# MycroftAI/mimic3

Hardware: AMD Instinct MI355X
Metric: 22.05 kHz audio samples/sec/node (en_UK/apope_low VITS hot path: run + int16, host ids in -> host int16 out) (higher is better)
Workload: dtype f32 (dense convs: operands split exactly into 3 x bf16, 6 bf16-MFMA products per multiply-add, f32 accumulate; f32 in / f32 out, parity at the f32 tolerances)

## Files before the change

include/mi355vits_lab.h:

```cpp
#ifndef MI355VITS_LAB_H
#define MI355VITS_LAB_H

#include "mi355vits.h"

#ifdef __cplusplus
extern "C" {
#endif

typedef struct mi355vits_conv_test {
    int32_t impl, B, Cin, Cout, T, K, dilation;
    const float* x;
    const float* w;
    const float* bias;
    const float* res;
    const int32_t* in_len;
    const int32_t* out_len;
    float in_slope;
    int32_t relu;
    float out_scale;
    int32_t res_sub;
    float* y;
    int32_t accumulate;
    int32_t math;
    const float* cond;
    int32_t mask_before_res;
    int32_t fixed_rule;
} mi355vits_conv_test;
int mi355vits_test_conv1d(int device, const mi355vits_conv_test* t);
int mi355vits_test_conv_transpose1d(int device, int impl, int B, int Cin, int Cout, int Tin, int K, int stride,
                                    const float* x, const float* w, const float* bias, float in_slope, const int32_t* in_len, float* y);
enum {
    MI355VITS_CONVK_GENERIC = 0, MI355VITS_CONVK_F32_STAGED = 1, MI355VITS_CONVK_F32_DIRECT = 2, MI355VITS_CONVK_F32_SPLITK = 3,
    MI355VITS_CONVK_B3_STAGED32 = 4, MI355VITS_CONVK_B3_STAGED64 = 5, MI355VITS_CONVK_B3_PC = 6, MI355VITS_CONVK_ENC_B3 = 7,
    MI355VITS_CONVK_ENC_B3W8 = 8, MI355VITS_CONVK_ENC_B3W6 = 9, MI355VITS_CONVK_RB_CONV = 10, MI355VITS_CONVK_RB_CONV_PW = 11,
    MI355VITS_CONVK_UPS_PL = 12, MI355VITS_CONVK_UPS64 = 13, MI355VITS_CONVK_CONVT_GENERIC = 14
};
typedef struct mi355vits_conv_plan {
    int32_t kernel;
    int32_t cols, rows;
    int32_t MT, NT, WM, WN;
    int32_t chunk;
    int32_t ring;
    int32_t rb_loop;
    int32_t vec, yvec, ovec;
    int32_t grid[3];
    int32_t lds_bytes;
} mi355vits_conv_plan;
int mi355vits_lab_conv_plan(int impl, int B, int Cin, int Cout, int T, int K, int dilation, int stride, int math, int fixed_rule,
                            int has_res, int has_cond, const int32_t* len, mi355vits_conv_plan* out);
int mi355vits_test_enc_o_ln(int device, int math, int B, int T, const float* x, const float* w, const float* bias, const float* res,
                            const float* gamma, const float* beta, float eps, const int32_t* in_len, const int32_t* ln_out_len,
                            int in_place, float* y);
int mi355vits_test_conv_post(int device, int B, int Cin, int K, int L, const float* x, const float* w, const int32_t* valid_len,
                             const double* volumes, float* audio, float* peaks, int16_t* pcm, int32_t* kernel);
int mi355vits_test_fill_workspace(mi355vits_handle h, uint32_t pattern);
int mi355vits_test_rel_attention(int device, int impl, int B, int T, int H, int n_heads, int W, const float* qkv,
                                 const float* emb_rel_k, const float* emb_rel_v, const int32_t* len, float* out);
typedef struct mi355vits_wn_test {
    int32_t impl, B, H, T, K, dilation, Crs, skip_init, math;
    const float* h_in;
    const float* w_in;
    const float* b_in;
    const float* w_rs;
    const float* b_rs;
    const float* cond;
    const int32_t* len;
    float* h_out;
    float* skip;
} mi355vits_wn_test;
int mi355vits_test_wn_layer(int device, const mi355vits_wn_test* t);
int mi355vits_lab_wn_plan(int B, int T, int K, int dilation, int32_t* b3_tile, int32_t* f32_geometry);
typedef struct mi355vits_mrf_test {
    int32_t impl, B, C, T, nrb, math, seg;
    int32_t k[4], d1[4], d2[4];
    const float* x;
    const float* w[4][2];
    const float* bias[4][2];
    const int32_t* len;
    float out_scale;
    float* y;
} mi355vits_mrf_test;
int mi355vits_test_mrf_stage(int device, const mi355vits_mrf_test* t);
int mi355vits_lab_mrf_plan(int impl, int C, int nrb, const int32_t* k, const int32_t* d1, const int32_t* d2, int32_t* width,
                           int32_t* halo, int32_t* x_ring, int32_t* x1_ring);
typedef struct mi355vits_dds_stack_test {
    int32_t impl, math, B, C, T, K, n_layers, pre_mode, zch, proj_cout, spline, nb;
    float tail, inv_sqrt_fc;
    const float* src;
    const float* pre_w;
    const float* pre_b;
    const float* cond;
    const float* dw_w[4];
    const float* dw_b[4];
    const float* g1[4];
    const float* b1[4];
    const float* w1x1[4];
    const float* bias1x1[4];
    const float* g2[4];
    const float* b2[4];
    const float* proj_w;
    const float* proj_b;
    const int32_t* len;
    float* z;
    float* out;
    float* x_out;
} mi355vits_dds_stack_test;
int mi355vits_test_dds_stack(int device, const mi355vits_dds_stack_test* t);
int mi355vits_test_spline_inverse(int device, int B, int T, int nb, int ch_x0, float tail, float inv_sqrt_fc, const float* theta,
                                  const int32_t* len, float* z);
int mi355vits_test_durations(int device, int B, int T, int ch, float ea_m, float ea_logs, const float* z, const int32_t* len,
                             const int32_t* forced, const float* scales, float* logw, int32_t* w_ceil, int32_t* cum, int32_t* ylen);
int mi355vits_test_fit_durations(int device, int B, int T, const float* u, const int32_t* len, const int32_t* min_frames,
                                 const int32_t* target, int32_t* frames, int32_t* cum, int32_t* ylen, float* factor, int32_t* status);
int mi355vits_test_expand_prior(int device, int B, int I, int Tx, int Ty, const float* stats, const int32_t* cum, const int32_t* ylen,
                                const float* injected, int injected_frames, const float* scales, float* z);
int mi355vits_test_speaker_cond(int device, int B, int gin, int n_speakers, int Cout, const float* emb_g, const int64_t* sid,
                                const float* w, const float* bias, float* out, size_t out_floats);
typedef struct mi355vits_speaker_mix_test {
    int32_t B, gin, n_speakers, n_terms, n_jobs;
    const float* emb_g;
    const int64_t* mix_sid;
    const float* mix_weight;
    const float* vectors;
    const float* w[10];
    const float* bias[10];
    int32_t Cout[10];
    float* out[10];
    size_t out_floats[10];
    float* g;
    size_t g_floats;
} mi355vits_speaker_mix_test;
int mi355vits_test_speaker_cond_mix(int device, const mi355vits_speaker_mix_test* t);
int mi355vits_test_levels(int device, int B, int T, int hop, const int32_t* cum, const int32_t* len, const float* gain,
                          const int32_t* ramp, const int32_t* alen, int64_t audio_bs, float* audio, size_t audio_floats, float* peaks);
int mi355vits_test_pitch_table(float* out, size_t capacity);
int mi355vits_test_pitch_plan(int device, int B, int T, int hop, const int32_t* cum, const int32_t* len, const float* ratio,
                              int64_t* tq, int32_t* wc, int32_t* wlen);
int mi355vits_test_pitch(int device, int B, int T, int hop, const int32_t* cum, const int32_t* len, const float* ratio,
                         const float* x, int64_t x_bs, size_t x_floats, float* y, int64_t y_bs, int32_t y_ld, size_t y_floats,
                         float* peaks, int32_t* wlen);
int mi355vits_test_resample(int device, int B, int64_t row_stride, const float* x, const int32_t* lengths, int32_t in_hz,
                            int32_t out_hz, int64_t y_stride, float* y, int32_t* y_lengths, float* peaks);
int mi355vits_test_alignment(int device, int B, int T, const int32_t* frames, const int32_t* len, int64_t row_stride, const float* audio,
                             const int32_t* alen, int32_t hop, int32_t L, int32_t M, int32_t* out_frames, int32_t* out_start,
                             int32_t* out_samples, float* out_peak, float* out_rms);
int mi355vits_lab_edges(const float* audio, long stride, const int32_t* lens, const float* peaks, int B, float ratio, int32_t* s_first,
                        int32_t* s_last);
int mi355vits_lab_loudness(const float* audio, long stride, const int32_t* lens, int B, int32_t rate, double* lufs, int32_t* blocks,
                           int32_t* gated);
int mi355vits_lab_limit(const float* audio, long stride, const int32_t* lens, int B, const double* g, double c, double U, int32_t L,
                        float* scale_out, int64_t* sq_min, int32_t* reduced);
int mi355vits_lab_limit_env(const float* audio, long stride, const int32_t* lens, int B, const double* g, double c, double U, int32_t L,
                            const double* env, float* scale_out, int64_t* sq_min, int32_t* reduced);
int mi355vits_lab_true_peak(const float* audio, long stride, const int32_t* lens, int B, int32_t offset_floats, double* tp, double* env_out);
// ... 18 lines not shown
```

mimic3_amd/_native.py:

```python
from __future__ import annotations

import contextlib
import ctypes
import os
import threading
from typing import Dict, List, Optional, Tuple

import numpy as np

from .config import CVitsConfig, VitsConfig

WANT_FLOAT = 1
WANT_PCM16 = 2
DEVICE_ONLY = 4
DEBUG_TAPS = 8

_HERE = os.path.dirname(os.path.abspath(__file__))
DEFAULT_LIBRARY = os.path.join(_HERE, "csrc", "libmi355vits.so")
HOOKS_LIBRARY = os.path.join(_HERE, "csrc", "libmi355vits_hooks.so")

EXPORTED_SYMBOLS = (
    "mi355vits_version", "mi355vits_device_count", "mi355vits_create", "mi355vits_create_from_buffer", "mi355vits_clone", "mi355vits_destroy",
    "mi355vits_device_result", "mi355vits_set_math", "mi355vits_get_math",
    "mi355vits_get_config", "mi355vits_run", "mi355vits_run_rows", "mi355vits_run_timed", "mi355vits_run_speakers", "mi355vits_run_levels", "mi355vits_run_pitch",
    "mi355vits_get_speaker_embedding", "mi355vits_fetch", "mi355vits_free_result",
    "mi355vits_last_error", "mi355vits_profile_enable", "mi355vits_profile_reset",
    "mi355vits_profile_report", "mi355vits_last_run_ms", "mi355vits_get_tap", "mi355vits_get_tap_rows", "mi355vits_list_taps",
    "mi355vits_run_packed", "mi355vits_fetch_packed", "mi355vits_free_packed",
    "mi355vits_set_output_rate", "mi355vits_get_output_rate",
    "mi355vits_set_output_encoding", "mi355vits_get_output_encoding",
    "mi355vits_set_output_compression", "mi355vits_get_output_compression",
    "mi355vits_fetch_alignment", "mi355vits_free_alignment",
    "mi355vits_set_edge_trim", "mi355vits_get_edge_trim", "mi355vits_fetch_edges", "mi355vits_free_edges",
    "mi355vits_set_loudness_target", "mi355vits_get_loudness_target", "mi355vits_fetch_loudness", "mi355vits_free_loudness",
    "mi355vits_run_streams", "mi355vits_fetch_streams", "mi355vits_free_streams",
    "mi355vits_run_streams2", "mi355vits_fetch_streams2", "mi355vits_free_streams2",
    "mi355vits_set_loudness_limiter", "mi355vits_get_loudness_limiter", "mi355vits_fetch_limiter", "mi355vits_free_limiter",
    "mi355vits_set_loudness_ceiling_mode", "mi355vits_get_loudness_ceiling_mode", "mi355vits_fetch_true_peak", "mi355vits_free_true_peak",
)
LAB_SYMBOLS = (
    "mi355vits_test_conv1d", "mi355vits_test_conv_transpose1d", "mi355vits_test_mfma_layout", "mi355vits_bench_conv1d", "mi355vits_probe_device", "mi355vits_probe_weights",
    "mi355vits_test_rel_attention", "mi355vits_test_fill_workspace", "mi355vits_test_resample",
    "mi355vits_lab_g711_encode", "mi355vits_test_alignment", "mi355vits_lab_edges",
    "mi355vits_lab_loudness", "mi355vits_lab_loudness_plan", "mi355vits_lab_limit",
    "mi355vits_lab_limit_env", "mi355vits_lab_true_peak", "mi355vits_lab_true_peak_plan", "mi355vits_lab_flac", "mi355vits_lab_flac_jobs",
    "mi355vits_test_wn_layer", "mi355vits_lab_wn_plan", "mi355vits_test_mrf_stage", "mi355vits_lab_mrf_plan",
    "mi355vits_test_dds_stack", "mi355vits_test_spline_inverse", "mi355vits_test_durations", "mi355vits_test_expand_prior",
    "mi355vits_test_fit_durations", "mi355vits_test_speaker_cond", "mi355vits_test_speaker_cond_mix", "mi355vits_test_levels",
    "mi355vits_test_pitch_table", "mi355vits_test_pitch_plan", "mi355vits_test_pitch",
    "mi355vits_lab_conv_plan", "mi355vits_test_enc_o_ln", "mi355vits_test_conv_post",
)


class NativeError(RuntimeError):
    def __init__(self, code: int, message: str):
        super().__init__(f"mi355vits error {code}: {message}")
        self.code = code


class WnTest(ctypes.Structure):
    _fields_ = [(n, ctypes.c_int32) for n in ("impl", "B", "H", "T", "K", "dilation", "Crs", "skip_init", "math")] + [
        (n, ctypes.POINTER(ctypes.c_float)) for n in ("h_in", "w_in", "b_in", "w_rs", "b_rs", "cond")] + [
        ("len", ctypes.POINTER(ctypes.c_int32)), ("h_out", ctypes.POINTER(ctypes.c_float)), ("skip", ctypes.POINTER(ctypes.c_float))]


class MrfTest(ctypes.Structure):
    _fields_ = [(n, ctypes.c_int32) for n in ("impl", "B", "C", "T", "nrb", "math", "seg")] + [
        (n, ctypes.c_int32 * 4) for n in ("k", "d1", "d2")] + [
        ("x", ctypes.POINTER(ctypes.c_float)), ("w", (ctypes.POINTER(ctypes.c_float) * 2) * 4),
        ("bias", (ctypes.POINTER(ctypes.c_float) * 2) * 4), ("len", ctypes.POINTER(ctypes.c_int32)),
        ("out_scale", ctypes.c_float), ("y", ctypes.POINTER(ctypes.c_float))]


class DdsStackTest(ctypes.Structure):
    _fields_ = [(n, ctypes.c_int32) for n in ("impl", "math", "B", "C", "T", "K", "n_layers", "pre_mode", "zch", "proj_cout", "spline", "nb")] + [
        ("tail", ctypes.c_float), ("inv_sqrt_fc", ctypes.c_float)] + [
        (n, ctypes.POINTER(ctypes.c_float)) for n in ("src", "pre_w", "pre_b", "cond")] + [
        (n, ctypes.POINTER(ctypes.c_float) * 4) for n in ("dw_w", "dw_b", "g1", "b1", "w1x1", "bias1x1", "g2", "b2")] + [
        ("proj_w", ctypes.POINTER(ctypes.c_float)), ("proj_b", ctypes.POINTER(ctypes.c_float)), ("len", ctypes.POINTER(ctypes.c_int32)),
        ("z", ctypes.POINTER(ctypes.c_float)), ("out", ctypes.POINTER(ctypes.c_float)), ("x_out", ctypes.POINTER(ctypes.c_float))]


MATH_F32, MATH_BF16X3, MATH_BF16W = 0, 1, 2


class RunArgs(ctypes.Structure):
    _fields_ = [
        ("batch", ctypes.c_int32),
        ("tx_max", ctypes.c_int32),
        ("ids", ctypes.POINTER(ctypes.c_int64)),
        ("lengths", ctypes.POINTER(ctypes.c_int64)),
        ("scales", ctypes.POINTER(ctypes.c_float)),
        ("sid", ctypes.POINTER(ctypes.c_int64)),
        ("seed", ctypes.c_uint64),
        ("utterance_base", ctypes.c_uint64),
        ("noise_w", ctypes.POINTER(ctypes.c_float)),
        ("noise_z", ctypes.POINTER(ctypes.c_float)),
        ("noise_z_frames", ctypes.c_int32),
        ("forced_durations", ctypes.POINTER(ctypes.c_int32)),
        ("flags", ctypes.c_uint32),
        ("pcm_volume", ctypes.c_double),
    ]


class RowArgs(ctypes.Structure):
    _fields_ = [
        ("scales", ctypes.POINTER(ctypes.c_float)),
        ("pcm_volume", ctypes.POINTER(ctypes.c_double)),
        ("utterance", ctypes.POINTER(ctypes.c_uint64)),
    ]


class TimingArgs(ctypes.Structure):
    _fields_ = [
        ("stretch", ctypes.POINTER(ctypes.c_float)),
        ("min_frames", ctypes.POINTER(ctypes.c_int32)),
        ("target_frames", ctypes.POINTER(ctypes.c_int32)),
        ("factor_out", ctypes.POINTER(ctypes.c_float)),
        ("reserved", ctypes.c_int32 * 6),
    ]


class SpeakerArgs(ctypes.Structure):
    _fields_ = [
        ("n_terms", ctypes.c_int32),
        ("mix_sid", ctypes.POINTER(ctypes.c_int64)),
        ("mix_weight", ctypes.POINTER(ctypes.c_float)),
        ("vectors", ctypes.POINTER(ctypes.c_float)),
        ("reserved", ctypes.c_int32 * 6),
# ... 400 lines not shown
        L.mi355vits_free_streams2.restype = None
        L.mi355vits_fetch_alignment.argtypes = [H, ctypes.c_uint32, ctypes.POINTER(AlignmentResult)]
        L.mi355vits_free_alignment.argtypes = [ctypes.POINTER(AlignmentResult)]
        L.mi355vits_free_alignment.restype = None
        L.mi355vits_set_edge_trim.argtypes = [H, ctypes.c_float, ctypes.c_int32]
        L.mi355vits_get_edge_trim.argtypes = [H, ctypes.POINTER(ctypes.c_float), ctypes.POINTER(ctypes.c_int32)]
        L.mi355vits_fetch_edges.argtypes = [H, ctypes.POINTER(EdgesResult)]
        L.mi355vits_free_edges.argtypes = [ctypes.POINTER(EdgesResult)]
        L.mi355vits_free_edges.restype = None
        L.mi355vits_set_loudness_target.argtypes = [H, ctypes.c_float, ctypes.c_float]
        L.mi355vits_get_loudness_target.argtypes = [H, ctypes.POINTER(ctypes.c_float), ctypes.POINTER(ctypes.c_float)]
        L.mi355vits_fetch_loudness.argtypes = [H, ctypes.POINTER(LoudnessResult)]
        L.mi355vits_free_loudness.argtypes = [ctypes.POINTER(LoudnessResult)]
        L.mi355vits_free_loudness.restype = None
        L.mi355vits_set_loudness_limiter.argtypes = [H, ctypes.c_int32]
        L.mi355vits_get_loudness_limiter.argtypes = [H]
        L.mi355vits_get_loudness_limiter.restype = ctypes.c_int32
        L.mi355vits_fetch_limiter.argtypes = [H, ctypes.POINTER(LimiterResult)]
        L.mi355vits_free_limiter.argtypes = [ctypes.POINTER(LimiterResult)]
        L.mi355vits_free_limiter.restype = None
        L.mi355vits_set_loudness_ceiling_mode.argtypes = [H, ctypes.c_int]
        L.mi355vits_get_loudness_ceiling_mode.argtypes = [H]
        L.mi355vits_fetch_true_peak.argtypes = [H, ctypes.POINTER(TruePeakResult)]
        L.mi355vits_free_true_peak.argtypes = [ctypes.POINTER(TruePeakResult)]
        L.mi355vits_free_true_peak.restype = None
        L.mi355vits_last_error.argtypes = [H]
        L.mi355vits_last_error.restype = ctypes.c_char_p
        L.mi355vits_profile_enable.argtypes = [H, ctypes.c_int]
        L.mi355vits_profile_reset.argtypes = [H]
        L.mi355vits_profile_report.argtypes = [H, ctypes.c_char_p, ctypes.c_size_t]
        L.mi355vits_profile_report.restype = ctypes.c_long
        L.mi355vits_last_run_ms.argtypes = [H]
        L.mi355vits_last_run_ms.restype = ctypes.c_float
        L.mi355vits_get_tap.argtypes = [H, ctypes.c_char_p, ctypes.POINTER(ctypes.c_float), ctypes.c_size_t,
                                        ctypes.POINTER(ctypes.c_int64)]
        L.mi355vits_get_tap.restype = ctypes.c_long
        L.mi355vits_get_tap_rows.argtypes = [H, ctypes.c_char_p, ctypes.c_long, ctypes.c_long, ctypes.POINTER(ctypes.c_float), ctypes.c_size_t,
                                            ctypes.POINTER(ctypes.c_int64)]
        L.mi355vits_get_tap_rows.restype = ctypes.c_long
        L.mi355vits_list_taps.argtypes = [H, ctypes.c_char_p, ctypes.c_size_t]
        L.mi355vits_list_taps.restype = ctypes.c_long
        present = [hasattr(L, sym) for sym in LAB_SYMBOLS]
        if any(present) and not all(present):
            raise RuntimeError(f"{self.path} exports only part of include/mi355vits_lab.h")
        self.has_hooks = all(present)
        if self.has_hooks:
            L.mi355vits_test_conv1d.argtypes = [ctypes.c_int, ctypes.POINTER(ConvTest)]
            L.mi355vits_test_conv_transpose1d.argtypes = [
                ctypes.c_int, ctypes.c_int, ctypes.c_int, ctypes.c_int, ctypes.c_int, ctypes.c_int, ctypes.c_int,
                ctypes.c_int, ctypes.POINTER(ctypes.c_float), ctypes.POINTER(ctypes.c_float),
                ctypes.POINTER(ctypes.c_float), ctypes.c_float, ctypes.POINTER(ctypes.c_int32), ctypes.POINTER(ctypes.c_float)]
            L.mi355vits_test_fill_workspace.argtypes = [ctypes.c_void_p, ctypes.c_uint32]
            L.mi355vits_test_mfma_layout.argtypes = [ctypes.c_int, ctypes.POINTER(ctypes.c_float)]
            L.mi355vits_bench_conv1d.argtypes = [ctypes.c_int] * 9 + [ctypes.POINTER(ctypes.c_float)]
            L.mi355vits_probe_device.argtypes = [ctypes.c_int, ctypes.POINTER(ctypes.c_double)]
            L.mi355vits_probe_weights.argtypes = [ctypes.c_void_p, ctypes.POINTER(ctypes.c_double)]
            L.mi355vits_test_resample.argtypes = [ctypes.c_int, ctypes.c_int, ctypes.c_int64, ctypes.POINTER(ctypes.c_float),
                                                  ctypes.POINTER(ctypes.c_int32), ctypes.c_int32, ctypes.c_int32, ctypes.c_int64,
                                                  ctypes.POINTER(ctypes.c_float), ctypes.POINTER(ctypes.c_int32),
                                                  ctypes.POINTER(ctypes.c_float)]
            L.mi355vits_lab_g711_encode.argtypes = [ctypes.c_int, ctypes.POINTER(ctypes.c_int16), ctypes.c_long, ctypes.POINTER(ctypes.c_uint8)]
            i32p, f32p = ctypes.POINTER(ctypes.c_int32), ctypes.POINTER(ctypes.c_float)
            L.mi355vits_lab_flac.argtypes = [ctypes.c_void_p, ctypes.c_long, ctypes.c_int32, ctypes.c_int32, ctypes.POINTER(ctypes.c_uint8),
                                             ctypes.c_size_t, ctypes.POINTER(ctypes.c_size_t), i32p]
            L.mi355vits_lab_flac_jobs.argtypes = [ctypes.POINTER(ctypes.c_void_p), ctypes.POINTER(ctypes.c_long), ctypes.c_int32, ctypes.c_int32,
                                                  ctypes.POINTER(ctypes.c_uint8), ctypes.c_size_t, ctypes.POINTER(ctypes.c_size_t),
                                                  ctypes.POINTER(ctypes.c_int64), ctypes.POINTER(ctypes.c_int64)]
            L.mi355vits_lab_edges.argtypes = [f32p, ctypes.c_long, i32p, f32p, ctypes.c_int, ctypes.c_float, i32p, i32p]
            L.mi355vits_lab_loudness.argtypes = [f32p, ctypes.c_long, i32p, ctypes.c_int, ctypes.c_int32, ctypes.POINTER(ctypes.c_double), i32p, i32p]
            L.mi355vits_lab_loudness_plan.argtypes = [ctypes.c_int32, i32p, i32p, i32p]
            L.mi355vits_lab_limit.argtypes = [f32p, ctypes.c_long, i32p, ctypes.c_int, ctypes.POINTER(ctypes.c_double), ctypes.c_double,
                                              ctypes.c_double, ctypes.c_int32, f32p, ctypes.POINTER(ctypes.c_int64), i32p]
            f64p = ctypes.POINTER(ctypes.c_double)
            L.mi355vits_lab_limit_env.argtypes = [f32p, ctypes.c_long, i32p, ctypes.c_int, f64p, ctypes.c_double, ctypes.c_double,
                                                  ctypes.c_int32, f64p, f32p, ctypes.POINTER(ctypes.c_int64), i32p]
            L.mi355vits_lab_true_peak.argtypes = [f32p, ctypes.c_long, i32p, ctypes.c_int, ctypes.c_int32, f64p, f64p]
            L.mi355vits_lab_true_peak_plan.argtypes = [f64p, i32p]
            L.mi355vits_test_alignment.argtypes = [ctypes.c_int, ctypes.c_int, ctypes.c_int, i32p, i32p, ctypes.c_int64, f32p, i32p,
                                                   ctypes.c_int32, ctypes.c_int32, ctypes.c_int32, i32p, i32p, i32p, f32p, f32p]
            L.mi355vits_test_rel_attention.argtypes = [ctypes.c_int] * 7 + [ctypes.POINTER(ctypes.c_float)] * 3 + [
                ctypes.POINTER(ctypes.c_int32), ctypes.POINTER(ctypes.c_float)]
            L.mi355vits_test_wn_layer.argtypes = [ctypes.c_int, ctypes.POINTER(WnTest)]
            L.mi355vits_lab_wn_plan.argtypes = [ctypes.c_int] * 4 + [i32p, i32p]
            L.mi355vits_test_mrf_stage.argtypes = [ctypes.c_int, ctypes.POINTER(MrfTest)]
            L.mi355vits_lab_mrf_plan.argtypes = [ctypes.c_int] * 3 + [i32p] * 7
            L.mi355vits_lab_conv_plan.argtypes = [ctypes.c_int] * 12 + [i32p, ctypes.POINTER(ConvPlan)]
            L.mi355vits_test_enc_o_ln.argtypes = [ctypes.c_int] * 4 + [f32p] * 6 + [ctypes.c_float, i32p, i32p, ctypes.c_int, f32p]
            L.mi355vits_test_conv_post.argtypes = [ctypes.c_int] * 5 + [f32p, f32p, i32p, ctypes.POINTER(ctypes.c_double), f32p, f32p,
                                                   ctypes.POINTER(ctypes.c_int16), i32p]
            L.mi355vits_test_dds_stack.argtypes = [ctypes.c_int, ctypes.POINTER(DdsStackTest)]
            L.mi355vits_test_spline_inverse.argtypes = [ctypes.c_int] * 5 + [ctypes.c_float, ctypes.c_float, f32p, i32p, f32p]
            L.mi355vits_test_fit_durations.argtypes = [ctypes.c_int] * 3 + [f32p, i32p, i32p, i32p, i32p, i32p, i32p, f32p, i32p]
            L.mi355vits_test_speaker_cond.argtypes = [ctypes.c_int] * 5 + [f32p, ctypes.POINTER(ctypes.c_int64), f32p, f32p, f32p, ctypes.c_size_t]
            L.mi355vits_test_speaker_cond_mix.argtypes = [ctypes.c_int, ctypes.POINTER(SpeakerMixTest)]
            L.mi355vits_test_levels.argtypes = [ctypes.c_int] * 4 + [i32p, i32p, f32p, i32p, i32p, ctypes.c_int64, f32p, ctypes.c_size_t, f32p]
            L.mi355vits_test_pitch_table.argtypes = [f32p, ctypes.c_size_t]
            L.mi355vits_test_pitch_plan.argtypes = [ctypes.c_int] * 4 + [i32p, i32p, f32p, ctypes.POINTER(ctypes.c_int64), i32p, i32p]
            L.mi355vits_test_pitch.argtypes = [ctypes.c_int] * 4 + [i32p, i32p, f32p, f32p, ctypes.c_int64, ctypes.c_size_t, f32p, ctypes.c_int64,
                                               ctypes.c_int32, ctypes.c_size_t, f32p, i32p]
            L.mi355vits_test_durations.argtypes = [ctypes.c_int] * 4 + [ctypes.c_float, ctypes.c_float, f32p, i32p, i32p, f32p, f32p, i32p, i32p, i32p]
            L.mi355vits_test_expand_prior.argtypes = [ctypes.c_int] * 5 + [f32p, i32p, i32p, f32p, ctypes.c_int, f32p, f32p]

    def _need_hooks(self):
        if not self.has_hooks:
            raise RuntimeError(f"{self.path} is the product library: the hooks of include/mi355vits_lab.h live in "
                               "libmi355vits_hooks.so (mimic3_amd._native.hooks_library()), the lab build and the CPU model")

    def version(self) -> str:
        return self.lib.mi355vits_version().decode()

    def device_count(self) -> int:
        return int(self.lib.mi355vits_device_count())

    def create_error(self) -> str:
        return (self.lib.mi355vits_last_error(None) or b"").decode("utf-8", "replace")

    def lab_g711_encode(self, law, samples) -> np.ndarray:
        self._need_hooks()
        x = np.ascontiguousarray(samples, np.int16).reshape(-1)
        out = np.empty(x.shape[0], np.uint8)
        rc = self.lib.mi355vits_lab_g711_encode(encoding_id(law), x.ctypes.data_as(ctypes.POINTER(ctypes.c_int16)), x.shape[0],
                                                out.ctypes.data_as(ctypes.POINTER(ctypes.c_uint8)))
        if rc != 0:
            raise NativeError(rc, self.create_error())
        return out

    def lab_flac(self, samples, rate: int, first_frame: int = 0):
        self._need_hooks()
        x = np.asarray(samples)
        if x.dtype != np.int16 or x.ndim != 1 or not x.flags.c_contiguous:
            x = np.ascontiguousarray(samples, np.int16).reshape(-1)
        n = int(x.shape[0])
        frames = (n + 4095) // 4096
        out = np.empty(42 + 16 * frames + 2 * n, np.uint8)
        sizes = np.zeros(max(frames, 1), np.int32)
        got = ctypes.c_size_t(0)
        rc = self.lib.mi355vits_lab_flac(ctypes.c_void_p(x.ctypes.data), n, int(rate), int(first_frame),
                                         out.ctypes.data_as(ctypes.POINTER(ctypes.c_uint8)), out.shape[0], ctypes.byref(got),
                                         sizes.ctypes.data_as(ctypes.POINTER(ctypes.c_int32)))
        if rc != 0:
            raise NativeError(rc, self.create_error())
        return out[: int(got.value)].tobytes(), sizes[:frames].copy()

    def lab_flac_jobs(self, arrays, rate: int):
        self._need_hooks()
        xs = []
        for a in arrays:
            x = np.asarray(a)
            if x.dtype != np.int16 or x.ndim != 1 or not x.flags.c_contiguous:
                x = np.ascontiguousarray(a, np.int16).reshape(-1)
            xs.append(x)
        J = len(xs)
        ptrs = (ctypes.c_void_p * max(J, 1))(*[x.ctypes.data for x in xs])
        ns = (ctypes.c_long * max(J, 1))(*[int(x.shape[0]) for x in xs])
        cap = sum(((42 + 16 * ((int(x.shape[0]) + 4095) // 4096) + 2 * int(x.shape[0]) + 15) & ~15) for x in xs) + 16
        out = np.empty(cap, np.uint8)
        offsets, sizes = np.zeros(max(J, 1), np.int64), np.zeros(max(J, 1), np.int64)
        got = ctypes.c_size_t(0)
        rc = self.lib.mi355vits_lab_flac_jobs(ptrs, ns, J, int(rate), out.ctypes.data_as(ctypes.POINTER(ctypes.c_uint8)), cap, ctypes.byref(got),
                                              offsets.ctypes.data_as(ctypes.POINTER(ctypes.c_int64)),
                                              sizes.ctypes.data_as(ctypes.POINTER(ctypes.c_int64)))
        if rc != 0:
            raise NativeError(rc, self.create_error())
        return out[: int(got.value)].copy(), offsets[:J].copy(), sizes[:J].copy()

    def lab_edges(self, audio, lengths, peaks, ratio):
# ... 163 lines not shown
        assert C == 192 and res.shape == x.shape and w.shape == (C, C, 1) and gamma.shape == beta.shape == (C,)
        y = np.zeros_like(x) if y_prior is None else f(y_prior).copy()
        i32 = lambda a: None if a is None else np.ascontiguousarray(a, np.int32)
        il, ol = i32(in_len), i32(ln_out_len)
        ip = lambda a: None if a is None else a.ctypes.data_as(ctypes.POINTER(ctypes.c_int32))
        rc = self.lib.mi355vits_test_enc_o_ln(device, int(math), B, T, _fptr(x), _fptr(w), _fptr(bias), _fptr(res), _fptr(gamma), _fptr(beta),
                                              float(eps), ip(il), ip(ol), int(bool(in_place)), _fptr(y))
        if rc != 0:
            raise NativeError(rc, self.create_error())
        return y

    def test_conv_post(self, x, w, valid_len, volumes=None, audio_prior=None, pcm_prior=None, device=0):
        self._need_hooks()
        x = np.ascontiguousarray(x, np.float32)
        w = np.ascontiguousarray(w, np.float32)
        B, Cin, L = x.shape
        assert w.shape[:2] == (1, Cin)
        K = w.shape[2]
        vl = np.ascontiguousarray(valid_len, np.int32)
        assert vl.shape == (B,)
        vol = None if volumes is None else np.ascontiguousarray(volumes, np.float64)
        audio = np.zeros((B, L), np.float32) if audio_prior is None else np.ascontiguousarray(audio_prior, np.float32).copy()
        pcm = np.zeros((B, L), np.int16) if pcm_prior is None else np.ascontiguousarray(pcm_prior, np.int16).copy()
        peaks = np.full(B, -1.0, np.float32)
        kernel = ctypes.c_int32(-1)
        rc = self.lib.mi355vits_test_conv_post(device, B, Cin, K, L, _fptr(x), _fptr(w), vl.ctypes.data_as(ctypes.POINTER(ctypes.c_int32)),
                                               None if vol is None else vol.ctypes.data_as(ctypes.POINTER(ctypes.c_double)), _fptr(audio),
                                               _fptr(peaks), pcm.ctypes.data_as(ctypes.POINTER(ctypes.c_int16)), ctypes.byref(kernel))
        if rc != 0:
            raise NativeError(rc, self.create_error())
        return audio, peaks, pcm, int(kernel.value)

    def emu_set_cu_count(self, n: int) -> None:
        if not hasattr(self.lib, "mi355vits_emu_set_cu_count"):
            raise RuntimeError(f"{self.path} is not the CPU model of the kernels")
        self.lib.mi355vits_emu_set_cu_count(ctypes.c_int(int(n)))

    def test_rel_attention(self, qkv, emb_rel_k, emb_rel_v, lengths, n_heads, impl=2, device=0) -> np.ndarray:
        self._need_hooks()
        qkv = np.ascontiguousarray(qkv, np.float32)
        ek = np.ascontiguousarray(emb_rel_k, np.float32)
        ev = np.ascontiguousarray(emb_rel_v, np.float32)
        ln = np.ascontiguousarray(lengths, np.int32)
        B, H3, T = qkv.shape
        H = H3 // 3
        W = (ek.shape[0] - 1) // 2
        out = np.zeros((B, H, T), np.float32)
        rc = self.lib.mi355vits_test_rel_attention(device, impl, B, T, H, n_heads, W, _fptr(qkv), _fptr(ek), _fptr(ev),
                                                   ln.ctypes.data_as(ctypes.POINTER(ctypes.c_int32)), _fptr(out))
        if rc != 0:
            raise NativeError(rc, self.create_error())
        return out

    def test_wn_layer(self, h, skip, w_in, b_in, w_rs, b_rs, lengths, dilation=1, cond=None, skip_init=False, impl=1, math=None,
                      h_out_prior=None, device=0):
        self._need_hooks()
        f = lambda a: np.ascontiguousarray(a, np.float32)
        h, w_in, b_in, w_rs, b_rs = f(h), f(w_in), f(b_in), f(w_rs), f(b_rs)
        skip = f(skip).copy()
        B, H, T = h.shape
        ln = np.ascontiguousarray(lengths, np.int32)
        h_out = np.zeros_like(h) if h_out_prior is None else f(h_out_prior).copy()
        assert skip.shape == h.shape == h_out.shape and w_in.shape[:2] == (2 * H, H) and w_rs.shape[1:] == (H, 1) and ln.shape == (B,)
        assert b_in.shape == (2 * H,) and b_rs.shape == (w_rs.shape[0],)
        c = None if cond is None else f(cond)
        assert c is None or c.shape == (B, 2 * H)
        t = WnTest()
        t.impl, t.B, t.H, t.T, t.K, t.dilation, t.Crs, t.skip_init = impl, B, H, T, w_in.shape[2], int(dilation), w_rs.shape[0], int(bool(skip_init))
        t.math = (MATH_BF16X3 if impl == 2 else MATH_F32) if math is None else int(math)
        t.h_in, t.w_in, t.b_in, t.w_rs, t.b_rs, t.cond = _fptr(h), _fptr(w_in), _fptr(b_in), _fptr(w_rs), _fptr(b_rs), _fptr(c)
        t.len, t.h_out, t.skip = ln.ctypes.data_as(ctypes.POINTER(ctypes.c_int32)), _fptr(h_out), _fptr(skip)
        rc = self.lib.mi355vits_test_wn_layer(device, ctypes.byref(t))
        if rc != 0:
            raise NativeError(rc, self.create_error())
        return h_out, skip

    def lab_wn_plan(self, B, T, K=5, dilation=1):
        self._need_hooks()
        tile, geom = ctypes.c_int32(), ctypes.c_int32()
        rc = self.lib.mi355vits_lab_wn_plan(int(B), int(T), int(K), int(dilation), ctypes.byref(tile), ctypes.byref(geom))
        if rc != 0:
            raise NativeError(rc, self.create_error())
        return int(tile.value), int(geom.value)

    def test_mrf_stage(self, x, ks, d1, d2, weights, biases, lengths, impl=0, math=None, out_scale=0.0, seg=0, y_prior=None, device=0):
        self._need_hooks()
        x = np.ascontiguousarray(x, np.float32)
        B, C, T = x.shape
        ln = np.ascontiguousarray(lengths, np.int32)
        y = np.zeros_like(x) if y_prior is None else np.ascontiguousarray(y_prior, np.float32).copy()
        nrb = len(ks)
        assert y.shape == x.shape and ln.shape == (B,) and 1 <= nrb <= 4 and len(d1) == len(d2) == len(weights) == len(biases) == nrb
        t = MrfTest()
        t.impl, t.B, t.C, t.T, t.nrb, t.seg = impl, B, C, T, nrb, int(seg)
        t.math = (MATH_F32 if impl == 0 else MATH_BF16X3) if math is None else int(math)
        keep = []
        for j in range(nrb):
            t.k[j], t.d1[j], t.d2[j] = int(ks[j]), int(d1[j]), int(d2[j])
            for q in range(2):
                w = np.ascontiguousarray(weights[j][q], np.float32)
                bq = np.ascontiguousarray(biases[j][q], np.float32)
                assert w.shape == (C, C, ks[j]) and bq.shape == (C,)
                keep += [w, bq]
                t.w[j][q], t.bias[j][q] = _fptr(w), _fptr(bq)
        t.x, t.len, t.out_scale, t.y = _fptr(x), ln.ctypes.data_as(ctypes.POINTER(ctypes.c_int32)), float(out_scale), _fptr(y)
        rc = self.lib.mi355vits_test_mrf_stage(device, ctypes.byref(t))
        if rc != 0:
            raise NativeError(rc, self.create_error())
        return y

    def lab_mrf_plan(self, impl, C, ks, d1, d2):
        self._need_hooks()
        arr = lambda v: (ctypes.c_int32 * len(v))(*[int(e) for e in v])
        out = [ctypes.c_int32() for _ in range(4)]
        rc = self.lib.mi355vits_lab_mrf_plan(int(impl), int(C), len(ks), arr(ks), arr(d1), arr(d2), *[ctypes.byref(o) for o in out])
        if rc != 0:
            raise NativeError(rc, self.create_error())
        return tuple(int(o.value) for o in out)

    def test_dds_stack(self, src, pre_w, pre_b, layers, lengths, impl=2, math=None, cond=None, z=None, zch=0, proj_w=None, proj_b=None,
                       spline=False, nb=0, tail=0.0, inv_sqrt_fc=0.0, out_prior=None, x_out_prior=None, device=0):
        self._need_hooks()
        f = lambda a: np.ascontiguousarray(a, np.float32)
        src, pre_w, pre_b = f(src), f(pre_w), f(pre_b)
        B, C, T = src.shape
        ln = np.ascontiguousarray(lengths, np.int32)
        affine = pre_w.ndim == 1
        assert pre_w.shape == ((C,) if affine else (C, C, 1)) and pre_b.shape == (C,) and ln.shape == (B,) and 1 <= len(layers) <= 4
        t = DdsStackTest()
        keep = []
        K = np.asarray(layers[0]["dw_w"]).shape[2]
        for i, lay in enumerate(layers):
            for name, shape in (("dw_w", (C, 1, K)), ("dw_b", (C,)), ("g1", (C,)), ("b1", (C,)), ("w1x1", (C, C, 1)), ("bias1x1", (C,)),
                                ("g2", (C,)), ("b2", (C,))):
                a = f(lay[name])
                assert a.shape == shape, (name, a.shape, shape)
                keep.append(a)
                getattr(t, name)[i] = _fptr(a)
        c = None if cond is None else f(cond)
        assert c is None or c.shape == (B, C)
        zz = None if z is None else f(z).copy()
        assert zz is None or zz.shape == (B, 2, T)
        pw = None if proj_w is None else f(proj_w)
        pb = None if proj_b is None else f(proj_b)
        Cp = 0 if pw is None else pw.shape[0]
        assert pw is None or (pw.shape == (Cp, C, 1) and pb is not None and pb.shape == (Cp,))
        out = None if pw is None else (np.zeros((B, Cp, T), np.float32) if out_prior is None else f(out_prior).copy())
        x_out = np.zeros_like(src) if x_out_prior is None else f(x_out_prior).copy()
        assert x_out.shape == src.shape and (out is None or out.shape == (B, Cp, T))
        t.impl, t.B, t.C, t.T, t.K, t.n_layers, t.pre_mode, t.zch = int(impl), B, C, T, K, len(layers), int(affine), int(zch)
        t.math = (MATH_BF16X3 if impl == 3 else MATH_F32) if math is None else int(math)
        t.proj_cout, t.spline, t.nb, t.tail, t.inv_sqrt_fc = Cp, int(bool(spline)), int(nb), float(tail), float(inv_sqrt_fc)
        t.src, t.pre_w, t.pre_b, t.cond, t.proj_w, t.proj_b = _fptr(src), _fptr(pre_w), _fptr(pre_b), _fptr(c), _fptr(pw), _fptr(pb)
        t.len, t.z, t.out, t.x_out = ln.ctypes.data_as(ctypes.POINTER(ctypes.c_int32)), _fptr(zz), _fptr(out), _fptr(x_out)
        rc = self.lib.mi355vits_test_dds_stack(device, ctypes.byref(t))
        if rc != 0:
            raise NativeError(rc, self.create_error())
        return x_out, out, zz

    def test_spline_inverse(self, theta, z, lengths, nb, ch_x0=0, tail=5.0, inv_sqrt_fc=1.0, device=0) -> np.ndarray:
        self._need_hooks()
        theta = np.ascontiguousarray(theta, np.float32)
        z = np.ascontiguousarray(z, np.float32).copy()
        ln = np.ascontiguousarray(lengths, np.int32)
        B, _, T = z.shape
        assert z.shape == (B, 2, T) and theta.shape[0] == B and theta.shape[2] == T and ln.shape == (B,)
# ... 1008 lines not shown
```

mimic3_amd/csrc/b3.h:

```cpp
#pragma once
#include "kernels.h"

namespace m355 {

#ifdef MI355_EMU
static inline int b3_drop() {
    const char* e = getenv("MI355VITS_EMU_DROP");
    return e ? atoi(e) : 0;
}
#else
__device__ __forceinline__ constexpr int b3_drop() { return 0; }
#endif

template <int MT, int NT, int NG, int NA = NT, bool W1 = false>
__device__ __forceinline__ void b3_chunk(f32x16 (&acc)[MT][NA], const uint4* const (&wp)[MT], const uint4* __restrict__ xq, int PS ,
                                         int LD, int K, int groups_per_tap, int dil) {
    uint4 ra[2][MT][3];
    uint4 rb[2][NT][3];
    const int drop = b3_drop();
    constexpr int NPA = W1 ? 1 : 3;
    MI355_UNROLL
    for (int i = 0; i < MT; ++i)
        MI355_UNROLL
        for (int p = 0; p < NPA; ++p) ra[0][i][p] = wp[i][p * 64];
// ... 207 lines not shown
        MI355_UNROLL
        for (int i = 0; i < MT; ++i)
            MI355_UNROLL
            for (int p = 0; p < NPA; ++p) dst[i][p] = wp[i][woff + p * 64];
    };
    MI355_UNROLL
    for (int d = 0; d < D; ++d) load_a(d, ra[d]);
    MI355_UNROLL
    for (int j = 0; j < NT; ++j)
        MI355_UNROLL
        for (int p = 0; p < 3; ++p) rb[j][p] = xq[p * PS + j * 32];
    for (int k = 0; k < K; ++k) {
        const bool last_tap = k == K - 1;
        MI355_UNROLL
        for (int g = 0; g < NG; ++g) {
            const bool wrap = g + 1 == NG;
            const int xoff = wrap ? (last_tap ? k * dil + g * 2 * LD : (k + 1) * dil) : k * dil + (g + 1) * 2 * LD;
            load_a(k * NG + g + D, ra[(g + D) % RA]);
            SCHED_FENCE();
            MI355_UNROLL
            for (int j = 0; j < NT; ++j) {
                if constexpr (!W1) {
                    MI355_UNROLL
                    for (int i = 0; i < MT; ++i) acc[i][j] = MFMA_32x32x16_BF16(ra[g % RA][i][2], rb[j][0], acc[i][j]);
                }
                MI355_UNROLL
                for (int i = 0; i < MT; ++i) acc[i][j] = MFMA_32x32x16_BF16(ra[g % RA][i][0], rb[j][2], acc[i][j]);
                if constexpr (!W1) {
                    MI355_UNROLL
                    for (int i = 0; i < MT; ++i) acc[i][j] = MFMA_32x32x16_BF16(ra[g % RA][i][1], rb[j][1], acc[i][j]);
                    MI355_UNROLL
                    for (int i = 0; i < MT; ++i) acc[i][j] = MFMA_32x32x16_BF16(ra[g % RA][i][1], rb[j][0], acc[i][j]);
                }
                MI355_UNROLL
                for (int i = 0; i < MT; ++i) acc[i][j] = MFMA_32x32x16_BF16(ra[g % RA][i][0], rb[j][1], acc[i][j]);
                MI355_UNROLL
                for (int i = 0; i < MT; ++i) acc[i][j] = MFMA_32x32x16_BF16(ra[g % RA][i][0], rb[j][0], acc[i][j]);
                SCHED_FENCE();
                MI355_UNROLL
                for (int p = 0; p < 3; ++p) rb[j][p] = xq[p * PS + xoff + j * 32];
                SCHED_FENCE();
            }
        }
    }
}

template <int MT, int NT, int NG>
__device__ __forceinline__ void h2_chunk_lean(f32x16 (&acc)[MT][NT], const uint4* const (&wp)[MT], const uint4* __restrict__ xq, int PS, int LD,
                                              int K, int groups_per_tap, int dil) {
    uint4 ra[2][MT][2];
    uint4 rb[NT][2];
    MI355_UNROLL
    for (int i = 0; i < MT; ++i)
        MI355_UNROLL
        for (int p = 0; p < 2; ++p) ra[0][i][p] = wp[i][p * 64];
    MI355_UNROLL
    for (int j = 0; j < NT; ++j)
        MI355_UNROLL
        for (int p = 0; p < 2; ++p) rb[j][p] = xq[p * PS + j * 32];
    for (int k = 0; k < K; ++k) {
        const bool last_tap = k == K - 1;
        MI355_UNROLL
        for (int g = 0; g < NG; ++g) {
            const int cur = g & 1, nxt = cur ^ 1;
            const bool wrap = g + 1 == NG;
            const long woff = (wrap ? (last_tap ? (long)k * groups_per_tap + g : (long)(k + 1) * groups_per_tap) : (long)k * groups_per_tap + g + 1) * 128;
            const int xoff = wrap ? (last_tap ? k * dil + g * 2 * LD : (k + 1) * dil) : k * dil + (g + 1) * 2 * LD;
            MI355_UNROLL
            for (int i = 0; i < MT; ++i)
                MI355_UNROLL
                for (int p = 0; p < 2; ++p) ra[nxt][i][p] = wp[i][woff + p * 64];
            SCHED_FENCE();
            MI355_UNROLL
            for (int j = 0; j < NT; ++j) {
                MI355_UNROLL
                for (int i = 0; i < MT; ++i) acc[i][j] = MFMA_32x32x16_F16(ra[cur][i][1], rb[j][0], acc[i][j]);
                MI355_UNROLL
                for (int i = 0; i < MT; ++i) acc[i][j] = MFMA_32x32x16_F16(ra[cur][i][0], rb[j][1], acc[i][j]);
                MI355_UNROLL
                for (int i = 0; i < MT; ++i) acc[i][j] = MFMA_32x32x16_F16(ra[cur][i][0], rb[j][0], acc[i][j]);
                SCHED_FENCE();
                MI355_UNROLL
                for (int p = 0; p < 2; ++p) rb[j][p] = xq[p * PS + xoff + j * 32];
                SCHED_FENCE();
            }
        }
    }
}

template <int NG, int GB = 4, bool F16 = false>
__device__ __forceinline__ void stage_planes(const float* __restrict__ xb, long x_ld, int LD, int ts, int tend, float slope,
                                             uint4* __restrict__ planes, int PS, int tid, int nthreads) {
    static_assert((NG * 2) % GB == 0, "batches of GB (group, half) rows");
    const int last = tend > 0 ? tend - 1 : 0;
    int nparts = 1, part = 0, col0 = tid;
    if (nthreads >= 2 * LD) {
        nparts = nthreads / LD;
        part = tid / LD;
        col0 = tid - part * LD;
        if (part >= nparts) return;
    }
    for (int col = col0; col < LD; col += nthreads) {
        const int tt = ts + col;
        const bool in = tt >= 0 && tt < tend;
        const int tc = tt < 0 ? 0 : (tt > last ? last : tt);
        for (int g0 = part * GB; g0 < NG * 2; g0 += nparts * GB) {
            float v[GB][8];
            MI355_UNROLL
            for (int u = 0; u < GB; ++u) {
                const int gh = g0 + u, cbase = (gh >> 1) * 16 + (gh & 1) * 4;
                MI355_UNROLL
                for (int e = 0; e < 8; ++e) v[u][e] = xb[(long)(cbase + 8 * (e >> 2) + (e & 3)) * x_ld + tc];
            }
            SCHED_FENCE();
            MI355_UNROLL
            for (int u = 0; u < GB; ++u) {
                MI355_UNROLL
                for (int e = 0; e < 8; ++e) v[u][e] = in ? lrelu_f(v[u][e], slope) : 0.0f;
                const int o = (g0 + u) * LD + col;
                if constexpr (F16) {
                    MI355_UNROLL
                    for (int e = 0; e < 8; ++e) v[u][e] *= F16X2_X_SCALE;
                    uint4 h, m;
                    split2_pk(v[u][0], v[u][1], h.x, m.x);
                    split2_pk(v[u][2], v[u][3], h.y, m.y);
                    split2_pk(v[u][4], v[u][5], h.z, m.z);
                    split2_pk(v[u][6], v[u][7], h.w, m.w);
                    planes[o] = h;
                    planes[PS + o] = m;
                } else {
                    uint4 h, m, l;
                    split3_pk(v[u][0], v[u][1], h.x, m.x, l.x);
                    split3_pk(v[u][2], v[u][3], h.y, m.y, l.y);
                    split3_pk(v[u][4], v[u][5], h.z, m.z, l.z);
                    split3_pk(v[u][6], v[u][7], h.w, m.w, l.w);
                    planes[o] = h;
                    planes[PS + o] = m;
                    planes[2 * PS + o] = l;
                }
            }
        }
    }
}

}
```

mimic3_amd/csrc/engine.cpp:

```cpp
#include "engine.h"

#include <algorithm>
#include <cmath>
#include <cstdlib>
#include <cstring>
#include <fstream>
#include <sstream>
#include <type_traits>

namespace m355 {

namespace {
struct Reader {
    const unsigned char* p;
    size_t n, pos = 0;
    void need(size_t k) const {
        if (pos + k > n) throw EngineError(MI355VITS_ERR_FORMAT, "weight container truncated");
    }
    template <typename T> T get() {
        need(sizeof(T));
        T v;
        memcpy(&v, p + pos, sizeof(T));
        pos += sizeof(T);
        return v;
// ... 144 lines not shown
void Profiler::clear() {
    (void)hipStreamSynchronize(stream);
    for (auto& r : recs) { pool.push_back(r.a); pool.push_back(r.b); }
    recs.clear();
}
std::string Profiler::report() {
    HIP_CHECK(hipStreamSynchronize(stream));
    struct Agg { long calls = 0; double ms = 0, flops = 0, bytes = 0; };
    std::vector<Agg> agg(names.size());
    for (auto& r : recs) {
        float ms = 0;
        if (hipEventElapsedTime(&ms, r.a, r.b) != hipSuccess) ms = 0;
        Agg& a = agg[r.name_id];
        a.calls++;
        a.ms += ms;
        a.flops += r.flops;
        a.bytes += r.bytes;
    }
    std::ostringstream os;
    os.precision(9);
    for (size_t i = 0; i < names.size(); ++i)
        if (agg[i].calls) os << names[i] << " " << agg[i].calls << " " << agg[i].ms << " " << agg[i].flops << " " << agg[i].bytes << "\n";
    return os.str();
}

size_t Engine::stage(const float* p, size_t n) {
    const size_t off = (host_stage_.size() + 63) & ~size_t(63);
    host_stage_.resize(off + n);
    if (n) memcpy(host_stage_.data() + off, p, n * sizeof(float));
    return off;
}

const ConvW& Engine::add_conv_data(const std::string& key, const std::vector<float>& w, const std::vector<float>* bias,
                                   int Cout, int Cin, int K, int epi, ConvRole role) {
    if (w.size() != (size_t)Cout * Cin * K) throw EngineError(MI355VITS_ERR_INTERNAL, "add_conv_data size: " + key);
    ConvW c;
    c.Cout = Cout; c.Cin = Cin; c.K = K; c.epi = epi;
    c.raw = stage(w.data(), w.size());
    if (bias) c.bias = stage(bias->data(), bias->size());
    if (conv1d_mfma_supported(Cin, Cout, K, 1)) {
        std::vector<float> pk(mfma_packed_floats(Cout, Cin, K), 0.0f);
        pack_conv_weights_mfma_mode(w.data(), Cout, Cin, K, epi == EPI_GATE ? EPI_GATE : EPI_STD, pk.data());
        c.packed = stage(pk.data(), pk.size());
        const bool rb = role == ROLE_RESBLOCK && epi == EPI_STD;
        if (rb && Cin % 8 == 0 && Cout % 32 == 0) {
            std::vector<float> p4(pk.size());
            regroup_packed_x4(pk.data(), pk.size(), p4.data());
            c.packed4 = stage(p4.data(), p4.size());
        }
        if (rb && Cin % 16 == 0 && Cout % 32 == 0) {
            std::vector<uint32_t> b3(bf16x3_packed_words(Cout, Cin, K));
            pack_conv_weights_bf16x3(w.data(), Cout, Cin, K, b3.data());
            static_assert(sizeof(uint32_t) == sizeof(float), "bit patterns travel in the float arena");
            c.packed_b3 = stage(reinterpret_cast<const float*>(b3.data()), b3.size());
            std::vector<uint32_t> h2(f16x2_packed_words(Cout, Cin, K));
            if (pack_conv_weights_f16x2(w.data(), Cout, Cin, K, h2.data()))
                c.packed_h2 = stage(reinterpret_cast<const float*>(h2.data()), h2.size());
        }
        if (rb && Cin == Cout && Cin % 32 == 0 && (K == 3 || K == 5 || K == 7)) {
            std::vector<uint32_t> pp(p16_packed_words(Cout, Cin, K));
            pack_conv_weights_p16(w.data(), Cout, Cin, K, pp.data());
            c.packed_p = stage(reinterpret_cast<const float*>(pp.data()), pp.size());
        }
        if (role == ROLE_UPSAMPLER && epi == EPI_STD && (Cin == 64 || Cin == 128 || Cin == 256) && Cout % 128 == 0 && K == 2) {
            std::vector<uint32_t> pp(p16_packed_words(Cout, Cin, K));
            pack_conv_weights_p16n(w.data(), Cout, Cin, K, pp.data());
            c.packed_p = stage(reinterpret_cast<const float*>(pp.data()), pp.size());
        }
        if (Cin % 32 == 0 && (epi == EPI_GATE ? (Cout / 2) % 32 == 0 : true)) {
            const int pe = epi == EPI_GATE ? EPI_GATE : EPI_STD;
            std::vector<uint32_t> b3(bf16x3_packed_words_mode(Cout, Cin, K, pe));
            pack_conv_weights_bf16x3_mode(w.data(), Cout, Cin, K, pe, 1, b3.data());
            c.packed_b3s = stage(reinterpret_cast<const float*>(b3.data()), b3.size());
            std::vector<float> wg;
            if (epi == EPI_GATE && Cout % 32 == 0) {
                const int Hh = Cout / 2;
                const size_t row = (size_t)Cin * K;
                wg.resize(w.size());
                for (int q = 0; q < Cout / 32; ++q)
                    for (int r = 0; r < 32; ++r) {
                        const int src = (r < 16 ? 0 : Hh) + 16 * q + (r & 15);
                        memcpy(wg.data() + ((size_t)32 * q + r) * row, w.data() + (size_t)src * row, row * sizeof(float));
                    }
                std::vector<uint32_t> bw(bf16x3_packed_words_mode(Cout, Cin, K, EPI_STD));
                pack_conv_weights_bf16x3_mode(wg.data(), Cout, Cin, K, EPI_STD, 1, bw.data());
                c.packed_b3w = stage(reinterpret_cast<const float*>(bw.data()), bw.size());
            }
            if (Cin % 16 == 0 && Cout % 32 == 0) {
                std::vector<uint32_t> h2(f16x2_packed_words(Cout, Cin, K));
                if (pack_conv_weights_f16x2(wg.empty() ? w.data() : wg.data(), Cout, Cin, K, h2.data(), 1))
                    c.packed_h2s = stage(reinterpret_cast<const float*>(h2.data()), h2.size());
            }
        }
    }
    return model_->convs[key] = c;
}

const ConvW& Engine::add_conv(const WeightsFile& wf, const std::string& key, const std::string& tensor, int Cout, int Cin,
                              int K, bool bias, int epi, ConvRole role) {
    const HostTensor& w = wf.get(tensor + ".weight", {Cout, Cin, K});
    std::vector<float> wv(w.data, w.data + w.count), bv;
    if (bias) {
        const HostTensor& b = wf.get(tensor + ".bias", {Cout});
        bv.assign(b.data, b.data + b.count);
    }
    return add_conv_data(key, wv, bias ? &bv : nullptr, Cout, Cin, K, epi, role);
}

void Engine::add_vec(const WeightsFile& wf, const std::string& name, std::initializer_list<int> dims) {
    const HostTensor& t = wf.get(name, dims);
    model_->vecs[name] = stage(t.data, t.count);
}
const float* Engine::vec(const std::string& name) const {
    auto it = model_->vecs.find(name);
    if (it == model_->vecs.end()) throw EngineError(MI355VITS_ERR_INTERNAL, "unknown tensor: " + name);
    return model_->dev_weights + it->second;
}
const ConvW& Engine::cw(const std::string& key) const {
    auto it = model_->convs.find(key);
    if (it == model_->convs.end()) throw EngineError(MI355VITS_ERR_INTERNAL, "unknown conv: " + key);
    return it->second;
}

static std::string S(const char* fmt, int a = 0, int b = 0, int c = 0) {
    char buf[160];
    snprintf(buf, sizeof(buf), fmt, a, b, c);
    return buf;
}

static void validate_config(const mi355vits_config& c) {
    auto bad = [](const std::string& m) { throw EngineError(MI355VITS_ERR_FORMAT, "invalid voice config: " + m); };
    if (c.num_symbols < 1 || c.n_speakers < 1) bad("num_symbols / n_speakers");
    if (c.hidden_channels < 2 || c.hidden_channels % 2 || c.inter_channels < 2 || c.inter_channels % 2) bad("channel counts must be even");
    if (c.n_heads < 1 || c.hidden_channels % c.n_heads) bad("hidden_channels % n_heads");
    if (c.resblock != 1 && c.resblock != 2) bad("resblock must be 1 or 2");
    if (c.n_upsamples < 1 || c.n_upsamples > MI355VITS_MAX_STAGES) bad("n_upsamples");
    if (c.n_resblock_kernels < 1 || c.n_resblock_kernels > MI355VITS_MAX_STAGES) bad("n_resblock_kernels");
    long hop = 1;
    int ch = c.upsample_initial_channel;
    for (int i = 0; i < c.n_upsamples; ++i) {
        if (c.upsample_rates[i] < 1 || c.upsample_kernel_sizes[i] < c.upsample_rates[i]) bad("upsample stage");
        if ((c.upsample_kernel_sizes[i] - c.upsample_rates[i]) % 2) bad("upsample kernel - rate must be even");
        if (ch % 2) bad("upsample channels must halve evenly");
        ch /= 2;
        hop *= c.upsample_rates[i];
    }
    if (ch % 2) bad("decoder channel counts must be even");
    if (hop != c.hop_length) bad("hop_length must equal the product of upsample_rates");
    for (int j = 0; j < c.n_resblock_kernels; ++j) {
        if (c.resblock_kernel_sizes[j] < 1 || c.resblock_kernel_sizes[j] % 2 == 0) bad("resblock kernel sizes must be odd");
        if (c.resblock_n_dilations[j] < 1 || c.resblock_n_dilations[j] > MI355VITS_MAX_STAGES) bad("resblock dilations");
    }
    if (c.n_speakers > 1 && c.gin_channels < 1) bad("multi-speaker voice needs gin_channels");
    const bool det_dp = c.dp_n_flows == 0;
    if (det_dp ? (c.dp_num_bins != 0 || c.dp_dds_layers != 0) : (c.dp_num_bins < 2 || c.dp_num_bins > 16)) bad("dp_num_bins");
    if ((!det_dp && c.dp_n_flows < 2) || c.flow_n_flows < 1 || c.flow_wn_layers < 1) bad("flow depth");
    if (c.flow_wn_kernel % 2 == 0 || c.dp_kernel_size % 2 == 0) bad("flow / dp kernels must be odd");
    if (c.window_size < 0 || c.n_layers < 1 || c.kernel_size < 1) bad("encoder");
    if (c.num_symbols > (1 << 20) || c.n_speakers > (1 << 20) || c.hidden_channels > 8192 || c.inter_channels > 8192 ||
        c.filter_channels < 1 || c.filter_channels > 32768 || c.upsample_initial_channel < 2 || c.upsample_initial_channel > 8192 ||
        c.gin_channels < 0 || c.gin_channels > 8192)
        bad("channel / symbol counts out of range");
    if (c.n_layers > 64 || c.kernel_size > 63 || c.window_size > 15 || c.flow_n_flows > 32 || c.flow_wn_layers > 32 ||
        c.flow_wn_kernel < 1 || c.flow_wn_kernel > 63 || c.flow_wn_dilation_rate < 1 || c.flow_wn_dilation_rate > 8 ||
        c.dp_n_flows > 16 || (!det_dp && c.dp_dds_layers < 1) || c.dp_dds_layers > 8 || c.dp_kernel_size < 1 || c.dp_kernel_size > 63 ||
        !(c.dp_tail_bound > 0.0f) || c.hop_length > (1 << 16))
        bad("depth / kernel sizes out of range");
    for (int i = 0; i < c.n_upsamples; ++i)
        if (c.upsample_rates[i] > 64 || c.upsample_kernel_sizes[i] > 256) bad("upsample stage out of range");
// ... 757 lines not shown
    ConvArgs pr;
    pr.x = d_d0_; pr.x_bs = bs; pr.x_ld = Tx;
    pr.y = d_h_; pr.y_bs = bs; pr.y_ld = Tx;
    pr.in_len = d_len_; pr.out_len = d_len_;
    pr.B = B; pr.T = Tx;
    if (!stack) conv("dp.proj", cw("dp.proj"), pr);
    tap("dp.h", d_h_, {B, H, Tx});

    {
        ProfScope ps(prof_, "sdp.noise");
        launch_sdp_noise(d_z2_, d_noise_w_, B, Tx, d_scales_, in.seed, d_utt_, stream_);
    }
    int ch0 = 0;
    for (int j = c.dp_n_flows - 1; j >= 1; --j) {
        ch0 ^= 1;
        const std::string p = S("dp.flows.%d", 1 + 2 * j);
        if (stack && stack_w(cw(p + ".proj")) != nullptr) {
            DdsStackArgs a;
            a.src = d_h_;
            a.pre_mode = DDS_PRE_AFFINE;
            a.pre_w = vec(p + ".pre.weight");
            a.pre_b = vec(p + ".pre.bias");
            a.z = d_z2_;
            a.zch = ch0;
            stack_layers(a, p + ".convs");
            a.proj_w = stack_w(cw(p + ".proj"));
            a.proj_b = P(cw(p + ".proj").bias);
            a.proj_cout = nth;
            a.spline = 1;
            a.nb = c.dp_num_bins;
            a.tail = c.dp_tail_bound;
            a.inv_sqrt_fc = 1.0f / sqrtf((float)H);
            ProfScope ps(prof_, "convflow.stack", stack_flops * c.dp_dds_layers + 2.0 * B * (double)Tx * H * nth, 12.0 * B * H * Tx);
            launch_dds_stack(a, H, stream_);
            continue;
        }
        {
            ProfScope ps(prof_, "convflow.pre", 0, 12.0 * B * H * Tx);
            launch_convflow_pre(d_z2_, ch0, vec(p + ".pre.weight"), vec(p + ".pre.bias"), d_h_, B, H, Tx, d_d0_, stream_);
        }
        dds(p + ".convs", d_d0_, d_d1_, d_d2_, B, Tx);
        ConvArgs a;
        a.x = d_d0_; a.x_bs = bs; a.x_ld = Tx;
        a.y = d_theta_; a.y_bs = (long)nth * Tx; a.y_ld = Tx;
        a.in_len = d_len_; a.out_len = d_len_;
        a.B = B; a.T = Tx;
        conv("convflow.proj", cw(p + ".proj"), a);
        {
            ProfScope ps(prof_, "spline");
            launch_spline_inverse(d_z2_, ch0, d_theta_, d_len_, B, Tx, c.dp_num_bins, c.dp_tail_bound,
                                  1.0f / sqrtf((float)H), stream_);
        }
    }
    ch0 ^= 1;
    durations(in, ch0, model_->ea_m[0], model_->ea_logs[0]);
}

static const char* stage_label(int i, const char* const (&t)[4]) { return t[std::min(i, 3)]; }

void Engine::coupling_layer(int j, int B, int Ty) {
    const mi355vits_config& c = cfg_;
    const int H = c.hidden_channels, I = c.inter_channels, half = I / 2;
    const long zbs = (long)I * Ty, hbs = (long)H * Ty;
    const bool rev = ((c.flow_n_flows - 1 - j) % 2) == 0;
    float* x0 = d_z_ + (rev ? (long)half * Ty : 0);
    float* x1 = d_z_ + (rev ? 0 : (long)half * Ty);
    ConvArgs pre;
    pre.x = x0; pre.x_bs = zbs; pre.x_ld = Ty;
    pre.y = d_fh_; pre.y_bs = hbs; pre.y_ld = Ty;
    pre.out_len = d_ylen_;
    pre.B = B; pre.T = Ty;
    conv("flow.pre", cw(S("flow.%d.pre", j)), pre);
    float* hcur = d_fh_;
    float* hnext = d_fh2_;
    for (int l = 0; l < c.flow_wn_layers; ++l) {
        int dil = 1;
        for (int q = 0; q < l; ++q) dil *= c.flow_wn_dilation_rate;
        const ConvW& win = cw(S("flow.%d.in.%d", j, l));
        const ConvW& wrs = cw(S("flow.%d.rs.%d", j, l));
        const float* cond_l = d_cond_flow_.empty() ? nullptr : d_cond_flow_[j] + (long)l * 2 * H;
        const bool wn_b3 = sw_.wn_b3 && math_on_bf16(kmath()) && win.packed_b3s != NO_OFF && wrs.packed_b3s != NO_OFF &&
                           conv1d_b3_supported(win.Cin, win.Cout, win.K, dil, Ty) && !sw_.force_generic;
        const bool fused = !sw_.force_generic && !sw_.no_fused_wn && !wn_b3;
        const bool b3 = fused && math_on_bf16(kmath()) && win.packed_b3w != NO_OFF && wrs.packed_b3s != NO_OFF &&
                        wn_layer_b3_supported(H, win.K, dil);
        if (b3 || (fused && wn_layer_fused_supported(H, win.K, dil))) {
            const bool h2 = b3 && math_ == MATH_F16X2 && win.packed_h2s != NO_OFF && wrs.packed_h2s != NO_OFF;
            WnArgs w;
            w.h_in = hcur; w.h_out = hnext; w.h_bs = hbs; w.h_ld = Ty;
            w.skip = d_fskip_; w.s_bs = hbs; w.s_ld = Ty;
            w.w_in = P(h2 ? win.packed_h2s : (b3 ? win.packed_b3w : win.packed)); w.b_in = P(win.bias);
            w.w_rs = P(h2 ? wrs.packed_h2s : (b3 ? wrs.packed_b3s : wrs.packed)); w.b_rs = P(wrs.bias);
            w.cond = cond_l; w.cond_bs = 2L * H * c.flow_wn_layers;
            w.len = d_ylen_;
            w.B = B; w.H = H; w.T = Ty; w.K = win.K; w.dil = dil; w.Crs = wrs.Cout; w.skip_init = (l == 0);
            if (b3) w.math = h2 ? (int)MATH_F16X2 : kmath();
            const double fl = 2.0 * B * (double)Ty * H * ((double)win.Cout * win.K + wrs.Cout);
            ProfScope ps(prof_, b3 ? "flow.wn_layer_b3" : "flow.wn_layer", fl, 4.0 * B * (double)Ty * H * 4);
            if (b3) launch_wn_layer_b3(w, stream_);
            else launch_wn_layer(w, stream_);
            if (wrs.Cout == 2 * H) std::swap(hcur, hnext);
            continue;
        }
        ConvArgs in;
        in.x = hcur; in.x_bs = hbs; in.x_ld = Ty;
        in.y = d_fu_; in.y_bs = hbs; in.y_ld = Ty;
        in.epi = EPI_GATE; in.H = H; in.dil = dil;
        if (cond_l) {
            in.cond = cond_l;
            in.cond_bs = 2L * H * c.flow_wn_layers;
        }
        in.B = B; in.T = Ty;
        if (wn_b3) in.math = kmath();
        conv("flow.in_gate", win, in);
        ConvArgs rs;
        rs.x = d_fu_; rs.x_bs = hbs; rs.x_ld = Ty;
        rs.y = hcur; rs.y_bs = hbs; rs.y_ld = Ty;
        rs.y2 = d_fskip_; rs.y2_bs = hbs; rs.y2_ld = Ty;
        rs.epi = EPI_RESSKIP; rs.H = H; rs.skip_init = (l == 0);
        rs.out_len = d_ylen_;
        rs.B = B; rs.T = Ty;
        if (wn_b3) rs.math = kmath();
        conv("flow.res_skip", wrs, rs);
    }
    ConvArgs post;
    post.x = d_fskip_; post.x_bs = hbs; post.x_ld = Ty;
    post.y = x1; post.y_bs = zbs; post.y_ld = Ty;
    post.res = x1; post.res_bs = zbs; post.res_ld = Ty; post.res_sub = 1;
    post.in_len = d_ylen_; post.out_len = d_ylen_;
    post.B = B; post.T = Ty;
    conv("flow.post_couple", cw(S("flow.%d.post", j)), post);
}

ConvArgs Engine::rb2_conv_args(int i, int j, int m, int B, int ch, long T) const {
    const mi355vits_config& c = cfg_;
    float* const pp[2] = {d_bufB_, d_bufT_};
    const bool last = (m == c.resblock_n_dilations[j] - 1);
    const float* src = m == 0 ? d_bufA_ : pp[(m - 1) & 1];
    ConvArgs a;
    a.x = src; a.x_bs = (long)ch * T; a.x_ld = (int)T;
    a.y = last ? d_bufC_ : pp[m & 1]; a.y_bs = (long)ch * T; a.y_ld = (int)T;
    a.res = src; a.res_bs = (long)ch * T; a.res_ld = (int)T;
    a.in_slope = 0.1f; a.dil = c.resblock_dilations[j * MI355VITS_MAX_STAGES + m];
    a.in_len = d_slen_ + (long)(i + 1) * B;
    if (last) { a.out_scale = 1.0f / c.n_resblock_kernels; a.accumulate = (j > 0); }
    a.B = B; a.T = (int)T;
    return a;
}

int Engine::mrf_stage(int i, int B, int ch, long T) {
    const mi355vits_config& c = cfg_;
    const int nk = c.n_resblock_kernels;
    if (sw_.force_generic || sw_.no_fused_mrf || c.resblock != 2 || nk > MRF_MAX_RB) return 0;
    MrfArgs m;
    for (int j = 0; j < nk; ++j) {
        if (c.resblock_n_dilations[j] != 2) return 0;
        m.k[j] = c.resblock_kernel_sizes[j];
        m.d1[j] = c.resblock_dilations[j * MI355VITS_MAX_STAGES + 0];
        m.d2[j] = c.resblock_dilations[j * MI355VITS_MAX_STAGES + 1];
    }
    m.x = d_bufA_; m.x_bs = (long)ch * T; m.x_ld = (int)T;
    m.y = d_bufC_; m.y_bs = (long)ch * T; m.y_ld = (int)T;
    m.len = d_slen_ + (long)(i + 1) * B; m.B = B; m.C = ch; m.T = (int)T;
    m.len_host = h_slen_.data() + (size_t)(i + 1) * B;
    auto rb = [&](int j, int q) -> const ConvW& { return cw(S("dec.rb.%d.c.%d", i * nk + j, q)); };
    double flops = 0;
    auto take = [&](int n, size_t ConvW::*fmt) {
        flops = 0;
        for (int j = 0; j < n; ++j) {
            for (int q = 0; q < 2; ++q) {
                const ConvW& w = rb(j, q);
                if (w.*fmt == NO_OFF) return false;
                m.w[j][q] = P(w.*fmt);
                m.bias[j][q] = P(w.bias);
            }
// ... 652 lines not shown
```

mimic3_amd/csrc/engine.h:

```cpp
#pragma once
#include <map>
#include <memory>
#include <mutex>
#include <string>
#include <unordered_map>
#include <vector>

#include "../../include/mi355vits.h"
#include "kernels.h"

namespace m355 {

struct EngineError : std::runtime_error {
    int code;
    EngineError(int c, const std::string& m) : std::runtime_error(m), code(c) {}
};

struct HostTensor {
    std::vector<int> dims;
    const float* data = nullptr;
    size_t count = 0;
};
struct WeightsFile {
    mi355vits_config cfg{};
    std::map<std::string, HostTensor> tensors;
    std::vector<unsigned char> storage;
    void parse(const void* blob, size_t n);
    void load(const std::string& path);
    const HostTensor& get(const std::string& name, std::initializer_list<int> dims) const;
};

class DeviceArena {
  public:
    ~DeviceArena();
    void reserve(size_t bytes, hipStream_t s);
    void reset() { off_ = 0; }
    void rewind(size_t off) { off_ = off; }
    void fill(uint32_t pattern, hipStream_t s);
    template <typename T> T* alloc(size_t n) { return reinterpret_cast<T*>(alloc_bytes(n * sizeof(T))); }
    size_t capacity() const { return cap_; }
    size_t used() const { return off_; }
    static size_t padded(size_t bytes) { return (bytes + 255) & ~size_t(255); }

  private:
    void* alloc_bytes(size_t bytes);
    unsigned char* base_ = nullptr;
    size_t cap_ = 0, off_ = 0;
};
struct ArenaCount {
    size_t bytes = 0;
    template <typename T> T* alloc(size_t n) { bytes += DeviceArena::padded(n * sizeof(T)); return nullptr; }
};

struct Profiler {
    struct Rec { int name_id; hipEvent_t a, b; double flops, bytes; };
    bool enabled = false;
    std::vector<std::string> names;
    std::unordered_map<std::string, int> ids;
    std::vector<Rec> recs;
    std::vector<hipEvent_t> pool;
    hipStream_t stream = nullptr;
    ~Profiler();
    int begin(const char* name, double flops, double bytes);
    void end(int rec);
    void clear();
    std::string report();
  private:
    hipEvent_t get_event();
};
struct ProfScope {
    Profiler& p;
    int rec;
    ProfScope(Profiler& prof, const char* name, double flops = 0, double bytes = 0) : p(prof), rec(-1) {
        if (p.enabled) rec = p.begin(name, flops, bytes);
    }
    ~ProfScope() {
        if (rec >= 0) p.end(rec);
    }
};

struct Tap {
    std::string name;
    float* dev;
    std::vector<int64_t> dims;
    size_t count;
};

constexpr size_t NO_OFF = ~size_t(0);

struct ConvW {
    size_t raw = NO_OFF;
    size_t packed = NO_OFF;
    size_t packed4 = NO_OFF;
    size_t packed_b3 = NO_OFF;
    size_t packed_b3s = NO_OFF;
    size_t packed_b3w = NO_OFF;
    size_t packed_h2 = NO_OFF;
    size_t packed_p = NO_OFF;
    size_t packed_h2s = NO_OFF;
    size_t bias = NO_OFF;
    int Cout = 0, Cin = 0, K = 1;
    int epi = EPI_STD;
};
enum ConvRole { ROLE_PLAIN, ROLE_RESBLOCK, ROLE_UPSAMPLER };
enum ConvKernel { UPS_PL, RB_CONV, ENC_B3, STAGED_B3, STAGED_F16X2, MFMA_F32, GENERIC };

struct LabSwitches {
    bool force_generic = false;
    bool no_fused_wn = false;
    bool no_fused_mrf = false;
    int b3_min_work = 256;
    bool wn_b3 = false;
    bool no_mrf_p = false;
    bool no_rbc = false;
    bool no_fused_dds = false;
    bool no_dds_stack = false;
    bool no_dds_stack_b3 = false;
    bool no_enc_gemm = false;
    bool no_enc_o_ln = false;
    bool no_flow_gemm = false;
    bool no_f16x2_convs = false;
    static LabSwitches from_env();
};

struct Model {
    int device = 0;
    float* dev_weights = nullptr;
    std::unordered_map<std::string, ConvW> convs;
    std::unordered_map<std::string, size_t> vecs;
    float ea_m[2] = {0, 0}, ea_logs[2] = {0, 0};
    std::vector<float> emb_g;
    int dp_filter = 0;
    bool flow_reversed_out = false;
    size_t bytes = 0;
    ~Model();
};

struct PackSettings {
    int enc = PACK_ENC_S16;
    float trim_ratio = 0.0f;
    int trim_keep = 0;
    float loud_target = 0.0f, loud_ceiling = -1.0f;
    int limit_window = 0;
    int ceil_mode = 0;
    int compress = 0;
    bool trimmed() const { return trim_ratio != 0.0f; }
    bool normalised() const { return loud_target != 0.0f; }
    bool limiting() const { return normalised() && limit_window > 0; }
    bool true_peak() const { return normalised() && ceil_mode == MI355VITS_CEILING_TRUE_PEAK; }
    bool flac() const { return compress == MI355VITS_COMPRESS_FLAC; }
};

struct RunCall {
    const mi355vits_run_args& args;
    const mi355vits_row_args* rows = nullptr;
    const mi355vits_timing_args* timing = nullptr;
    const mi355vits_speaker_args* speakers = nullptr;
    const mi355vits_level_args* levels = nullptr;
    const mi355vits_pitch_args* pitch = nullptr;
};
struct RunInputs {
    int B = 0, Tx = 0;
    uint64_t seed = 0;
    uint32_t flags = 0;
    const int64_t* ids = nullptr;
    const int64_t* sid = nullptr;
    std::vector<int> len32;
    std::vector<float> sc3;
    std::vector<double> vol;
    std::vector<unsigned long long> utt;
    const int32_t* forced_durations = nullptr;
    const float* noise_w = nullptr;
    const float* noise_z = nullptr;
    int noise_z_frames = 0;
    bool any_noise_z = false;
    mi355vits_timing_args timing{};
    bool timed() const { return timing.stretch || timing.min_frames || timing.target_frames; }
    enum Speakers { SPK_NONE, SPK_MIX, SPK_VECTORS };
// ... 330 lines not shown
```

mimic3_amd/csrc/kernels.h:

```cpp
#pragma once
#include "hipx.h"

#include <vector>

namespace m355 {

struct Profiler;

enum ConvEpilogue { EPI_STD = 0, EPI_GATE = 1, EPI_RESSKIP = 2 };

struct ConvArgs {
    const float* x = nullptr; long x_bs = 0; int x_ld = 0;
    float* y = nullptr;       long y_bs = 0; int y_ld = 0;
    const float* w = nullptr;
    const float* wb3 = nullptr;
    int math = 0;
    const float* bias = nullptr;
    const float* cond = nullptr; long cond_bs = 0;
    const float* res = nullptr; long res_bs = 0; int res_ld = 0;
    float* y2 = nullptr; long y2_bs = 0; int y2_ld = 0;
    const int* in_len = nullptr;
    const int* in_len_host = nullptr;
    int nvalid = 0;
    int rb_loop = 0;
// ... 77 lines not shown
size_t bf16x3_packed_words_mode(int Cout, int Cin, int K, int epi);
void pack_conv_weights_bf16x3_mode(const float* w, int Cout, int Cin, int K, int epi, int layout, uint32_t* out);
bool conv1d_b3_supported(int Cin, int Cout, int K, int dil, int T_hint);
void pack_conv_weights_mfma_mode(const float* w, int Cout, int Cin, int K, int epi, float* out);

struct ConvTArgs {
    const float* x = nullptr; long x_bs = 0; int x_ld = 0;
    float* y = nullptr; long y_bs = 0; int y_ld = 0;
    const float* w = nullptr;
    const float* bias = nullptr;
    const int* in_len = nullptr;
    int B = 1, Cin = 0, Cout = 0, Tin = 0, K = 0, stride = 0, pad = 0;
    float in_slope = 1.0f;
};
void launch_conv_transpose1d(const ConvTArgs& a, hipStream_t s);
ConvPlan conv_transpose1d_plan(const ConvTArgs& a);
int convt_taps(int K, int stride);
void convt_to_polyphase(const float* w, const float* bias, int Cin, int Cout, int K, int stride, float* w_out,
                        float* bias_out);

constexpr int MRF_MAX_RB = 4;
struct MrfArgs {
    const float* x = nullptr; long x_bs = 0; int x_ld = 0;
    float* y = nullptr; long y_bs = 0; int y_ld = 0;
    const float* w[MRF_MAX_RB][2] = {};
    int math = 0;
    const float* bias[MRF_MAX_RB][2] = {};
    int k[MRF_MAX_RB] = {}, d1[MRF_MAX_RB] = {}, d2[MRF_MAX_RB] = {};
    int nrb = 0;
    const int* len = nullptr;
    int B = 1, C = 0, T = 0;
    int R = 0, ldx = 0, ld1 = 0, vec = 0;
    float out_scale = 0.0f;
    int ablate = 0;
    int seg = 0;
    unsigned* clk = nullptr;
    const int* len_host = nullptr;
    int nvalid = 0;
    int prio = 0;
};
bool mrf_fused_supported(int C, int nrb, const int* k, const int* d1, const int* d2);
void launch_mrf_fused(MrfArgs a, hipStream_t s);
inline int mrf_stage_halo(int nrb, const int* k, const int* d1, const int* d2) {
    int R = 0;
    for (int j = 0; j < nrb; ++j) {
        const int r = (k[j] - 1) / 2 * d1[j] + (k[j] - 1) / 2 * d2[j];
        R = R > r ? R : r;
    }
    return R;
}
struct MrfPlan { int width = 0, halo = 0, x_ring = 0, x1_ring = 0; };
bool mrf_fused_plan(int C, int nrb, const int* k, const int* d1, const int* d2, MrfPlan* out);
bool mrf_p_plan(int C, int nrb, const int* k, const int* d1, const int* d2, MrfPlan* out);
bool mrf_s_plan(int C, int nrb, const int* k, const int* d1, const int* d2, MrfPlan* out);
size_t p16_packed_words(int Cout, int Cin, int K);
void pack_conv_weights_p16(const float* w, int Cout, int Cin, int K, uint32_t* out);
bool mrf_p_supported(int C, int nrb, const int* k, const int* d1, const int* d2);
void launch_mrf_p(MrfArgs a, hipStream_t s);
bool mrf_s_supported(int C, int nrb, const int* k, const int* d1, const int* d2);
int mrf_s_segment(int C, int B, int T, int cus, const int* len_host = nullptr);
void launch_mrf_s(MrfArgs a, hipStream_t s);
bool rb_conv_supported(const ConvArgs& a);
void launch_rb_conv(ConvArgs a, hipStream_t s);
void pack_conv_weights_p16n(const float* w, int Cout, int Cin, int K, uint32_t* out);
bool ups_pl_supported(const ConvArgs& a);
void launch_ups_pl(ConvArgs a, hipStream_t s);
int valid_items(const int* len_host, const int* len_dev, int B, int T, int block, int extra = 0);
int current_device_cu_count();
void set_max_dynamic_lds(const void* fn, int bytes);

struct WnArgs {
    const float* h_in = nullptr; float* h_out = nullptr; long h_bs = 0; int h_ld = 0;
    float* skip = nullptr; long s_bs = 0; int s_ld = 0;
    const float* w_in = nullptr;
    const float* b_in = nullptr;
    const float* w_rs = nullptr;
    const float* b_rs = nullptr;
    const float* cond = nullptr; long cond_bs = 0;
    const int* len = nullptr;
    int B = 1, H = 0, T = 0, K = 1, dil = 1, Crs = 0, skip_init = 0;
    int ldx = 0, vec = 0;
    int ablate = 0;
    int math = 0;
};
bool wn_layer_fused_supported(int H, int K, int dil);
void launch_wn_layer(WnArgs a, hipStream_t s);
bool wn_layer_b3_supported(int H, int K, int dil);
void launch_wn_layer_b3(WnArgs a, hipStream_t s);
int wn_layer_b3_column_tiles(const WnArgs& a);
int wn_layer_geometry(const WnArgs& a);

void launch_conv_post_tanh(const float* x, long x_bs, int x_ld, const float* w, int Cin, int K, int B, int L,
                           const int* valid_len, float* audio, long audio_bs, unsigned* peak_bits, hipStream_t s);
int conv_post_kernel(const float* x, long x_bs, int x_ld, int Cin, int K, const float* audio, long audio_bs);
void launch_pcm16(const float* audio, long audio_bs, const unsigned* peak_bits, const int* valid_len, int B, int L,
                  int16_t* pcm, long pcm_bs, hipStream_t s, const double* volumes = nullptr);
enum PackEncoding { PACK_ENC_S16 = 0, PACK_ENC_ULAW = 1, PACK_ENC_ALAW = 2, PACK_ENC_F32 = 3 };
constexpr int pack_bytes_per_sample(int enc) { return enc == PACK_ENC_S16 ? 2 : enc == PACK_ENC_F32 ? 4 : 1; }
inline size_t pack_capacity_bytes(int enc, long total) { return ((size_t)total * pack_bytes_per_sample(enc) + 15) & ~size_t(15); }
enum { PACK_SEG_OFFSET = 0, PACK_SEG_ROW = 1, PACK_SEG_LENGTH = 2, PACK_SEG_SKIP = 3 };
constexpr int pack_seg_scale_row(bool trimmed) { return trimmed ? 4 : 3; }
constexpr int pack_seg_rows(bool trimmed, bool normalised) { return pack_seg_scale_row(trimmed) + (normalised ? 1 : 0); }
constexpr int pack_seg_curve_row(bool trimmed) { return pack_seg_scale_row(trimmed) + 1; }
constexpr int pack_seg_rows(bool trimmed, bool normalised, bool curved) { return pack_seg_rows(trimmed, normalised) + (curved ? 1 : 0); }
void launch_pack(int enc, const float* audio, long audio_bs, const unsigned* peak_bits, const double* volumes, const int* seg, int n,
                 uint8_t* out, long total, hipStream_t s, bool trimmed, bool normalised, const float* curve = nullptr);
enum { PACK_ENT_OFFSET = 0, PACK_ENT_ROW = 1, PACK_ENT_LENGTH = 2, PACK_ENT_SKIP = 3, PACK_ENT_ENC = 4, PACK_ENT_SCALE = 5, PACK_ENT_ROWS = 6 };
enum { PACK_ENT_SCALED = 4, PACK_ENT_CURVED = 8 };
enum { PACK_ENT_CURVE = 6 };
constexpr int pack_ent_rows(bool curved) { return curved ? PACK_ENT_ROWS + 1 : PACK_ENT_ROWS; }
enum { PACK_STREAM_BEGIN = 0, PACK_STREAM_DATA = 1, PACK_STREAM_END = 2, PACK_STREAM_ENC = 3, PACK_STREAM_HEADER = 4, PACK_STREAM_WORDS = 20 };
constexpr long PACK_STREAMS_ITEM_BYTES = 256L * 16;
inline size_t pack_streams_capacity(long n_bytes) { return ((size_t)n_bytes + 15) & ~size_t(15); }
inline size_t pack_streams_table_words(int n_entries, int n_streams, bool curved = false) {
    return (size_t)pack_ent_rows(curved) * n_entries + (size_t)PACK_STREAM_WORDS * n_streams;
}
void launch_pack_streams(const float* audio, long audio_bs, const unsigned* peak_bits, const double* volumes, const int* tab, int n_entries,
                         int n_streams, uint8_t* out, long n_bytes, hipStream_t s, const float* curve = nullptr);
void launch_g711_encode(int law, const int16_t* in, long n, uint8_t* out, hipStream_t s);

constexpr int FLAC_BLOCK = 4096;
constexpr int FLAC_SLOT_BYTES = 8208;
constexpr int FLAC_HEADER_BYTES = 42;
constexpr int FLAC_MAX_RATE = 0xfffff;
constexpr long FLAC_MAX_FRAME_NUMBER = 0x1fffff;
struct FlacJob {
    const int16_t* src;
    long n;
    int first_frame;
    int slot0;
};
inline long flac_frames(long n) { return (n + FLAC_BLOCK - 1) / FLAC_BLOCK; }
inline size_t flac_out_capacity(long n_frames, long total) { return (16 * (size_t)n_frames + 2 * (size_t)total + 15) & ~size_t(15); }
void launch_flac_frames(const FlacJob* jobs, int n_jobs, long n_frames, int rate, uint8_t* slots, int* sizes, hipStream_t s);
void launch_flac_gather(const uint8_t* slots, int* sizes, long long* offsets, long n_frames, uint8_t* out, hipStream_t s);
void flac_stream_header(uint8_t* h, int rate, int64_t total, const int* sizes, long n_frames);
enum { FLAC_INFO_BASE = 0, FLAC_INFO_BYTES = 1, FLAC_INFO_MIN = 2, FLAC_INFO_MAX = 3, FLAC_INFO_WORDS = 4 };
constexpr int FLAC_HDR_WORDS = 12;
constexpr int FLAC_JTAB_ROWS = 5;
constexpr long FLAC_GATHER_ITEM_BYTES = 256L * 16;
inline size_t flac_info_words(long n_frames, int n_jobs) { return (size_t)n_frames + (size_t)FLAC_INFO_WORDS * n_jobs + 1; }
inline size_t flac_gather_items(long bound_bytes) { return (size_t)((bound_bytes + FLAC_GATHER_ITEM_BYTES - 1) / FLAC_GATHER_ITEM_BYTES) + 2; }
inline long flac_file_bound(long total) { return (FLAC_HEADER_BYTES + 16 * flac_frames(total) + 2 * total + 15) & ~15L; }
void launch_flac_place(const FlacJob* jobs, int n_jobs, long n_frames, int rate, long base0, int* sizes, unsigned* pre, int2* ftab,
                       unsigned* hdr, int* item_first, int* jtab, hipStream_t s);
void launch_flac_gather_streams(int n_jobs, long n_frames, const uint8_t* slots, const int* sizes, const int2* ftab, const unsigned* hdr,
                                const int* item_first, long base0, long bound_bytes, uint8_t* out, hipStream_t s);

constexpr int RESAMPLE_MAX_RATIO = 640;
struct ResampleFilter {
    int in_hz = 0, out_hz = 0;
    int L = 1, M = 1, half = 0;
    int tpp = 0;
    int tp = 0;
    int tile = 0;
    std::vector<float> table;
};
bool resample_design(int in_hz, int out_hz, ResampleFilter& f);
inline long long resample_out_len(long long n, int L, int M) { return (n * L + M - 1) / M; }
inline size_t resample_tab_ints(int B) { return 2 * (size_t)B + 1; }
long resample_fill_tab(const ResampleFilter& f, const int* n_in, int B, int* tab);
void launch_resample(const ResampleFilter& f, const float* coef, const float* x, long x_bs, const int* x_len, int B, const int* tab,
                     long items, float* y, long y_bs, int y_ld, unsigned* peak_bits, hipStream_t s);

void launch_align(const int* w_ceil, const int* cum, const int* len, int B, int T, const float* audio, long audio_bs, const int* alen,
                  int hop, int L, int M, int* frames, int* start, int* samples, float* peak, float* rms, hipStream_t s,
                  const int* wc = nullptr );

void launch_edges(const float* audio, long audio_bs, const int* alen, const unsigned* peak_bits, int B, long l_max, float ratio,
                  int* first, int* last, hipStream_t s);

// ... 212 lines not shown
```

mimic3_amd/csrc/kernels_conv.cpp:

```cpp
#include <cmath>
#include <cstdio>
#include <cstdlib>

#include <cstring>

#include "kernels.h"
#include <atomic>
#include <type_traits>
#include "b3.h"

namespace m355 {

__device__ __forceinline__ void epi_std(const ConvArgs& a, int b, int co, int t, float v, int out_len) {
    if (a.bias) v += a.bias[co];
    if (a.shuf_s) {
        const int c = co / a.shuf_s, r = co - c * a.shuf_s;
        const int n = t * a.shuf_s + r - a.shuf_p;
        if (n >= 0 && n < a.shuf_T) a.y[(long)b * a.y_bs + (long)c * a.y_ld + n] = v;
        return;
    }
    if (a.cond) v += a.cond[(long)b * a.cond_bs + co];
    if (a.relu) v = fmaxf(v, 0.0f);
    if (a.mask_before_res && t >= out_len) v = 0.0f;
    if (a.res) {
// ... 377 lines not shown
    p.gz = a.B;
    return p;
}

void launch_conv1d_generic(const ConvArgs& a, hipStream_t s) {
    if (a.T <= 0 || a.B <= 0) return;
    const ConvPlan p = conv1d_generic_plan(a);
    LAUNCH_KERNEL(k_conv1d_generic, dim3(p.gx, p.gy, p.gz), dim3(256), p.shmem, s, a);
}

static inline int tile_row_to_co(int epi, int tile, int r, int Cout, int H) {
    if (epi == EPI_GATE) {
        const int c = 32 * (tile >> 1) + r;
        return c < H ? (tile & 1) * H + c : -1;
    }
    const int co = 32 * tile + r;
    return co < Cout ? co : -1;
}
static inline int n_tiles_for(int epi, int Cout, int H) {
    return epi == EPI_GATE ? 2 * ((H + 31) / 32) : (Cout + 31) / 32;
}

size_t mfma_packed_floats(int Cout, int Cin, int K) {
    const int nt_std = (Cout + 31) / 32;
    const int nt_gate = 2 * ((Cout / 2 + 31) / 32);
    const int nt = nt_std > nt_gate ? nt_std : nt_gate;
    return (size_t)nt * K * (Cin / 2) * 64;
}

void pack_conv_weights_mfma_mode(const float* w, int Cout, int Cin, int K, int epi, float* out) {
    const int H = Cout / 2;
    const int nt = n_tiles_for(epi, Cout, H);
    const int cp_n = Cin / 2;
    for (int tile = 0; tile < nt; ++tile)
        for (int k = 0; k < K; ++k)
            for (int cp = 0; cp < cp_n; ++cp)
                for (int l = 0; l < 64; ++l) {
                    const int co = tile_row_to_co(epi, tile, l & 31, Cout, H);
                    const int ci = 2 * cp + (l >> 5);
                    out[(((size_t)tile * K + k) * cp_n + cp) * 64 + l] = co >= 0 ? w[((size_t)co * Cin + ci) * K + k] : 0.0f;
                }
}
void regroup_packed_x4(const float* packed, size_t n_floats, float* out) {
    const size_t recs = n_floats / 64;
    for (size_t r = 0; r < recs; ++r)
        for (int l = 0; l < 64; ++l) out[((r >> 2) * 64 + l) * 4 + (r & 3)] = packed[r * 64 + l];
}
size_t bf16x3_packed_words(int Cout, int Cin, int K) { return (size_t)(Cout / 32) * K * (Cin / 16) * 3 * 64 * 4; }

static inline uint32_t bf16_rne_bits(float f) {
    uint32_t u;
    memcpy(&u, &f, 4);
    if ((u & 0x7fffffffu) > 0x7f800000u) return (u >> 16) | 0x40u;
    u += 0x7fffu + ((u >> 16) & 1u);
    return u >> 16;
}
static inline float bf16_bits_to_float(uint32_t b) {
    const uint32_t u = b << 16;
    float f;
    memcpy(&f, &u, 4);
    return f;
}

static inline int b3_slot_channel(int layout, int half, int e) {
    return layout == 0 ? (e < 4 ? 0 : 8) + half + 2 * (e & 3) : 8 * (e >> 2) + 4 * half + (e & 3);
}

size_t bf16x3_packed_words_mode(int Cout, int Cin, int K, int epi) {
    return (size_t)n_tiles_for(epi, Cout, Cout / 2) * K * (Cin / 16) * 3 * 64 * 4;
}

void pack_conv_weights_bf16x3_mode(const float* w, int Cout, int Cin, int K, int epi, int layout, uint32_t* out) {
    const int ng = Cin / 16, H = Cout / 2;
    const int nt = n_tiles_for(epi, Cout, H);
    for (int tile = 0; tile < nt; ++tile)
        for (int k = 0; k < K; ++k)
            for (int g = 0; g < ng; ++g)
                for (int l = 0; l < 64; ++l) {
                    const int co = tile_row_to_co(epi, tile, l & 31, Cout, H), half = l >> 5;
                    uint32_t plane[3][8];
                    for (int e = 0; e < 8; ++e) {
                        const int ci = 16 * g + b3_slot_channel(layout, half, e);
                        const float v = co >= 0 ? w[((size_t)co * Cin + ci) * K + k] : 0.0f;
                        const uint32_t h = bf16_rne_bits(v);
                        const float r1 = v - bf16_bits_to_float(h);
                        const uint32_t m = bf16_rne_bits(r1);
                        const float r2 = r1 - bf16_bits_to_float(m);
                        plane[0][e] = h; plane[1][e] = m; plane[2][e] = bf16_rne_bits(r2);
                    }
                    for (int p = 0; p < 3; ++p) {
                        uint32_t* o = out + (((((size_t)tile * K + k) * ng + g) * 3 + p) * 64 + l) * 4;
                        for (int j = 0; j < 4; ++j) o[j] = plane[p][2 * j] | (plane[p][2 * j + 1] << 16);
                    }
                }
}

static inline uint32_t f16_rne_bits(float f) {
    uint32_t u;
    memcpy(&u, &f, 4);
    const uint32_t sign = (u >> 16) & 0x8000u, ax = u & 0x7fffffffu;
    if (ax > 0x7f800000u) return sign | 0x7e00u;
    if (ax >= 0x477ff000u) return sign | 0x7c00u;
    const int e = (int)(ax >> 23) - 127;
    if (e < -25) return sign;
    if (e >= -14) {
        uint32_t r = ax + 0xfffu + ((ax >> 13) & 1u);
        return sign | (((r >> 23) - 112) << 10) | ((r >> 13) & 0x3ffu);
    }
    const double v = (double)f < 0 ? -(double)f : (double)f;
    const double q = v * 16777216.0;
    uint32_t n = (uint32_t)q;
    const double frac = q - n;
    if (frac > 0.5 || (frac == 0.5 && (n & 1))) ++n;
    return sign | n;
}
static inline float f16_bits_to_float(uint32_t h) {
    const uint32_t sign = (h & 0x8000u) << 16, e = (h >> 10) & 0x1fu, m = h & 0x3ffu;
    uint32_t u;
    float f;
    if (e == 0) {
        f = (float)m * 5.9604644775390625e-08f;
        memcpy(&u, &f, 4);
        u |= sign;
    } else if (e == 31) {
        u = sign | 0x7f800000u | (m << 13);
    } else {
        u = sign | ((e + 112) << 23) | (m << 13);
    }
    memcpy(&f, &u, 4);
    return f;
}

size_t f16x2_packed_words(int Cout, int Cin, int K) { return (size_t)(Cout / 32) * K * (Cin / 16) * 2 * 64 * 4; }

bool pack_conv_weights_f16x2(const float* w, int Cout, int Cin, int K, uint32_t* out, int layout) {
    const size_t n = (size_t)Cout * Cin * K;
    for (size_t i = 0; i < n; ++i)
        if (!(std::fabs(w[i]) < 7.99f)) return false;
    const int ng = Cin / 16, nt = Cout / 32;
    for (int tile = 0; tile < nt; ++tile)
        for (int k = 0; k < K; ++k)
            for (int g = 0; g < ng; ++g)
                for (int l = 0; l < 64; ++l) {
                    const int co = 32 * tile + (l & 31), half = l >> 5;
                    uint32_t plane[2][8];
                    for (int e = 0; e < 8; ++e) {
                        const int ci = 16 * g + b3_slot_channel(layout, half, e);
                        const float v = w[((size_t)co * Cin + ci) * K + k] * F16X2_W_SCALE;
                        const uint32_t h = f16_rne_bits(v);
                        plane[0][e] = h;
                        plane[1][e] = f16_rne_bits(v - f16_bits_to_float(h));
                    }
                    for (int p = 0; p < 2; ++p) {
                        uint32_t* o = out + (((((size_t)tile * K + k) * ng + g) * 2 + p) * 64 + l) * 4;
                        for (int j = 0; j < 4; ++j) o[j] = plane[p][2 * j] | (plane[p][2 * j + 1] << 16);
                    }
                }
    return true;
}

void pack_conv_weights_bf16x3(const float* w, int Cout, int Cin, int K, uint32_t* out) {
    pack_conv_weights_bf16x3_mode(w, Cout, Cin, K, EPI_STD, 0, out);
}

void pack_conv_weights_mfma(const float* w, int Cout, int Cin, int K, float* out) {
    pack_conv_weights_mfma_mode(w, Cout, Cin, K, EPI_STD, out);
// ... 1681 lines not shown
```

mimic3_amd/csrc/kernels_wn.cpp:

```cpp
#include "kernels.h"
#include "b3.h"

namespace m355 {

template <int CP>
__device__ __forceinline__ void wn_mfma2(f32x16& acc0, f32x16& acc1, const float* __restrict__ wp0,
                                         const float* __restrict__ wp1, const float* __restrict__ xw, int LD, int K, int dil) {
    static_assert(CP % 8 == 0, "channel pairs per tap must be a multiple of 8");
    const int ld2 = 2 * LD;
    float r0[8], r1[8];
    MI355_UNROLL
    for (int u = 0; u < 4; ++u) { r0[u] = wp0[u * 64]; r1[u] = wp1[u * 64]; }
    float bb[2];
    bb[0] = xw[0];
    const float* g0 = wp0;
    const float* g1 = wp1;
    for (int k = 0; k < K; ++k) {
        MI355_UNROLL
        for (int cp0 = 0; cp0 < CP; cp0 += 8) {
            const float* base = xw + k * dil + cp0 * ld2;
            const bool last = (k == K - 1) && (cp0 + 8 == CP);
            const float* nbase = last ? base : ((cp0 + 8 < CP) ? base + 8 * ld2 : xw + (k + 1) * dil);
            const float* h0 = last ? g0 - 8 * 64 : g0;
            const float* h1 = last ? g1 - 8 * 64 : g1;
// ... 305 lines not shown
                a.h_out[(long)b * a.h_bs + (long)(32 * q + (r & 3) + 8 * (r >> 2) + 4 * brow) * a.h_ld + t] = live ? hr[r] + acc[r] : 0.0f;
            return;
        }
        float* sp = a.skip + (long)b * a.s_bs + (long)(32 * q - (two ? H : 0) + 4 * brow) * a.s_ld + t;
        float old[16];
        if (!a.skip_init) {
            MI355_UNROLL
            for (int r = 0; r < 16; ++r) old[r] = sp[(long)((r & 3) + 8 * (r >> 2)) * a.s_ld];
        }
        MI355_UNROLL
        for (int r = 0; r < 16; ++r) sp[(long)((r & 3) + 8 * (r >> 2)) * a.s_ld] = a.skip_init ? acc[r] : old[r] + acc[r];
    };
    if (two) {
        f32x16 acc[MT];
        const float* wp[MT];
        MI355_UNROLL
        for (int m = 0; m < MT; ++m) {
            const int q = MT * w + m;
            MI355_UNROLL
            for (int r = 0; r < 16; ++r) acc[m][r] = a.b_rs[32 * q + (r & 3) + 8 * (r >> 2) + 4 * brow];
            wp[m] = a.w_rs + (long)q * CP * 64 + lane;
        }
        if (!(LAB_ABLATE(a) & 1)) wn_mfma_b4<MT, CP>(acc, wp, U, 32, 1, 0);
        MI355_UNROLL
        for (int m = 0; m < MT; ++m) finish(acc[m], MT * w + m, hres[m]);
    } else if (NW == 12) {
        if (w < 6) {
            f32x16 a1[1];
            const float* w1[1] = {a.w_rs + (long)w * CP * 64 + lane};
            MI355_UNROLL
            for (int r = 0; r < 16; ++r) a1[0][r] = a.b_rs[32 * w + (r & 3) + 8 * (r >> 2) + 4 * brow];
            if (!(LAB_ABLATE(a) & 1)) wn_mfma_b4<1, CP>(a1, w1, U, 32, 1, 0);
            finish(a1[0], w, hres[0]);
        }
    } else {
        const int nq = w < 2 ? 2 : 1;
        f32x16 acc[2];
        const float* wp[2];
        MI355_UNROLL
        for (int m = 0; m < 2; ++m) {
            const int q = m == 0 ? w : w + 4;
            const int qq = q < 6 ? q : w;
            MI355_UNROLL
            for (int r = 0; r < 16; ++r) acc[m][r] = a.b_rs[32 * qq + (r & 3) + 8 * (r >> 2) + 4 * brow];
            wp[m] = a.w_rs + (long)qq * CP * 64 + lane;
        }
        if (!(LAB_ABLATE(a) & 1)) {
            if (nq == 2) {
                wn_mfma_b4<2, CP>(acc, wp, U, 32, 1, 0);
            } else {
                f32x16 a1[1] = {acc[0]};
                const float* w1[1] = {wp[0]};
                wn_mfma_b4<1, CP>(a1, w1, U, 32, 1, 0);
                acc[0] = a1[0];
            }
        }
        finish(acc[0], w, hres[0]);
        if (nq == 2) finish(acc[1], w + 4, hres[0]);
    }
}

constexpr int WNB_H = 192, WNB_NG = WNB_H / 16;
constexpr int WNB_RING = 4;
constexpr int WNB_EPI = 1;
#if defined(MI355_LAB) && !defined(MI355_EMU)
#define WN_TS_DECL() long long wn_ts[7] = {0, 0, 0, 0, 0, 0, 0}
#define WN_TS(i) do { if (a.ablate & 64) wn_ts[i] = __builtin_readcyclecounter(); } while (0)
#define WN_TS_END()                                                                                                                  \
    do {                                                                                                                             \
        if ((a.ablate & 64) && blockIdx.x == 3 && blockIdx.y == 5 && threadIdx.x == 0) {                                            \
            __builtin_amdgcn_s_waitcnt(0);                                                                                           \
            wn_ts[6] = __builtin_readcyclecounter();                                                                                 \
            printf("wn phases (cycles): stage %lld inconv %lld rawstore %lld gate+planes %lld rs %lld epilogue %lld total %lld\n", wn_ts[1] - wn_ts[0], \
                   wn_ts[2] - wn_ts[1], wn_ts[3] - wn_ts[2], wn_ts[4] - wn_ts[3], wn_ts[5] - wn_ts[4], wn_ts[6] - wn_ts[5], wn_ts[6] - wn_ts[0]);   \
        }                                                                                                                            \
    } while (0)
#else
#define WN_TS_DECL() ((void)0)
#define WN_TS(i) ((void)0)
#define WN_TS_END() ((void)0)
#endif


template <bool W1, int NT, bool H2, int RA, int EP>
__device__ __forceinline__ void wn_layer_b3_body(const WnArgs& a) {
    constexpr int MW = 3, NWV = 4, NTH = 256;
    static_assert(!(W1 && H2), "one reduced-operand variant at a time");
    constexpr int H = WNB_H, T_B = 32 * NT, NG = WNB_NG;
    constexpr int NP = H2 ? 2 : 3, GW = H2 ? 128 : 192;
    constexpr float ACC = H2 ? F16X2_ACC_SCALE : 1.0f, UNACC = H2 ? 1.0f / F16X2_ACC_SCALE : 1.0f;
    DYN_SMEM(float, smem);
    uint4* planes = reinterpret_cast<uint4*>(smem);
    const int tid = threadIdx.x, lane = tid & 63, w = WAVE_UNIFORM(tid >> 6);
    const int brow = lane >> 5, bcol = lane & 31;
    const int b = blockIdx.y;
    const int t0 = blockIdx.x * T_B;
    int len = a.len ? a.len[b] : a.T;
    if (len > a.T) len = a.T;
    if (t0 >= len) return;
    const int pad = (a.K - 1) / 2 * a.dil;
    const int tlo = t0 - pad;
    const int ts = tlo >= 0 ? (tlo & ~3) : -(((-tlo) + 3) & ~3);
    const int toff = tlo - ts;
    const int LD = a.ldx;
    WN_TS_DECL();
    WN_TS(0);
    const int PS = NG * 2 * LD;
    const bool two = a.Crs == 2 * H;

    if (!(LAB_ABLATE(a) & 2)) stage_planes<NG, NG, H2>(a.h_in + (long)b * a.h_bs, a.h_ld, LD, ts, len, 1.0f, planes, PS, tid, NTH);
    __syncthreads();
    WN_TS(1);

    const float* condp = a.cond ? a.cond + (long)b * a.cond_bs : a.b_in;
    const float cond_on = a.cond ? 1.0f : 0.0f;
    {
        f32x16 acc[MW][NT];
        const uint4* wp[MW];
        MI355_UNROLL
        for (int i = 0; i < MW; ++i) {
            const int q = w + NWV * i;
            MI355_UNROLL
            for (int r = 0; r < 16; ++r) {
                const int c = (r < 8 ? 0 : H) + 16 * q + (r & 3) + 8 * ((r >> 2) & 1) + 4 * brow;
                const float v = (a.b_in[c] + cond_on * condp[c]) * ACC;
                MI355_UNROLL
                for (int j = 0; j < NT; ++j) acc[i][j][r] = v;
            }
            wp[i] = reinterpret_cast<const uint4*>(a.w_in) + (long)q * a.K * NG * GW + lane;
        }
        if (!(LAB_ABLATE(a) & 1)) {
            if constexpr (H2) h2_chunk<MW, NT, NG, NT>(acc, wp, planes + brow * LD + bcol + toff, PS, LD, a.K, NG, a.dil);
            else if constexpr (RA > 2 && NT >= 4) b3_chunk_lean_ra<MW, NT, NG, W1, RA>(acc, wp, planes + brow * LD + bcol + toff, PS, LD, a.K, NG, a.dil);
            else if constexpr (RA > 2) b3_chunk_ra<MW, NT, NG, NT, W1, RA>(acc, wp, planes + brow * LD + bcol + toff, PS, LD, a.K, NG, a.dil);
            else b3_chunk<MW, NT, NG, NT, W1>(acc, wp, planes + brow * LD + bcol + toff, PS, LD, a.K, NG, a.dil);
        }
        __syncthreads();
        WN_TS(2);
        WN_TS(3);
        constexpr int PSU0 = NG * 2 * T_B;
        MI355_UNROLL
        for (int i = 0; i < MW; ++i)
            MI355_UNROLL
            for (int j = 0; j < NT; ++j) {
                float u[8];
                MI355_UNROLL
                for (int e = 0; e < 8; ++e) u[e] = wn_gate_f(acc[i][j][e] * UNACC, acc[i][j][e + 8] * UNACC);
                const int idx = (2 * (w + NWV * i) + brow) * T_B + 32 * j + bcol;
                if constexpr (H2) {
                    uint4 h4, m4;
                    split2_pk(u[0] * F16X2_X_SCALE, u[1] * F16X2_X_SCALE, h4.x, m4.x);
                    split2_pk(u[2] * F16X2_X_SCALE, u[3] * F16X2_X_SCALE, h4.y, m4.y);
                    split2_pk(u[4] * F16X2_X_SCALE, u[5] * F16X2_X_SCALE, h4.z, m4.z);
                    split2_pk(u[6] * F16X2_X_SCALE, u[7] * F16X2_X_SCALE, h4.w, m4.w);
                    planes[idx] = h4;
                    planes[PSU0 + idx] = m4;
                } else {
                    uint4 h4, m4, l4;
                    split3_pk(u[0], u[1], h4.x, m4.x, l4.x);
                    split3_pk(u[2], u[3], h4.y, m4.y, l4.y);
                    split3_pk(u[4], u[5], h4.z, m4.z, l4.z);
                    split3_pk(u[6], u[7], h4.w, m4.w, l4.w);
                    planes[idx] = h4;
                    planes[PSU0 + idx] = m4;
                    planes[2 * PSU0 + idx] = l4;
                }
            }
    }
    const int ntr = a.Crs / 32;
    const float* src[MW];
    float* dst[MW];
    long ldr[MW];
    bool valid[MW], use_old[MW], to_h[MW];
    MI355_UNROLL
    for (int i = 0; i < MW; ++i) {
        const int q = w + NWV * i;
        valid[i] = q < ntr;
        const int qc = valid[i] ? q : ntr - 1;
        to_h[i] = two && 32 * qc < H;
        if (to_h[i]) {
            src[i] = a.h_in + (long)b * a.h_bs + (long)(32 * qc) * a.h_ld;
            dst[i] = a.h_out + (long)b * a.h_bs + (long)(32 * qc) * a.h_ld;
            ldr[i] = a.h_ld;
            use_old[i] = true;
        } else {
            const int sub = two ? H : 0;
            src[i] = a.skip + (long)b * a.s_bs + (long)(32 * qc - sub) * a.s_ld;
            dst[i] = a.skip + (long)b * a.s_bs + (long)(32 * qc - sub) * a.s_ld;
            ldr[i] = a.s_ld;
            use_old[i] = !a.skip_init;
        }
    }
    auto load_tile = [&](int i, int j, float (&old)[16]) {
        const int t = t0 + j * 32 + bcol;
        const int tc = t < a.T ? t : a.T - 1;
        if (valid[i] && use_old[i]) {
            MI355_UNROLL
            for (int r = 0; r < 16; ++r) old[r] = src[i][(long)((r & 3) + 8 * (r >> 2) + 4 * brow) * ldr[i] + tc];
        } else {
            MI355_UNROLL
            for (int r = 0; r < 16; ++r) old[r] = 0.0f;
        }
    };
    constexpr int EPA = EP == 0 ? 1 : 3, EPR = EPA + 1;
    float old[EPR][16];
    auto load_tile_b = [&](int i, int j, float (&o)[16]) MI355_INLINE_LAMBDA {
        const int t = t0 + j * 32 + bcol;
        const int tc = t < a.T ? t : a.T - 1;
        const BufRsrc rs = buf_rsrc(src[i]);
        const unsigned row4 = 4u * (unsigned)ldr[i];
        const unsigned vo = (valid[i] && use_old[i]) ? (unsigned)(4 * brow) * row4 + 4u * (unsigned)tc : BUF_OOB;
        MI355_UNROLL
        for (int r = 0; r < 16; ++r) o[r] = buf_load_f32(rs, vo, (unsigned)((r & 3) + 8 * (r >> 2)) * row4);
    };
    constexpr int PSU = NG * 2 * T_B;
    __syncthreads();
    WN_TS(4);
    f32x16 acc[MW][NT];
    {
        const uint4* wp[MW];
        MI355_UNROLL
        for (int i = 0; i < MW; ++i) {
            int q = w + NWV * i;
            if (q >= ntr) q = ntr - 1;
            MI355_UNROLL
            for (int r = 0; r < 16; ++r) {
                const float v = a.b_rs[32 * q + (r & 3) + 8 * (r >> 2) + 4 * brow] * ACC;
                MI355_UNROLL
                for (int j = 0; j < NT; ++j) acc[i][j][r] = v;
            }
            wp[i] = reinterpret_cast<const uint4*>(a.w_rs) + (long)q * NG * GW + lane;
        }
        if (!(LAB_ABLATE(a) & 1)) {
            if (two) {
                if constexpr (H2) h2_chunk<MW, NT, NG, NT>(acc, wp, planes + brow * T_B + bcol, PSU, T_B, 1, NG, 0);
                else if constexpr (RA > 2 && NT >= 4) b3_chunk_lean_ra<MW, NT, NG, W1, RA>(acc, wp, planes + brow * T_B + bcol, PSU, T_B, 1, NG, 0);
                else if constexpr (RA > 2) b3_chunk_ra<MW, NT, NG, NT, W1, RA>(acc, wp, planes + brow * T_B + bcol, PSU, T_B, 1, NG, 0);
                else b3_chunk<MW, NT, NG, NT, W1>(acc, wp, planes + brow * T_B + bcol, PSU, T_B, 1, NG, 0);
            } else {
                f32x16 a2[2][NT];
                const uint4* w2[2] = {wp[0], wp[1]};
                MI355_UNROLL
                for (int i = 0; i < 2; ++i)
                    MI355_UNROLL
                    for (int j = 0; j < NT; ++j) a2[i][j] = acc[i][j];
                if constexpr (H2) h2_chunk<2, NT, NG, NT>(a2, w2, planes + brow * T_B + bcol, PSU, T_B, 1, NG, 0);
                else b3_chunk<2, NT, NG, NT, W1>(a2, w2, planes + brow * T_B + bcol, PSU, T_B, 1, NG, 0);
                MI355_UNROLL
                for (int i = 0; i < 2; ++i)
                    MI355_UNROLL
                    for (int j = 0; j < NT; ++j) acc[i][j] = a2[i][j];
            }
        }
        if constexpr (H2) {
            MI355_UNROLL
            for (int i = 0; i < MW; ++i)
                MI355_UNROLL
                for (int j = 0; j < NT; ++j)
                    MI355_UNROLL
                    for (int r = 0; r < 16; ++r) acc[i][j][r] *= UNACC;
        }
    }
    WN_TS(5);
    if ((LAB_ABLATE(a) & 4) && acc[0][0][0] != 1.2345f) return;
    auto store_tile = [&](int i, int j, const float (&old)[16]) {
        const int t = t0 + j * 32 + bcol;
        if (!valid[i] || t >= a.T) return;
        const bool live = t < len || !to_h[i];
        MI355_UNROLL
        for (int r = 0; r < 16; ++r) dst[i][(long)((r & 3) + 8 * (r >> 2) + 4 * brow) * ldr[i] + t] = live ? old[r] + acc[i][j][r] : 0.0f;
    };
    if constexpr (EP == 0) {
        load_tile(0, 0, old[0]);
        MI355_UNROLL
        for (int k = 0; k < MW * NT; ++k) {
            if (k + 1 < MW * NT) load_tile((k + 1) / NT, (k + 1) % NT, old[(k + 1) & 1]);
            SCHED_FENCE();
            store_tile(k / NT, k % NT, old[k & 1]);
            SCHED_FENCE();
        }
    } else {
        auto store_tile_b = [&](int i, int j, const float (&o)[16]) MI355_INLINE_LAMBDA {
            const int t = t0 + j * 32 + bcol;
            const bool live = t < len || !to_h[i];
            const BufRsrc rs = buf_rsrc(dst[i]);
            const unsigned row4 = 4u * (unsigned)ldr[i];
            const unsigned vo = (valid[i] && t < a.T) ? (unsigned)(4 * brow) * row4 + 4u * (unsigned)t : BUF_OOB;
            MI355_UNROLL
            for (int r = 0; r < 16; ++r) buf_store_f32(rs, vo, (unsigned)((r & 3) + 8 * (r >> 2)) * row4, live ? o[r] + acc[i][j][r] : 0.0f);
        };
        MI355_UNROLL
        for (int k = 0; k < EPA && k < MW * NT; ++k) load_tile_b(k / NT, k % NT, old[k]);
        MI355_UNROLL
        for (int k = 0; k < MW * NT; ++k) {
            if (k + EPA < MW * NT) load_tile_b((k + EPA) / NT, (k + EPA) % NT, old[(k + EPA) % EPR]);
            SCHED_FENCE();
            store_tile_b(k / NT, k % NT, old[k % EPR]);
            SCHED_FENCE();
        }
    }
    WN_TS_END();
}

template <bool W1, int NT, bool H2 = false, int RA = 2, int EP = 0>
__global__ __launch_bounds__(256) void k_wn_layer_b3(WnArgs a) {
    wn_layer_b3_body<W1, NT, H2, RA, EP>(a);
}

bool wn_layer_b3_supported(int H, int K, int dil) {
    return H == WNB_H && (K % 2) == 1 && K >= 1 && dil >= 1 && (K - 1) * dil <= 24;
}

int wn_layer_b3_column_tiles(const WnArgs& a) {
    const char* nt_s = lab_getenv("MI355VITS_WN_B3_NT");
    const long nwg3 = (long)((a.T + 95) / 96) * a.B;
    int nt = nt_s ? atoi(nt_s) : (nwg3 < 128 ? 1 : 3);
    if (!nt_s && nt == 3 && a.math != MATH_F16X2) {
        const long cus = current_device_cu_count();
        const long nwg4 = (long)((a.T + 127) / 128) * a.B;
        if ((double)((nwg4 + cus - 1) / cus) * 1.28 < (double)((nwg3 + cus - 1) / cus)) nt = 4;
    }
    if (nt == 4 && (a.math == MATH_F16X2 || ((long)a.h_ld * 128 >= 0x7fffffffL || (long)a.s_ld * 128 >= 0x7fffffffL || (a.K - 1) * a.dil > 8))) nt = 3;
    return nt;
}

void launch_wn_layer_b3(WnArgs a, hipStream_t s) {
    if (a.T <= 0 || a.B <= 0) return;
    if (!wn_layer_b3_supported(a.H, a.K, a.dil)) throw std::runtime_error("wn_layer_b3: unsupported shape");
    static const int ablate = lab_getenv("MI355VITS_WN_ABLATE") ? atoi(lab_getenv("MI355VITS_WN_ABLATE")) : 0;
    a.ablate = ablate;
    a.vec = (a.h_ld % 4 == 0) && (a.h_bs % 4 == 0) && (reinterpret_cast<uintptr_t>(a.h_in) % 16 == 0);
    const int nt = wn_layer_b3_column_tiles(a);
    const int tb = 32 * nt;
    a.ldx = (tb + (a.K - 1) * a.dil + 3 + 3) & ~3;
    const size_t shmem = (size_t)3 * WNB_NG * 2 * a.ldx * 16;
    dim3 grid((a.T + tb - 1) / tb, a.B);
    auto go = [&](auto kfn) {
#ifndef MI355_EMU
        set_max_dynamic_lds(reinterpret_cast<const void*>(kfn), 160 * 1024);
#endif
        LAUNCH_KERNEL(kfn, grid, dim3(256), shmem, s, a);
    };
    if (nt == 4 && a.math != MATH_F16X2) {
        if (a.math == MATH_BF16W) go(k_wn_layer_b3<true, 4, false, WNB_RING, 1>);
        else go(k_wn_layer_b3<false, 4, false, WNB_RING, 1>);
    } else if (nt == 1) {
        if (a.math == MATH_F16X2) go(k_wn_layer_b3<false, 1, true>);
        else if (a.math == MATH_BF16W) go(k_wn_layer_b3<true, 1>);
        else go(k_wn_layer_b3<false, 1>);
    } else {
        int epi = WNB_EPI;
        if (const char* f = lab_getenv("MI355VITS_WN_EPI")) epi = atoi(f);
        if ((long)a.h_ld * 128 >= 0x7fffffffL || (long)a.s_ld * 128 >= 0x7fffffffL) epi = 0;
        if (a.math == MATH_F16X2) go(k_wn_layer_b3<false, 3, true>);
        else if (a.math == MATH_BF16W) go(k_wn_layer_b3<true, 3>);
        else if (epi == 1) go(k_wn_layer_b3<false, 3, false, WNB_RING, 1>);
        else go(k_wn_layer_b3<false, 3, false, WNB_RING>);
    }
}

bool wn_layer_fused_supported(int H, int K, int dil) {
    return (H == 32 || H == 192) && (K % 2) == 1 && K >= 1 && dil >= 1 && (size_t)H * (32 + (K - 1) * dil + 8) * 4 <= 48 * 1024;
}

int wn_layer_geometry(const WnArgs& a) {
    const char* six_s = lab_getenv("MI355VITS_WN_SIX_WAVES");
    const int six_env = six_s ? atoi(six_s) : -1;
    const long nwg = (long)((a.T + 31) / 32) * a.B;
    return six_env >= 0 ? six_env : (nwg < 128 ? 2 : (nwg < 512 ? 1 : 0));
}

void launch_wn_layer(WnArgs a, hipStream_t s) {
    if (a.T <= 0 || a.B <= 0) return;
    if (!wn_layer_fused_supported(a.H, a.K, a.dil)) throw std::runtime_error("wn_layer: unsupported shape");
    a.ldx = (32 + (a.K - 1) * a.dil + 3 + 3) & ~3;
    static const int ablate = lab_getenv("MI355VITS_WN_ABLATE") ? atoi(lab_getenv("MI355VITS_WN_ABLATE")) : 0;
    a.ablate = ablate;
    a.vec = (a.h_ld % 4 == 0) && (a.h_bs % 4 == 0) && (reinterpret_cast<uintptr_t>(a.h_in) % 16 == 0);
    const size_t shmem = (size_t)a.H * a.ldx * sizeof(float);
    dim3 grid((a.T + 31) / 32, a.B);
    const int geom = wn_layer_geometry(a);
    const size_t sh4 = (size_t)a.H * (a.ldx > 64 ? a.ldx : 64) * sizeof(float);
    if (a.H == 192 && geom == 0) {
        LAUNCH_KERNEL(k_wn_layer_h192<4>, grid, dim3(256), sh4, s, a);
    } else if (a.H == 192 && geom == 2) {
        LAUNCH_KERNEL(k_wn_layer_h192<12>, grid, dim3(768), sh4, s, a);
    } else if (a.H == 192) {
        auto k = k_wn_layer<6>;
        LAUNCH_KERNEL(k, grid, dim3(384), shmem, s, a);
    } else {
        auto k = k_wn_layer<1>;
        LAUNCH_KERNEL(k, grid, dim3(64), shmem, s, a);
    }
}

}
```

mimic3_amd/csrc/lab_api.cpp:

```cpp
#include "c_api_internal.h"
#include "mi355vits_lab.h"

extern "C" {

int mi355vits_probe_weights(mi355vits_handle h, double out[8]) {
    if (!h || !out) return MI355VITS_ERR_INVALID;
    std::lock_guard<std::mutex> lk(h->eng->mu);
    return guarded(h, [&] { h->eng->probe_weights(out); });
}

}

namespace {
const float* const ALIGNED = reinterpret_cast<const float*>(uintptr_t(4096));

struct ConvHookOpts { bool bias, res, cond, in_len, out_len, relu, res_sub, accumulate, mask_before_res; float out_scale; };

ConvArgs conv_hook_args(int impl, int B, int Cin, int Cout, int T, int K, int dil, int math, int fixed_rule, const ConvHookOpts& o) {
    if (impl < 0 || impl > 4) throw EngineError(MI355VITS_ERR_INVALID, "impl must be 0 .. 4");
    if (B < 1 || Cin < 1 || Cout < 1 || T < 1 || K < 1 || dil < 1) throw EngineError(MI355VITS_ERR_INVALID, "bad shape");
    if ((size_t)B * std::max(Cin, Cout) * T >= 0x7fffffffull / 4) throw EngineError(MI355VITS_ERR_INVALID, "tensor too large for the hook");
    const bool ok_math = impl <= 1 ? math == MATH_F32 : impl == 4 ? math == MATH_BF16X3 : (math == MATH_BF16X3 || math == MATH_BF16W);
    if (!ok_math) throw EngineError(MI355VITS_ERR_INVALID, "math mode: MATH_F32 for impl 0 and 1, MATH_BF16X3 or MATH_BF16W for impl 2 and 3, MATH_BF16X3 for impl 4");
    if (fixed_rule && impl != 1 && impl != 2) throw EngineError(MI355VITS_ERR_INVALID, "fixed_rule: impl 1 and 2 only");
// ... 711 lines not shown
            launch_rel_attention_stream(dq.as<float>(), dk.as<float>(), dv.as<float>(), dl.as<int>(), B, T, H, n_heads, W, dout.as<float>(), nullptr);
        HIP_CHECK(hipDeviceSynchronize());
        HIP_CHECK(hipGetLastError());
        HIP_CHECK(hipMemcpy(out, dout.p, no * 4, hipMemcpyDeviceToHost));
    });
}

int mi355vits_test_wn_layer(int device, const mi355vits_wn_test* t) {
    return guarded(nullptr, [&] {
        if (!t || !t->h_in || !t->w_in || !t->b_in || !t->w_rs || !t->b_rs || !t->len || !t->h_out || !t->skip) throw EngineError(MI355VITS_ERR_INVALID, "null argument");
        const int B = t->B, H = t->H, T = t->T, K = t->K, dil = t->dilation, Crs = t->Crs;
        if (B < 1 || H < 1 || T < 1 || K < 1 || (K % 2) == 0 || dil < 1 || (Crs != H && Crs != 2 * H)) throw EngineError(MI355VITS_ERR_INVALID, "bad shape");
        if ((long)B * H * T >= 0x7fffffffL / 4) throw EngineError(MI355VITS_ERR_INVALID, "tensor too large for the hook");
        for (int b = 0; b < B; ++b)
            if (t->len[b] < 0 || t->len[b] > T) throw EngineError(MI355VITS_ERR_INVALID, "len out of range");
        if (t->impl < 0 || t->impl > 2) throw EngineError(MI355VITS_ERR_INVALID, "impl must be 0, 1 or 2");
        if (t->impl == 2 ? t->math != MATH_BF16X3 : t->math != MATH_F32) throw EngineError(MI355VITS_ERR_INVALID, "math mode: MATH_F32 for impl 0 and 1, MATH_BF16X3 for impl 2");
        if (t->impl == 1 && !wn_layer_fused_supported(H, K, dil)) throw EngineError(MI355VITS_ERR_INVALID, "shape not supported by the fused f32 layer");
        if (t->impl == 2 && !wn_layer_b3_supported(H, K, dil)) throw EngineError(MI355VITS_ERR_INVALID, "shape not supported by the fused split-bf16 layer");
        HIP_CHECK(hipSetDevice(device));
        const size_t n = (size_t)B * H * T;
        const std::vector<float> w_in(t->w_in, t->w_in + (size_t)2 * H * H * K), w_rs(t->w_rs, t->w_rs + (size_t)Crs * H);
        DevBuf dh(n * 4), dho(n * 4), dsk(n * 4), du(n * 4), dbi((size_t)2 * H * 4), dbr((size_t)Crs * 4), dc((size_t)B * 2 * H * 4), dl((size_t)B * 4);
        HIP_CHECK(hipMemcpy(dh.p, t->h_in, n * 4, hipMemcpyHostToDevice));
        HIP_CHECK(hipMemcpy(dho.p, t->h_out, n * 4, hipMemcpyHostToDevice));
        HIP_CHECK(hipMemcpy(dsk.p, t->skip, n * 4, hipMemcpyHostToDevice));
        HIP_CHECK(hipMemcpy(dbi.p, t->b_in, (size_t)2 * H * 4, hipMemcpyHostToDevice));
        HIP_CHECK(hipMemcpy(dbr.p, t->b_rs, (size_t)Crs * 4, hipMemcpyHostToDevice));
        HIP_CHECK(hipMemcpy(dl.p, t->len, (size_t)B * 4, hipMemcpyHostToDevice));
        if (t->cond) HIP_CHECK(hipMemcpy(dc.p, t->cond, (size_t)B * 2 * H * 4, hipMemcpyHostToDevice));
        const long hbs = (long)H * T;
        auto upload = [](const void* p, size_t bytes) {
            std::unique_ptr<DevBuf> d(new DevBuf(bytes));
            HIP_CHECK(hipMemcpy(d->p, p, bytes, hipMemcpyHostToDevice));
            return d;
        };
        std::unique_ptr<DevBuf> dwi, dwr;
        const float* h_result = dho.as<float>();
        if (t->impl == 0) {
            const bool mfma_in = conv1d_mfma_supported(H, 2 * H, K, 1), mfma_rs = conv1d_mfma_supported(H, Crs, 1, 1);
            if (mfma_in) {
                std::vector<float> pi(mfma_packed_floats(2 * H, H, K), 0.0f);
                pack_conv_weights_mfma_mode(w_in.data(), 2 * H, H, K, EPI_GATE, pi.data());
                dwi = upload(pi.data(), pi.size() * 4);
            } else {
                dwi = upload(w_in.data(), w_in.size() * 4);
            }
            if (mfma_rs) {
                std::vector<float> pr(mfma_packed_floats(Crs, H, 1), 0.0f);
                pack_conv_weights_mfma_mode(w_rs.data(), Crs, H, 1, EPI_STD, pr.data());
                dwr = upload(pr.data(), pr.size() * 4);
            } else {
                dwr = upload(w_rs.data(), w_rs.size() * 4);
            }
            ConvArgs in;
            in.x = dh.as<float>(); in.x_bs = hbs; in.x_ld = T;
            in.y = du.as<float>(); in.y_bs = hbs; in.y_ld = T;
            in.epi = EPI_GATE; in.H = H; in.dil = dil;
            if (t->cond) { in.cond = dc.as<float>(); in.cond_bs = 2L * H; }
            in.B = B; in.T = T;
            in.fixed_rule = 1; in.Cin = H; in.Cout = 2 * H; in.K = K; in.bias = dbi.as<float>(); in.pad = (K * dil - dil) / 2;
            in.w = dwi->as<float>(); in.math = MATH_F32;
            ConvArgs rs;
            rs.x = du.as<float>(); rs.x_bs = hbs; rs.x_ld = T;
            rs.y = dh.as<float>(); rs.y_bs = hbs; rs.y_ld = T;
            rs.y2 = dsk.as<float>(); rs.y2_bs = hbs; rs.y2_ld = T;
            rs.epi = EPI_RESSKIP; rs.H = H; rs.skip_init = t->skip_init != 0;
            rs.out_len = dl.as<int>();
            rs.B = B; rs.T = T;
            rs.fixed_rule = 1; rs.Cin = H; rs.Cout = Crs; rs.K = 1; rs.bias = dbr.as<float>(); rs.pad = 0;
            rs.w = dwr->as<float>(); rs.math = MATH_F32;
            if (mfma_in) launch_conv1d_mfma(in, nullptr);
            else launch_conv1d_generic(in, nullptr);
            if (mfma_rs) launch_conv1d_mfma(rs, nullptr);
            else launch_conv1d_generic(rs, nullptr);
            h_result = dh.as<float>();
        } else {
            if (t->impl == 1) {
                std::vector<float> pi(mfma_packed_floats(2 * H, H, K), 0.0f), pr(mfma_packed_floats(Crs, H, 1), 0.0f);
                pack_conv_weights_mfma_mode(w_in.data(), 2 * H, H, K, EPI_GATE, pi.data());
                pack_conv_weights_mfma_mode(w_rs.data(), Crs, H, 1, EPI_STD, pr.data());
                dwi = upload(pi.data(), pi.size() * 4);
                dwr = upload(pr.data(), pr.size() * 4);
            } else {
                const size_t row = (size_t)H * K;
                std::vector<float> wg(w_in.size());
                for (int q = 0; q < 2 * H / 32; ++q)
                    for (int r = 0; r < 32; ++r) {
                        const int src = (r < 16 ? 0 : H) + 16 * q + (r & 15);
                        memcpy(wg.data() + ((size_t)32 * q + r) * row, w_in.data() + (size_t)src * row, row * sizeof(float));
                    }
                std::vector<uint32_t> bi(bf16x3_packed_words_mode(2 * H, H, K, EPI_STD)), br(bf16x3_packed_words_mode(Crs, H, 1, EPI_STD));
                pack_conv_weights_bf16x3_mode(wg.data(), 2 * H, H, K, EPI_STD, 1, bi.data());
                pack_conv_weights_bf16x3_mode(w_rs.data(), Crs, H, 1, EPI_STD, 1, br.data());
                dwi = upload(bi.data(), bi.size() * 4);
                dwr = upload(br.data(), br.size() * 4);
            }
            WnArgs w;
            w.h_in = dh.as<float>(); w.h_out = dho.as<float>(); w.h_bs = hbs; w.h_ld = T;
            w.skip = dsk.as<float>(); w.s_bs = hbs; w.s_ld = T;
            w.w_in = dwi->as<float>(); w.b_in = dbi.as<float>();
            w.w_rs = dwr->as<float>(); w.b_rs = dbr.as<float>();
            if (t->cond) { w.cond = dc.as<float>(); w.cond_bs = 2L * H; }
            w.len = dl.as<int>();
            w.B = B; w.H = H; w.T = T; w.K = K; w.dil = dil; w.Crs = Crs; w.skip_init = t->skip_init != 0;
            if (t->impl == 2) { w.math = MATH_BF16X3; launch_wn_layer_b3(w, nullptr); }
            else launch_wn_layer(w, nullptr);
        }
        HIP_CHECK(hipDeviceSynchronize());
        HIP_CHECK(hipGetLastError());
        if (t->impl != 0 || Crs == 2 * H) HIP_CHECK(hipMemcpy(t->h_out, h_result, n * 4, hipMemcpyDeviceToHost));
        HIP_CHECK(hipMemcpy(t->skip, dsk.p, n * 4, hipMemcpyDeviceToHost));
    });
}

int mi355vits_test_dds_stack(int device, const mi355vits_dds_stack_test* t) {
    return guarded(nullptr, [&] {
        if (!t || !t->src || !t->pre_w || !t->pre_b || !t->len || !t->x_out) throw EngineError(MI355VITS_ERR_INVALID, "null argument");
        const int B = t->B, C = t->C, T = t->T, K = t->K, NL = t->n_layers, PC = t->proj_w ? t->proj_cout : 0;
        if (B < 1 || C < 1 || T < 1 || K < 1 || (K % 2) == 0 || NL < 1 || NL > DDS_STACK_MAX_LAYERS) throw EngineError(MI355VITS_ERR_INVALID, "bad shape");
        if ((long)B * C * T >= 0x7fffffffL / 4) throw EngineError(MI355VITS_ERR_INVALID, "tensor too large for the hook");
        if (t->pre_mode != DDS_PRE_CONV && t->pre_mode != DDS_PRE_AFFINE) throw EngineError(MI355VITS_ERR_INVALID, "pre_mode must be 0 or 1");
        if (t->zch != 0 && t->zch != 1) throw EngineError(MI355VITS_ERR_INVALID, "zch must be 0 or 1");
        for (int i = 0; i < NL; ++i)
            if (!t->dw_w[i] || !t->dw_b[i] || !t->g1[i] || !t->b1[i] || !t->w1x1[i] || !t->bias1x1[i] || !t->g2[i] || !t->b2[i])
                throw EngineError(MI355VITS_ERR_INVALID, "null layer argument");
        if (t->proj_w && (!t->proj_b || !t->out || PC < 1)) throw EngineError(MI355VITS_ERR_INVALID, "proj needs proj_b, out and proj_cout >= 1");
        if (t->pre_mode == DDS_PRE_AFFINE && !t->z) throw EngineError(MI355VITS_ERR_INVALID, "the affine pre needs z");
        if (t->pre_mode == DDS_PRE_AFFINE && t->cond) throw EngineError(MI355VITS_ERR_INVALID, "cond goes with the conv pre only");
        if (t->spline && (!t->proj_w || !t->z)) throw EngineError(MI355VITS_ERR_INVALID, "the spline needs proj and z");
        if (t->spline && (t->nb < 2 || t->nb > 16)) throw EngineError(MI355VITS_ERR_INVALID, "spline: 2 <= nb <= 16");
        if (t->spline && PC != 3 * t->nb - 1) throw EngineError(MI355VITS_ERR_INVALID, "spline: proj_cout must be 3 nb - 1");
        for (int b = 0; b < B; ++b)
            if (t->len[b] < 0 || t->len[b] > T) throw EngineError(MI355VITS_ERR_INVALID, "len out of range");
        if (t->impl < 0 || t->impl > 3) throw EngineError(MI355VITS_ERR_INVALID, "impl must be 0, 1, 2 or 3");
        if (t->impl == 3 ? !math_on_bf16(t->math) : t->math != MATH_F32)
            throw EngineError(MI355VITS_ERR_INVALID, "math mode: MATH_F32 for impl 0, 1 and 2, MATH_BF16X3 or MATH_BF16W for impl 3");
        if (t->impl == 1 && !dds_layer_fused_supported(C)) throw EngineError(MI355VITS_ERR_INVALID, "shape not supported by the fused DDS layer");
        if (t->impl >= 2 && !dds_stack_supported(C, K, NL, PC)) throw EngineError(MI355VITS_ERR_INVALID, "shape not supported by the DDS stack kernels");
        HIP_CHECK(hipSetDevice(device));
        const size_t n = (size_t)B * C * T, nz = (size_t)B * 2 * T, no = (size_t)B * PC * T;
        auto upload = [](const void* p, size_t bytes) {
            std::unique_ptr<DevBuf> d(new DevBuf(bytes));
            if (bytes) HIP_CHECK(hipMemcpy(d->p, p, bytes, hipMemcpyHostToDevice));
            return d;
        };
        std::vector<std::unique_ptr<DevBuf>> keep;
        auto vecf = [&](const float* p, size_t count) -> const float* {
            keep.push_back(upload(p, count * 4));
            return keep.back()->as<float>();
        };
        const bool b3 = t->impl == 3;
        auto conv_mfma = [&](int Cout) { return conv1d_mfma_supported(C, Cout, 1, 1); };
        auto dense = [&](const float* w, int Cout) -> const float* {
            if (b3) {
                std::vector<uint32_t> p(bf16x3_packed_words_mode(Cout, C, 1, EPI_STD), 0u);
                pack_conv_weights_bf16x3_mode(w, Cout, C, 1, EPI_STD, 1, p.data());
                keep.push_back(upload(p.data(), p.size() * 4));
            } else if (t->impl != 0 || conv_mfma(Cout)) {
                std::vector<float> p(mfma_packed_floats(Cout, C, 1), 0.0f);
                pack_conv_weights_mfma_mode(w, Cout, C, 1, EPI_STD, p.data());
                keep.push_back(upload(p.data(), p.size() * 4));
            } else {
                keep.push_back(upload(w, (size_t)Cout * C * 4));
            }
            return keep.back()->as<float>();
        };
        DevBuf dsrc(n * 4), dxo(n * 4), dz(nz * 4), dout(no * 4), dl((size_t)B * 4), dcond((size_t)B * C * 4);
        HIP_CHECK(hipMemcpy(dsrc.p, t->src, n * 4, hipMemcpyHostToDevice));
        HIP_CHECK(hipMemcpy(dxo.p, t->x_out, n * 4, hipMemcpyHostToDevice));
        HIP_CHECK(hipMemcpy(dl.p, t->len, (size_t)B * 4, hipMemcpyHostToDevice));
        if (t->z) HIP_CHECK(hipMemcpy(dz.p, t->z, nz * 4, hipMemcpyHostToDevice));
        if (PC) HIP_CHECK(hipMemcpy(dout.p, t->out, no * 4, hipMemcpyHostToDevice));
        if (t->cond) HIP_CHECK(hipMemcpy(dcond.p, t->cond, (size_t)B * C * 4, hipMemcpyHostToDevice));
        const float* pre_w = t->pre_mode == DDS_PRE_AFFINE ? vecf(t->pre_w, C) : dense(t->pre_w, C);
        const float* pre_b = vecf(t->pre_b, C);
        const float *dw_w[DDS_STACK_MAX_LAYERS], *dw_b[DDS_STACK_MAX_LAYERS], *g1[DDS_STACK_MAX_LAYERS], *b1[DDS_STACK_MAX_LAYERS];
        const float *w1[DDS_STACK_MAX_LAYERS], *bb[DDS_STACK_MAX_LAYERS], *g2[DDS_STACK_MAX_LAYERS], *b2[DDS_STACK_MAX_LAYERS];
        for (int i = 0; i < NL; ++i) {
            dw_w[i] = vecf(t->dw_w[i], (size_t)C * K); dw_b[i] = vecf(t->dw_b[i], C);
            g1[i] = vecf(t->g1[i], C); b1[i] = vecf(t->b1[i], C);
            w1[i] = dense(t->w1x1[i], C); bb[i] = vecf(t->bias1x1[i], C);
            g2[i] = vecf(t->g2[i], C); b2[i] = vecf(t->b2[i], C);
        }
        const float* proj_w = PC ? dense(t->proj_w, PC) : nullptr;
        const float* proj_b = PC ? vecf(t->proj_b, PC) : nullptr;
        if (t->impl >= 2) {
            DdsStackArgs a;
            a.src = dsrc.as<float>(); a.pre_mode = t->pre_mode; a.pre_w = pre_w; a.pre_b = pre_b;
// ... 308 lines not shown
        if (ratio) HIP_CHECK(hipMemcpy(dr.p, ratio, nbt * 4, hipMemcpyHostToDevice));
        launch_pitch_plan(dc.as<int>(), dl.as<int>(), ratio ? dr.as<float>() : nullptr, B, T, hop, dq.as<long long>(), dw.as<int>(), dn.as<int>(), nullptr);
        HIP_CHECK(hipDeviceSynchronize());
        HIP_CHECK(hipGetLastError());
        HIP_CHECK(hipMemcpy(tq, dq.p, nbt * 8, hipMemcpyDeviceToHost));
        HIP_CHECK(hipMemcpy(wc, dw.p, nbt * 4, hipMemcpyDeviceToHost));
        HIP_CHECK(hipMemcpy(wlen, dn.p, (size_t)B * 4, hipMemcpyDeviceToHost));
    });
}

int mi355vits_test_pitch(int device, int B, int T, int hop, const int32_t* cum, const int32_t* len, const float* ratio,
                         const float* x, int64_t x_bs, size_t x_floats, float* y, int64_t y_bs, int32_t y_ld, size_t y_floats,
                         float* peaks, int32_t* wlen) {
    return guarded(nullptr, [&] {
        if (!x || !y || !peaks || !wlen) throw EngineError(MI355VITS_ERR_INVALID, "null argument");
        if (x_bs < 1 || y_bs < 1 || y_ld < 1 || y_ld > y_bs || B < 1 || x_floats < (size_t)B * (size_t)x_bs || y_floats < (size_t)B * (size_t)y_bs)
            throw EngineError(MI355VITS_ERR_INVALID, "bad shape");
        check_pitch_inputs(B, T, hop, cum, len, ratio, x_bs);
        HIP_CHECK(hipSetDevice(device));
        const size_t nbt = (size_t)B * T;
        const std::vector<float>& h = pitch_table();
        std::vector<int> alen(B);
        for (int b = 0; b < B; ++b) {
            const int frames = len[b] > 0 ? cum[(size_t)b * T + len[b] - 1] : 0;
            alen[b] = hop * (frames < 1 ? 1 : frames);
        }
        DevBuf dc(nbt * 4), dl((size_t)B * 4), dr(nbt * 4), dq(nbt * 8), dw(nbt * 4), dn((size_t)B * 4), da((size_t)B * 4),
            dx(x_floats * 4), dy(y_floats * 4), dp((size_t)B * 4), dh(h.size() * 4);
        HIP_CHECK(hipMemcpy(dc.p, cum, nbt * 4, hipMemcpyHostToDevice));
        HIP_CHECK(hipMemcpy(dl.p, len, (size_t)B * 4, hipMemcpyHostToDevice));
        if (ratio) HIP_CHECK(hipMemcpy(dr.p, ratio, nbt * 4, hipMemcpyHostToDevice));
        HIP_CHECK(hipMemcpy(da.p, alen.data(), (size_t)B * 4, hipMemcpyHostToDevice));
        HIP_CHECK(hipMemcpy(dx.p, x, x_floats * 4, hipMemcpyHostToDevice));
        HIP_CHECK(hipMemcpy(dy.p, y, y_floats * 4, hipMemcpyHostToDevice));
        HIP_CHECK(hipMemcpy(dh.p, h.data(), h.size() * 4, hipMemcpyHostToDevice));
        HIP_CHECK(hipMemset(dp.p, 0, (size_t)B * 4));
        const float* dratio = ratio ? dr.as<float>() : nullptr;
        launch_pitch_plan(dc.as<int>(), dl.as<int>(), dratio, B, T, hop, dq.as<long long>(), dw.as<int>(), dn.as<int>(), nullptr);
        HIP_CHECK(hipDeviceSynchronize());
        HIP_CHECK(hipMemcpy(wlen, dn.p, (size_t)B * 4, hipMemcpyDeviceToHost));
        for (int b = 0; b < B; ++b)
            if (wlen[b] < 1 || wlen[b] == 0x7fffffff || wlen[b] > y_ld) throw EngineError(MI355VITS_ERR_INVALID, "row " + std::to_string(b) + ": the warped row of " + std::to_string(wlen[b]) + " samples does not fit y_ld");
        std::vector<int64_t> w64(wlen, wlen + B);
        std::vector<int> tab(pitch_tab_ints(B));
        const long items = pitch_fill_tab(w64.data(), B, tab.data());
        DevBuf dt(tab.size() * 4);
        HIP_CHECK(hipMemcpy(dt.p, tab.data(), tab.size() * 4, hipMemcpyHostToDevice));
        launch_pitch(dx.as<float>(), (long)x_bs, da.as<int>(), dc.as<int>(), dl.as<int>(), dratio, dq.as<long long>(), dw.as<int>(), dt.as<int>(),
                     items, dh.as<float>(), B, T, hop, dy.as<float>(), (long)y_bs, y_ld, dp.as<unsigned>(), nullptr);
        HIP_CHECK(hipDeviceSynchronize());
        HIP_CHECK(hipGetLastError());
        HIP_CHECK(hipMemcpy(y, dy.p, y_floats * 4, hipMemcpyDeviceToHost));
        HIP_CHECK(hipMemcpy(peaks, dp.p, (size_t)B * 4, hipMemcpyDeviceToHost));
    });
}

int mi355vits_test_expand_prior(int device, int B, int I, int Tx, int Ty, const float* stats, const int32_t* cum, const int32_t* ylen,
                                const float* injected, int injected_frames, const float* scales, float* z) {
    return guarded(nullptr, [&] {
        if (!stats || !cum || !ylen || !scales || !z) throw EngineError(MI355VITS_ERR_INVALID, "null argument");
        if (B < 1 || I < 1 || Tx < 1 || Ty < 1) throw EngineError(MI355VITS_ERR_INVALID, "bad shape");
        if (injected && injected_frames < Ty) throw EngineError(MI355VITS_ERR_INVALID, "injected_frames must cover Ty");
        for (int b = 0; b < B; ++b) {
            if (ylen[b] < 0 || ylen[b] > Ty) throw EngineError(MI355VITS_ERR_INVALID, "ylen out of range");
            if (!injected && scales[3 * b] != 0.0f) throw EngineError(MI355VITS_ERR_INVALID, "noise_scale != 0 needs injected noise (no Philox path here)");
            for (int j = 0; j < Tx; ++j)
                if (cum[(size_t)b * Tx + j] < (j ? cum[(size_t)b * Tx + j - 1] : 0)) throw EngineError(MI355VITS_ERR_INVALID, "cum must be non-negative and non-decreasing");
        }
        HIP_CHECK(hipSetDevice(device));
        const size_t ns = (size_t)B * 2 * I * Tx, nc = (size_t)B * Tx, ni = injected ? (size_t)B * I * injected_frames : 0, nz = (size_t)B * I * Ty;
        DevBuf dst(ns * 4), dc(nc * 4), dy((size_t)B * 4), di(ni * 4), ds((size_t)B * 3 * 4), dz(nz * 4), du((size_t)B * 8);
        HIP_CHECK(hipMemcpy(dst.p, stats, ns * 4, hipMemcpyHostToDevice));
        HIP_CHECK(hipMemcpy(dc.p, cum, nc * 4, hipMemcpyHostToDevice));
        HIP_CHECK(hipMemcpy(dy.p, ylen, (size_t)B * 4, hipMemcpyHostToDevice));
        if (ni) HIP_CHECK(hipMemcpy(di.p, injected, ni * 4, hipMemcpyHostToDevice));
        HIP_CHECK(hipMemcpy(ds.p, scales, (size_t)B * 3 * 4, hipMemcpyHostToDevice));
        HIP_CHECK(hipMemcpy(dz.p, z, nz * 4, hipMemcpyHostToDevice));
        HIP_CHECK(hipMemset(du.p, 0, (size_t)B * 8));
        launch_expand_prior(dst.as<float>(), dc.as<int>(), dy.as<int>(), injected ? di.as<float>() : nullptr, injected_frames, B, I, Tx, Ty,
                            ds.as<float>(), 0ull, du.as<unsigned long long>(), dz.as<float>(), nullptr);
        HIP_CHECK(hipDeviceSynchronize());
        HIP_CHECK(hipGetLastError());
        HIP_CHECK(hipMemcpy(z, dz.p, nz * 4, hipMemcpyDeviceToHost));
    });
}

int mi355vits_lab_wn_plan(int B, int T, int K, int dilation, int32_t* b3_tile, int32_t* f32_geometry) {
    return guarded(nullptr, [&] {
        if (B < 1 || T < 1 || K < 1 || (K % 2) == 0 || dilation < 1) throw EngineError(MI355VITS_ERR_INVALID, "bad shape");
        WnArgs w;
        w.B = B; w.H = 192; w.T = T; w.K = K; w.dil = dilation; w.h_ld = w.s_ld = T; w.math = MATH_BF16X3;
        if (b3_tile) {
            if (!wn_layer_b3_supported(w.H, K, dilation)) throw EngineError(MI355VITS_ERR_INVALID, "shape not supported by the fused split-bf16 layer");
            *b3_tile = 32 * wn_layer_b3_column_tiles(w);
        }
        if (f32_geometry) *f32_geometry = wn_layer_geometry(w);
    });
}

static bool mrf_test_plan(int impl, int C, int nrb, const int32_t* k, const int32_t* d1, const int32_t* d2, MrfPlan* p) {
    if (nrb < 1 || nrb > MRF_MAX_RB || !k || !d1 || !d2) return false;
    int kk[MRF_MAX_RB], a1[MRF_MAX_RB], a2[MRF_MAX_RB];
    for (int j = 0; j < nrb; ++j) { kk[j] = k[j]; a1[j] = d1[j]; a2[j] = d2[j]; }
    return impl == 0 ? mrf_fused_plan(C, nrb, kk, a1, a2, p) : impl == 1 ? mrf_p_plan(C, nrb, kk, a1, a2, p) : impl == 2 ? mrf_s_plan(C, nrb, kk, a1, a2, p) : false;
}

int mi355vits_test_mrf_stage(int device, const mi355vits_mrf_test* t) {
    return guarded(nullptr, [&] {
        if (!t || !t->x || !t->len || !t->y) throw EngineError(MI355VITS_ERR_INVALID, "null argument");
        const int B = t->B, C = t->C, T = t->T, nrb = t->nrb;
        if (B < 1 || C < 1 || T < 1 || nrb < 1 || nrb > MRF_MAX_RB || !(t->out_scale >= 0.0f)) throw EngineError(MI355VITS_ERR_INVALID, "bad shape");
        if ((long)C * T * 4 >= 0x7fffffffL || (long)B * C * T >= 0x7fffffffL / 4) throw EngineError(MI355VITS_ERR_INVALID, "tensor too large for the hook");
        for (int j = 0; j < nrb; ++j)
            for (int q = 0; q < 2; ++q)
                if (!t->w[j][q] || !t->bias[j][q]) throw EngineError(MI355VITS_ERR_INVALID, "null weight or bias");
        for (int b = 0; b < B; ++b)
            if (t->len[b] < 0 || t->len[b] > T) throw EngineError(MI355VITS_ERR_INVALID, "len out of range");
        if (t->impl < 0 || t->impl > 2) throw EngineError(MI355VITS_ERR_INVALID, "impl must be 0, 1 or 2");
        if (t->impl == 0 ? (t->math != MATH_F32 && t->math != MATH_BF16X3) : t->math != MATH_BF16X3)
            throw EngineError(MI355VITS_ERR_INVALID, "math mode: MATH_F32 or MATH_BF16X3 for impl 0, MATH_BF16X3 for impl 1 and 2");
        MrfPlan plan;
        if (!mrf_test_plan(t->impl, C, nrb, t->k, t->d1, t->d2, &plan)) throw EngineError(MI355VITS_ERR_INVALID, "stage not supported by the chosen kernel");
        if (t->impl == 2 && (t->seg < plan.width || t->seg % plan.width != 0)) throw EngineError(MI355VITS_ERR_INVALID, "seg must be a positive multiple of the sweep's step");
        HIP_CHECK(hipSetDevice(device));
        const size_t n = (size_t)B * C * T;
        DevBuf dx(n * 4), dy(n * 4), dl((size_t)B * 4);
        HIP_CHECK(hipMemcpy(dx.p, t->x, n * 4, hipMemcpyHostToDevice));
        HIP_CHECK(hipMemcpy(dy.p, t->y, n * 4, hipMemcpyHostToDevice));
        HIP_CHECK(hipMemcpy(dl.p, t->len, (size_t)B * 4, hipMemcpyHostToDevice));
        std::vector<int> len_host(t->len, t->len + B);
        std::vector<std::unique_ptr<DevBuf>> keep;
        auto upload = [&](const void* p, size_t bytes) {
            keep.emplace_back(new DevBuf(bytes));
            HIP_CHECK(hipMemcpy(keep.back()->p, p, bytes, hipMemcpyHostToDevice));
            return keep.back()->as<float>();
        };
        MrfArgs m;
        m.x = dx.as<float>(); m.x_bs = (long)C * T; m.x_ld = T;
        m.y = dy.as<float>(); m.y_bs = (long)C * T; m.y_ld = T;
        m.len = dl.as<int>(); m.len_host = len_host.data(); m.B = B; m.C = C; m.T = T;
        m.nrb = nrb; m.math = t->math; m.out_scale = t->out_scale;
        for (int j = 0; j < nrb; ++j) {
            const int k = t->k[j];
            m.k[j] = k; m.d1[j] = t->d1[j]; m.d2[j] = t->d2[j];
            for (int q = 0; q < 2; ++q) {
                const float* w = t->w[j][q];
                if (t->impl != 0) {
                    std::vector<uint32_t> pp(p16_packed_words(C, C, k));
                    pack_conv_weights_p16(w, C, C, k, pp.data());
                    m.w[j][q] = upload(pp.data(), pp.size() * 4);
                } else if (t->math == MATH_BF16X3) {
                    std::vector<uint32_t> b3(bf16x3_packed_words(C, C, k));
                    pack_conv_weights_bf16x3(w, C, C, k, b3.data());
                    m.w[j][q] = upload(b3.data(), b3.size() * 4);
                } else {
                    std::vector<float> pk(mfma_packed_floats(C, C, k), 0.0f), p4(pk.size());
                    pack_conv_weights_mfma_mode(w, C, C, k, EPI_STD, pk.data());
                    regroup_packed_x4(pk.data(), pk.size(), p4.data());
                    m.w[j][q] = upload(p4.data(), p4.size() * 4);
                }
                m.bias[j][q] = upload(t->bias[j][q], (size_t)C * 4);
            }
        }
        if (t->impl == 0) launch_mrf_fused(m, nullptr);
        else if (t->impl == 1) launch_mrf_p(m, nullptr);
        else { m.seg = t->seg; launch_mrf_s(m, nullptr); }
// ... 155 lines not shown
```

Baseline: 795.5 million.

## Run fused WaveNet flow layer on 16x16x32 bf16 MFMA with new weight packing

```diff
diff --git a/include/mi355vits_lab.h b/include/mi355vits_lab.h
--- a/include/mi355vits_lab.h
+++ b/include/mi355vits_lab.h
@@ -70,6 +70,7 @@
 } mi355vits_wn_test;
 int mi355vits_test_wn_layer(int device, const mi355vits_wn_test* t);
 int mi355vits_lab_wn_plan(int B, int T, int K, int dilation, int32_t* b3_tile, int32_t* f32_geometry);
+int mi355vits_lab_pack_w16(const float* w, int Cout, int Cin, int K, int gate, uint32_t* out);
 typedef struct mi355vits_mrf_test {
     int32_t impl, B, C, T, nrb, math, seg;
     int32_t k[4], d1[4], d2[4];
diff --git a/mimic3_amd/_native.py b/mimic3_amd/_native.py
--- a/mimic3_amd/_native.py
+++ b/mimic3_amd/_native.py
@@ -44,7 +44,7 @@
     "mi355vits_lab_g711_encode", "mi355vits_test_alignment", "mi355vits_lab_edges",
     "mi355vits_lab_loudness", "mi355vits_lab_loudness_plan", "mi355vits_lab_limit",
     "mi355vits_lab_limit_env", "mi355vits_lab_true_peak", "mi355vits_lab_true_peak_plan", "mi355vits_lab_flac", "mi355vits_lab_flac_jobs",
-    "mi355vits_test_wn_layer", "mi355vits_lab_wn_plan", "mi355vits_test_mrf_stage", "mi355vits_lab_mrf_plan",
+    "mi355vits_test_wn_layer", "mi355vits_lab_wn_plan", "mi355vits_lab_pack_w16", "mi355vits_test_mrf_stage", "mi355vits_lab_mrf_plan",
     "mi355vits_test_dds_stack", "mi355vits_test_spline_inverse", "mi355vits_test_durations", "mi355vits_test_expand_prior",
     "mi355vits_test_fit_durations", "mi355vits_test_speaker_cond", "mi355vits_test_speaker_cond_mix", "mi355vits_test_levels",
     "mi355vits_test_pitch_table", "mi355vits_test_pitch_plan", "mi355vits_test_pitch",
@@ -611,6 +611,7 @@
                 ctypes.POINTER(ctypes.c_int32), ctypes.POINTER(ctypes.c_float)]
             L.mi355vits_test_wn_layer.argtypes = [ctypes.c_int, ctypes.POINTER(WnTest)]
             L.mi355vits_lab_wn_plan.argtypes = [ctypes.c_int] * 4 + [i32p, i32p]
+            L.mi355vits_lab_pack_w16.argtypes = [f32p] + [ctypes.c_int] * 4 + [ctypes.POINTER(ctypes.c_uint32)]
             L.mi355vits_test_mrf_stage.argtypes = [ctypes.c_int, ctypes.POINTER(MrfTest)]
             L.mi355vits_lab_mrf_plan.argtypes = [ctypes.c_int] * 3 + [i32p] * 7
             L.mi355vits_lab_conv_plan.argtypes = [ctypes.c_int] * 12 + [i32p, ctypes.POINTER(ConvPlan)]
@@ -940,6 +941,16 @@
         if rc != 0:
             raise NativeError(rc, self.create_error())
         return int(tile.value), int(geom.value)
+
+    def lab_pack_w16(self, w, gate=False):
+        self._need_hooks()
+        w = np.ascontiguousarray(w, np.float32)
+        Cout, Cin, K = w.shape
+        out = np.zeros((Cout // 16, K, Cin // 32, 3, 64, 4), np.uint32)
+        rc = self.lib.mi355vits_lab_pack_w16(_fptr(w), Cout, Cin, K, int(bool(gate)), out.ctypes.data_as(ctypes.POINTER(ctypes.c_uint32)))
+        if rc != 0:
+            raise NativeError(rc, self.create_error())
+        return out.view(np.uint16).reshape(Cout // 16, K, Cin // 32, 3, 64, 8)
 
     def test_mrf_stage(self, x, ks, d1, d2, weights, biases, lengths, impl=0, math=None, out_scale=0.0, seg=0, y_prior=None, device=0):
         self._need_hooks()
diff --git a/mimic3_amd/csrc/b3.h b/mimic3_amd/csrc/b3.h
--- a/mimic3_amd/csrc/b3.h
+++ b/mimic3_amd/csrc/b3.h
@@ -313,6 +313,69 @@
                 SCHED_FENCE();
                 MI355_UNROLL
                 for (int p = 0; p < 2; ++p) rb[j][p] = xq[p * PS + xoff + j * 32];
+                SCHED_FENCE();
+            }
+        }
+    }
+}
+
+template <int MT, int NC, int NG , bool W1>
+__device__ __forceinline__ void b3_chunk16(f32x4 (&acc)[MT][NC], const uint4* const (&wp)[MT], const uint4* __restrict__ xq, int PS, int LD, int K,
+                                           int dil) {
+    static_assert(NG % 2 == 0 && NC % 2 == 0, "the ring positions are the same in every tap / step");
+    uint4 ra[2][MT][3];
+    uint4 rb[2][3];
+    const int drop = b3_drop();
+    constexpr int NPA = W1 ? 1 : 3;
+    MI355_UNROLL
+    for (int i = 0; i < MT; ++i)
+        MI355_UNROLL
+        for (int p = 0; p < NPA; ++p) ra[0][i][p] = wp[i][p * 64];
+    MI355_UNROLL
+    for (int p = 0; p < 3; ++p) rb[0][p] = xq[p * PS];
+    for (int k = 0; k < K; ++k) {
+        const bool last_tap = k == K - 1;
+        MI355_UNROLL
+        for (int g = 0; g < NG; ++g) {
+            const int cur = g & 1, nxt = cur ^ 1;
+            const bool wrap = g + 1 == NG;
+            const long woff = (wrap ? (last_tap ? (long)k * NG + g : (long)(k + 1) * NG) : (long)k * NG + g + 1) * 192;
+            const int xcur = k * dil + g * 4 * LD;
+            const int xnxt = wrap ? (last_tap ? xcur : (k + 1) * dil) : xcur + 4 * LD;
+            MI355_UNROLL
+            for (int i = 0; i < MT; ++i)
+                MI355_UNROLL
+                for (int p = 0; p < NPA; ++p) ra[nxt][i][p] = wp[i][woff + p * 64];
+            SCHED_FENCE();
+            MI355_UNROLL
+            for (int c = 0; c < NC; ++c) {
+                const int bc = c & 1;
+                const int xo = c + 1 < NC ? xcur + 16 * (c + 1) : xnxt;
+                MI355_UNROLL
+                for (int p = 0; p < 3; ++p) rb[bc ^ 1][p] = xq[p * PS + xo];
+                SCHED_FENCE();
+                if constexpr (!W1) {
+                    if (drop != 1) {
+                        MI355_UNROLL
+                        for (int i = 0; i < MT; ++i) acc[i][c] = MFMA_16x16x32_BF16(ra[cur][i][2], rb[bc][0], acc[i][c]);
+                    }
+                }
+                if (drop != 2) {
+                    MI355_UNROLL
+                    for (int i = 0; i < MT; ++i) acc[i][c] = MFMA_16x16x32_BF16(ra[cur][i][0], rb[bc][2], acc[i][c]);
+                }
+                if constexpr (!W1) {
+                    if (drop != 3) {
+                        MI355_UNROLL
+                        for (int i = 0; i < MT; ++i) acc[i][c] = MFMA_16x16x32_BF16(ra[cur][i][1], rb[bc][1], acc[i][c]);
+                    }
+                    MI355_UNROLL
+                    for (int i = 0; i < MT; ++i) acc[i][c] = MFMA_16x16x32_BF16(ra[cur][i][1], rb[bc][0], acc[i][c]);
+                }
+                MI355_UNROLL
+                for (int i = 0; i < MT; ++i) acc[i][c] = MFMA_16x16x32_BF16(ra[cur][i][0], rb[bc][1], acc[i][c]);
+                MI355_UNROLL
+                for (int i = 0; i < MT; ++i) acc[i][c] = MFMA_16x16x32_BF16(ra[cur][i][0], rb[bc][0], acc[i][c]);
                 SCHED_FENCE();
             }
         }
diff --git a/mimic3_amd/csrc/engine.cpp b/mimic3_amd/csrc/engine.cpp
--- a/mimic3_amd/csrc/engine.cpp
+++ b/mimic3_amd/csrc/engine.cpp
@@ -250,9 +250,19 @@
                         const int src = (r < 16 ? 0 : Hh) + 16 * q + (r & 15);
                         memcpy(wg.data() + ((size_t)32 * q + r) * row, w.data() + (size_t)src * row, row * sizeof(float));
                     }
+#if defined(MI355_LAB) || defined(MI355_EMU)
                 std::vector<uint32_t> bw(bf16x3_packed_words_mode(Cout, Cin, K, EPI_STD));
                 pack_conv_weights_bf16x3_mode(wg.data(), Cout, Cin, K, EPI_STD, 1, bw.data());
                 c.packed_b3w = stage(reinterpret_cast<const float*>(bw.data()), bw.size());
+#endif
+            }
+            const bool wn_conv = key.compare(0, 5, "flow.") == 0 && (epi == EPI_GATE ? key.find(".in.") != std::string::npos && Cout == 2 * Cin
+                                                                                     : key.find(".rs.") != std::string::npos && K == 1 && epi == EPI_STD &&
+                                                                                           (Cout == Cin || Cout == 2 * Cin));
+            if (wn_conv && wn_layer_b3_supported(Cin, 1, 1)) {
+                std::vector<uint32_t> pw(w16_packed_words(Cout, Cin, K));
+                pack_conv_weights_w16(w.data(), Cout, Cin, K, epi == EPI_GATE, pw.data());
+                c.packed_w16 = stage(reinterpret_cast<const float*>(pw.data()), pw.size());
             }
             if (Cin % 16 == 0 && Cout % 32 == 0) {
                 std::vector<uint32_t> h2(f16x2_packed_words(Cout, Cin, K));
@@ -1176,15 +1186,18 @@
         const bool wn_b3 = sw_.wn_b3 && math_on_bf16(kmath()) && win.packed_b3s != NO_OFF && wrs.packed_b3s != NO_OFF &&
                            conv1d_b3_supported(win.Cin, win.Cout, win.K, dil, Ty) && !sw_.force_generic;
         const bool fused = !sw_.force_generic && !sw_.no_fused_wn && !wn_b3;
-        const bool b3 = fused && math_on_bf16(kmath()) && win.packed_b3w != NO_OFF && wrs.packed_b3s != NO_OFF &&
-                        wn_layer_b3_supported(H, win.K, dil);
+        const int wn_shape = wn_layer_b3_shape();
+        const bool b3 = fused && math_on_bf16(kmath()) && wn_layer_b3_supported(H, win.K, dil) &&
+                        (wn_shape == 32 ? win.packed_b3w != NO_OFF && wrs.packed_b3s != NO_OFF : win.packed_w16 != NO_OFF && wrs.packed_w16 != NO_OFF);
         if (b3 || (fused && wn_layer_fused_supported(H, win.K, dil))) {
             const bool h2 = b3 && math_ == MATH_F16X2 && win.packed_h2s != NO_OFF && wrs.packed_h2s != NO_OFF;
             WnArgs w;
             w.h_in = hcur; w.h_out = hnext; w.h_bs = hbs; w.h_ld = Ty;
             w.skip = d_fskip_; w.s_bs = hbs; w.s_ld = Ty;
-            w.w_in = P(h2 ? win.packed_h2s : (b3 ? win.packed_b3w : win.packed)); w.b_in = P(win.bias);
-            w.w_rs = P(h2 ? wrs.packed_h2s : (b3 ? wrs.packed_b3s : wrs.packed)); w.b_rs = P(wrs.bias);
+            const bool s16 = b3 && !h2 && wn_shape != 32;
+            w.w_in = P(h2 ? win.packed_h2s : (s16 ? win.packed_w16 : (b3 ? win.packed_b3w : win.packed))); w.b_in = P(win.bias);
+            w.w_rs = P(h2 ? wrs.packed_h2s : (s16 ? wrs.packed_w16 : (b3 ? wrs.packed_b3s : wrs.packed))); w.b_rs = P(wrs.bias);
+            w.shape = s16 ? 16 : 32;
             w.cond = cond_l; w.cond_bs = 2L * H * c.flow_wn_layers;
             w.len = d_ylen_;
             w.B = B; w.H = H; w.T = Ty; w.K = win.K; w.dil = dil; w.Crs = wrs.Cout; w.skip_init = (l == 0);
diff --git a/mimic3_amd/csrc/engine.h b/mimic3_amd/csrc/engine.h
--- a/mimic3_amd/csrc/engine.h
+++ b/mimic3_amd/csrc/engine.h
@@ -94,6 +94,7 @@
     size_t packed4 = NO_OFF;
     size_t packed_b3 = NO_OFF;
     size_t packed_b3s = NO_OFF;
+    size_t packed_w16 = NO_OFF;
     size_t packed_b3w = NO_OFF;
     size_t packed_h2 = NO_OFF;
     size_t packed_p = NO_OFF;
diff --git a/mimic3_amd/csrc/kernels.h b/mimic3_amd/csrc/kernels.h
--- a/mimic3_amd/csrc/kernels.h
+++ b/mimic3_amd/csrc/kernels.h
@@ -183,11 +183,15 @@
     int ldx = 0, vec = 0;
     int ablate = 0;
     int math = 0;
+    int shape = 16;
 };
 bool wn_layer_fused_supported(int H, int K, int dil);
 void launch_wn_layer(WnArgs a, hipStream_t s);
 bool wn_layer_b3_supported(int H, int K, int dil);
 void launch_wn_layer_b3(WnArgs a, hipStream_t s);
+int wn_layer_b3_shape();
+size_t w16_packed_words(int Cout, int Cin, int K);
+void pack_conv_weights_w16(const float* w, int Cout, int Cin, int K, bool gate, uint32_t* out);
 int wn_layer_b3_column_tiles(const WnArgs& a);
 int wn_layer_geometry(const WnArgs& a);
 
diff --git a/mimic3_amd/csrc/kernels_conv.cpp b/mimic3_amd/csrc/kernels_conv.cpp
--- a/mimic3_amd/csrc/kernels_conv.cpp
+++ b/mimic3_amd/csrc/kernels_conv.cpp
@@ -483,6 +483,33 @@
                     for (int e = 0; e < 8; ++e) {
                         const int ci = 16 * g + b3_slot_channel(layout, half, e);
                         const float v = co >= 0 ? w[((size_t)co * Cin + ci) * K + k] : 0.0f;
+                        const uint32_t h = bf16_rne_bits(v);
+                        const float r1 = v - bf16_bits_to_float(h);
+                        const uint32_t m = bf16_rne_bits(r1);
+                        const float r2 = r1 - bf16_bits_to_float(m);
+                        plane[0][e] = h; plane[1][e] = m; plane[2][e] = bf16_rne_bits(r2);
+                    }
+                    for (int p = 0; p < 3; ++p) {
+                        uint32_t* o = out + (((((size_t)tile * K + k) * ng + g) * 3 + p) * 64 + l) * 4;
+                        for (int j = 0; j < 4; ++j) o[j] = plane[p][2 * j] | (plane[p][2 * j + 1] << 16);
+                    }
+                }
+}
+
+size_t w16_packed_words(int Cout, int Cin, int K) { return (size_t)(Cout / 16) * K * (Cin / 32) * 3 * 64 * 4; }
+
+void pack_conv_weights_w16(const float* w, int Cout, int Cin, int K, bool gate, uint32_t* out) {
+    const int ng = Cin / 32, H = Cout / 2;
+    for (int tile = 0; tile < Cout / 16; ++tile)
+        for (int k = 0; k < K; ++k)
+            for (int g = 0; g < ng; ++g)
+                for (int l = 0; l < 64; ++l) {
+                    const int n = gate ? tile >> 1 : tile, row = l & 15, kq = l >> 4;
+                    const int co = (gate && (tile & 1) ? H : 0) + 32 * (n >> 1) + 8 * (row >> 2) + 4 * (n & 1) + (row & 3);
+                    uint32_t plane[3][8];
+                    for (int e = 0; e < 8; ++e) {
+                        const int ci = 32 * g + 16 * (kq >> 1) + b3_slot_channel(1, kq & 1, e);
+                        const float v = w[((size_t)co * Cin + ci) * K + k];
                         const uint32_t h = bf16_rne_bits(v);
                         const float r1 = v - bf16_bits_to_float(h);
                         const uint32_t m = bf16_rne_bits(r1);
diff --git a/mimic3_amd/csrc/kernels_wn.cpp b/mimic3_amd/csrc/kernels_wn.cpp
--- a/mimic3_amd/csrc/kernels_wn.cpp
+++ b/mimic3_amd/csrc/kernels_wn.cpp
@@ -411,71 +411,41 @@
 #endif
 
 
-template <bool W1, int NT, bool H2, int RA, int EP>
-__device__ __forceinline__ void wn_layer_b3_body(const WnArgs& a) {
-    constexpr int MW = 3, NWV = 4, NTH = 256;
-    static_assert(!(W1 && H2), "one reduced-operand variant at a time");
-    constexpr int H = WNB_H, T_B = 32 * NT, NG = WNB_NG;
-    constexpr int NP = H2 ? 2 : 3, GW = H2 ? 128 : 192;
-    constexpr float ACC = H2 ? F16X2_ACC_SCALE : 1.0f, UNACC = H2 ? 1.0f / F16X2_ACC_SCALE : 1.0f;
-    DYN_SMEM(float, smem);
-    uint4* planes = reinterpret_cast<uint4*>(smem);
-    const int tid = threadIdx.x, lane = tid & 63, w = WAVE_UNIFORM(tid >> 6);
-    const int brow = lane >> 5, bcol = lane & 31;
-    const int b = blockIdx.y;
-    const int t0 = blockIdx.x * T_B;
-    int len = a.len ? a.len[b] : a.T;
-    if (len > a.T) len = a.T;
-    if (t0 >= len) return;
-    const int pad = (a.K - 1) / 2 * a.dil;
-    const int tlo = t0 - pad;
-    const int ts = tlo >= 0 ? (tlo & ~3) : -(((-tlo) + 3) & ~3);
-    const int toff = tlo - ts;
-    const int LD = a.ldx;
-    WN_TS_DECL();
-    WN_TS(0);
-    const int PS = NG * 2 * LD;
-    const bool two = a.Crs == 2 * H;
-
-    if (!(LAB_ABLATE(a) & 2)) stage_planes<NG, NG, H2>(a.h_in + (long)b * a.h_bs, a.h_ld, LD, ts, len, 1.0f, planes, PS, tid, NTH);
-    __syncthreads();
-    WN_TS(1);
-
-    const float* condp = a.cond ? a.cond + (long)b * a.cond_bs : a.b_in;
-    const float cond_on = a.cond ? 1.0f : 0.0f;
-    {
-        f32x16 acc[MW][NT];
-        const uint4* wp[MW];
-        MI355_UNROLL
-        for (int i = 0; i < MW; ++i) {
-            const int q = w + NWV * i;
-            MI355_UNROLL
-            for (int r = 0; r < 16; ++r) {
-                const int c = (r < 8 ? 0 : H) + 16 * q + (r & 3) + 8 * ((r >> 2) & 1) + 4 * brow;
-                const float v = (a.b_in[c] + cond_on * condp[c]) * ACC;
-                MI355_UNROLL
-                for (int j = 0; j < NT; ++j) acc[i][j][r] = v;
-            }
-            wp[i] = reinterpret_cast<const uint4*>(a.w_in) + (long)q * a.K * NG * GW + lane;
-        }
-        if (!(LAB_ABLATE(a) & 1)) {
-            if constexpr (H2) h2_chunk<MW, NT, NG, NT>(acc, wp, planes + brow * LD + bcol + toff, PS, LD, a.K, NG, a.dil);
-            else if constexpr (RA > 2 && NT >= 4) b3_chunk_lean_ra<MW, NT, NG, W1, RA>(acc, wp, planes + brow * LD + bcol + toff, PS, LD, a.K, NG, a.dil);
-            else if constexpr (RA > 2) b3_chunk_ra<MW, NT, NG, NT, W1, RA>(acc, wp, planes + brow * LD + bcol + toff, PS, LD, a.K, NG, a.dil);
-            else b3_chunk<MW, NT, NG, NT, W1>(acc, wp, planes + brow * LD + bcol + toff, PS, LD, a.K, NG, a.dil);
-        }
-        __syncthreads();
-        WN_TS(2);
-        WN_TS(3);
-        constexpr int PSU0 = NG * 2 * T_B;
+template <int S> struct WnTiles;
+
+template <> struct WnTiles<32> {
+    typedef f32x16 Acc;
+    static constexpr int NR = 16, CW = 32, ROWS = 32, MW = 3, MW_LAST = 2;
+    static __device__ __forceinline__ int col(int lane) { return lane & 31; }
+    static __device__ __forceinline__ int krec(int lane) { return lane >> 5; }
+    static __device__ __forceinline__ int lane_row(int lane) { return 4 * (lane >> 5); }
+    static __device__ __forceinline__ int reg_row(int r) { return (r & 3) + 8 * (r >> 2); }
+    static __device__ __forceinline__ int tile_row0(int q) { return 32 * q; }
+    static __device__ __forceinline__ int gate_tile(int w, int i) { return w + 4 * i; }
+    static __device__ __forceinline__ int gate_row(int H, int w, int i, int r, int lane) {
+        return (r < 8 ? 0 : H) + 16 * (w + 4 * i) + (r & 3) + 8 * ((r >> 2) & 1) + 4 * (lane >> 5);
+    }
+    template <int MT, int NC, bool W1, bool H2, int RA, bool LAST>
+    static __device__ __forceinline__ void conv(Acc (&acc)[MT][NC], const uint4* const (&wp)[MT], const uint4* xq, int PS, int LD, int K, int dil) {
+        constexpr int NG = WNB_NG;
+        if constexpr (H2) h2_chunk<MT, NC, NG, NC>(acc, wp, xq, PS, LD, K, NG, dil);
+        else if constexpr (LAST) b3_chunk<MT, NC, NG, NC, W1>(acc, wp, xq, PS, LD, K, NG, dil);
+        else if constexpr (RA > 2 && NC >= 4) b3_chunk_lean_ra<MT, NC, NG, W1, RA>(acc, wp, xq, PS, LD, K, NG, dil);
+        else if constexpr (RA > 2) b3_chunk_ra<MT, NC, NG, NC, W1, RA>(acc, wp, xq, PS, LD, K, NG, dil);
+        else b3_chunk<MT, NC, NG, NC, W1>(acc, wp, xq, PS, LD, K, NG, dil);
+    }
+    template <int NC, bool H2>
+    static __device__ __forceinline__ void gate_store(const Acc (&acc)[MW][NC], uint4* planes, int w, int lane, float UNACC) {
+        constexpr int T_B = 32 * NC, PSU0 = WNB_NG * 2 * T_B;
+        const int brow = lane >> 5, bcol = lane & 31;
         MI355_UNROLL
         for (int i = 0; i < MW; ++i)
             MI355_UNROLL
-            for (int j = 0; j < NT; ++j) {
+            for (int j = 0; j < NC; ++j) {
                 float u[8];
                 MI355_UNROLL
                 for (int e = 0; e < 8; ++e) u[e] = wn_gate_f(acc[i][j][e] * UNACC, acc[i][j][e + 8] * UNACC);
-                const int idx = (2 * (w + NWV * i) + brow) * T_B + 32 * j + bcol;
+                const int idx = (2 * (w + 4 * i) + brow) * T_B + 32 * j + bcol;
                 if constexpr (H2) {
                     uint4 h4, m4;
                     split2_pk(u[0] * F16X2_X_SCALE, u[1] * F16X2_X_SCALE, h4.x, m4.x);
@@ -496,7 +466,107 @@
                 }
             }
     }
-    const int ntr = a.Crs / 32;
+};
+
+template <> struct WnTiles<16> {
+    typedef f32x4 Acc;
+    static constexpr int NR = 4, CW = 16, ROWS = 16, MW = 6, MW_LAST = 3;
+    static __device__ __forceinline__ int col(int lane) { return lane & 15; }
+    static __device__ __forceinline__ int krec(int lane) { return lane >> 4; }
+    static __device__ __forceinline__ int lane_row(int lane) { return 8 * (lane >> 4); }
+    static __device__ __forceinline__ int reg_row(int r) { return r; }
+    static __device__ __forceinline__ int tile_row0(int n) { return 32 * (n >> 1) + 4 * (n & 1); }
+    static __device__ __forceinline__ int gate_tile(int w, int i) { return 2 * (w + 4 * (i >> 1)) + (i & 1); }
+    static __device__ __forceinline__ int gate_row(int H, int w, int i, int r, int lane) {
+        return ((i & 1) ? H : 0) + tile_row0(w + 4 * (i >> 1)) + 8 * (lane >> 4) + r;
+    }
+    template <int MT, int NC, bool W1, bool H2, int RA, bool LAST>
+    static __device__ __forceinline__ void conv(Acc (&acc)[MT][NC], const uint4* const (&wp)[MT], const uint4* xq, int PS, int LD, int K, int dil) {
+        static_assert(!H2, "MATH_F16X2 runs on the 32x32x16 tiles");
+        b3_chunk16<MT, NC, WNB_H / 32, W1>(acc, wp, xq, PS, LD, K, dil);
+    }
+    template <int NC, bool H2>
+    static __device__ __forceinline__ void gate_store(const Acc (&acc)[MW][NC], uint4* planes, int w, int lane, float) {
+        constexpr int T_B = 16 * NC, PSU0 = WNB_NG * 2 * T_B;
+        uint2* p2 = reinterpret_cast<uint2*>(planes);
+        const int q = lane >> 4, c = lane & 15;
+        MI355_UNROLL
+        for (int i = 0; i < MW / 2; ++i) {
+            const int pr = w + 4 * i;
+            const int rec = 2 * (2 * (pr >> 1) + (q >> 1)) + (pr & 1);
+            MI355_UNROLL
+            for (int j = 0; j < NC; ++j) {
+                float u[4];
+                MI355_UNROLL
+                for (int e = 0; e < 4; ++e) u[e] = wn_gate_f(acc[2 * i][j][e], acc[2 * i + 1][j][e]);
+                const int idx = rec * T_B + 16 * j + c;
+                uint2 h2, m2, l2;
+                split3_pk(u[0], u[1], h2.x, m2.x, l2.x);
+                split3_pk(u[2], u[3], h2.y, m2.y, l2.y);
+                p2[2 * idx + (q & 1)] = h2;
+                p2[2 * (PSU0 + idx) + (q & 1)] = m2;
+                p2[2 * (2 * PSU0 + idx) + (q & 1)] = l2;
+            }
+        }
+    }
+};
+
+template <int S, bool W1, int NT, bool H2, int RA, int EP>
+__device__ __forceinline__ void wn_layer_b3_body(const WnArgs& a) {
+    typedef WnTiles<S> TL;
+    typedef typename TL::Acc Acc;
+    constexpr int MW = TL::MW, NR = TL::NR, NWV = 4, NTH = 256;
+    static_assert(!(W1 && H2), "one reduced-operand variant at a time");
+    constexpr int H = WNB_H, T_B = 32 * NT, NG = WNB_NG, NC = T_B / TL::CW;
+    constexpr int GW = H2 ? 128 : 192;
+    constexpr int TAPW = S == 16 ? (H / 32) * 192 : NG * GW;
+    constexpr float ACC = H2 ? F16X2_ACC_SCALE : 1.0f, UNACC = H2 ? 1.0f / F16X2_ACC_SCALE : 1.0f;
+    DYN_SMEM(float, smem);
+    uint4* planes = reinterpret_cast<uint4*>(smem);
+    const int tid = threadIdx.x, lane = tid & 63, w = WAVE_UNIFORM(tid >> 6);
+    const int lrow = TL::lane_row(lane), bcol = TL::col(lane);
+    const int b = blockIdx.y;
+    const int t0 = blockIdx.x * T_B;
+    int len = a.len ? a.len[b] : a.T;
+    if (len > a.T) len = a.T;
+    if (t0 >= len) return;
+    const int pad = (a.K - 1) / 2 * a.dil;
+    const int tlo = t0 - pad;
+    const int ts = tlo >= 0 ? (tlo & ~3) : -(((-tlo) + 3) & ~3);
+    const int toff = tlo - ts;
+    const int LD = a.ldx;
+    WN_TS_DECL();
+    WN_TS(0);
+    const int PS = NG * 2 * LD;
+    const bool two = a.Crs == 2 * H;
+
+    if (!(LAB_ABLATE(a) & 2)) stage_planes<NG, NG, H2>(a.h_in + (long)b * a.h_bs, a.h_ld, LD, ts, len, 1.0f, planes, PS, tid, NTH);
+    __syncthreads();
+    WN_TS(1);
+
+    const float* condp = a.cond ? a.cond + (long)b * a.cond_bs : a.b_in;
+    const float cond_on = a.cond ? 1.0f : 0.0f;
+    {
+        Acc acc[MW][NC];
+        const uint4* wp[MW];
+        MI355_UNROLL
+        for (int i = 0; i < MW; ++i) {
+            MI355_UNROLL
+            for (int r = 0; r < NR; ++r) {
+                const int c = TL::gate_row(H, w, i, r, lane);
+                const float v = (a.b_in[c] + cond_on * condp[c]) * ACC;
+                MI355_UNROLL
+                for (int j = 0; j < NC; ++j) acc[i][j][r] = v;
+            }
+            wp[i] = reinterpret_cast<const uint4*>(a.w_in) + (long)TL::gate_tile(w, i) * a.K * TAPW + lane;
+        }
+        if (!(LAB_ABLATE(a) & 1)) TL::template conv<MW, NC, W1, H2, RA, false>(acc, wp, planes + TL::krec(lane) * LD + bcol + toff, PS, LD, a.K, a.dil);
+        __syncthreads();
+        WN_TS(2);
+        WN_TS(3);
+        TL::template gate_store<NC, H2>(acc, planes, w, lane, UNACC);
+    }
+    const int ntr = a.Crs / TL::ROWS;
     const float* src[MW];
     float* dst[MW];
     long ldr[MW];
@@ -506,46 +576,47 @@
         const int q = w + NWV * i;
         valid[i] = q < ntr;
         const int qc = valid[i] ? q : ntr - 1;
-        to_h[i] = two && 32 * qc < H;
+        const int row0 = TL::tile_row0(qc);
+        to_h[i] = two && row0 < H;
         if (to_h[i]) {
-            src[i] = a.h_in + (long)b * a.h_bs + (long)(32 * qc) * a.h_ld;
-            dst[i] = a.h_out + (long)b * a.h_bs + (long)(32 * qc) * a.h_ld;
+            src[i] = a.h_in + (long)b * a.h_bs + (long)row0 * a.h_ld;
+            dst[i] = a.h_out + (long)b * a.h_bs + (long)row0 * a.h_ld;
             ldr[i] = a.h_ld;
             use_old[i] = true;
         } else {
             const int sub = two ? H : 0;
-            src[i] = a.skip + (long)b * a.s_bs + (long)(32 * qc - sub) * a.s_ld;
-            dst[i] = a.skip + (long)b * a.s_bs + (long)(32 * qc - sub) * a.s_ld;
+            src[i] = a.skip + (long)b * a.s_bs + (long)(row0 - sub) * a.s_ld;
+            dst[i] = a.skip + (long)b * a.s_bs + (long)(row0 - sub) * a.s_ld;
             ldr[i] = a.s_ld;
             use_old[i] = !a.skip_init;
         }
     }
-    auto load_tile = [&](int i, int j, float (&old)[16]) {
-        const int t = t0 + j * 32 + bcol;
+    auto load_tile = [&](int i, int j, float (&old)[NR]) {
+        const int t = t0 + j * TL::CW + bcol;
         const int tc = t < a.T ? t : a.T - 1;
         if (valid[i] && use_old[i]) {
             MI355_UNROLL
-            for (int r = 0; r < 16; ++r) old[r] = src[i][(long)((r & 3) + 8 * (r >> 2) + 4 * brow) * ldr[i] + tc];
+            for (int r = 0; r < NR; ++r) old[r] = src[i][(long)(TL::reg_row(r) + lrow) * ldr[i] + tc];
         } else {
             MI355_UNROLL
-            for (int r = 0; r < 16; ++r) old[r] = 0.0f;
+            for (int r = 0; r < NR; ++r) old[r] = 0.0f;
         }
     };
-    constexpr int EPA = EP == 0 ? 1 : 3, EPR = EPA + 1;
-    float old[EPR][16];
-    auto load_tile_b = [&](int i, int j, float (&o)[16]) MI355_INLINE_LAMBDA {
-        const int t = t0 + j * 32 + bcol;
+    constexpr int EPA = (EP == 0 ? 1 : 3) * (16 / NR), EPR = EPA + 1;
+    float old[EPR][NR];
+    auto load_tile_b = [&](int i, int j, float (&o)[NR]) MI355_INLINE_LAMBDA {
+        const int t = t0 + j * TL::CW + bcol;
         const int tc = t < a.T ? t : a.T - 1;
         const BufRsrc rs = buf_rsrc(src[i]);
         const unsigned row4 = 4u * (unsigned)ldr[i];
-        const unsigned vo = (valid[i] && use_old[i]) ? (unsigned)(4 * brow) * row4 + 4u * (unsigned)tc : BUF_OOB;
-        MI355_UNROLL
-        for (int r = 0; r < 16; ++r) o[r] = buf_load_f32(rs, vo, (unsigned)((r & 3) + 8 * (r >> 2)) * row4);
+        const unsigned vo = (valid[i] && use_old[i]) ? (unsigned)lrow * row4 + 4u * (unsigned)tc : BUF_OOB;
+        MI355_UNROLL
+        for (int r = 0; r < NR; ++r) o[r] = buf_load_f32(rs, vo, (unsigned)TL::reg_row(r) * row4);
     };
     constexpr int PSU = NG * 2 * T_B;
     __syncthreads();
     WN_TS(4);
-    f32x16 acc[MW][NT];
+    Acc acc[MW][NC];
     {
         const uint4* wp[MW];
         MI355_UNROLL
@@ -553,87 +624,93 @@
             int q = w + NWV * i;
             if (q >= ntr) q = ntr - 1;
             MI355_UNROLL
-            for (int r = 0; r < 16; ++r) {
-                const float v = a.b_rs[32 * q + (r & 3) + 8 * (r >> 2) + 4 * brow] * ACC;
-                MI355_UNROLL
-                for (int j = 0; j < NT; ++j) acc[i][j][r] = v;
-            }
-            wp[i] = reinterpret_cast<const uint4*>(a.w_rs) + (long)q * NG * GW + lane;
+            for (int r = 0; r < NR; ++r) {
+                const float v = a.b_rs[TL::tile_row0(q) + TL::reg_row(r) + lrow] * ACC;
+                MI355_UNROLL
+                for (int j = 0; j < NC; ++j) acc[i][j][r] = v;
+            }
+            wp[i] = reinterpret_cast<const uint4*>(a.w_rs) + (long)q * TAPW + lane;
         }
         if (!(LAB_ABLATE(a) & 1)) {
+            const uint4* xq = planes + TL::krec(lane) * T_B + bcol;
             if (two) {
-                if constexpr (H2) h2_chunk<MW, NT, NG, NT>(acc, wp, planes + brow * T_B + bcol, PSU, T_B, 1, NG, 0);
-                else if constexpr (RA > 2 && NT >= 4) b3_chunk_lean_ra<MW, NT, NG, W1, RA>(acc, wp, planes + brow * T_B + bcol, PSU, T_B, 1, NG, 0);
-                else if constexpr (RA > 2) b3_chunk_ra<MW, NT, NG, NT, W1, RA>(acc, wp, planes + brow * T_B + bcol, PSU, T_B, 1, NG, 0);
-                else b3_chunk<MW, NT, NG, NT, W1>(acc, wp, planes + brow * T_B + bcol, PSU, T_B, 1, NG, 0);
+                TL::template conv<MW, NC, W1, H2, RA, false>(acc, wp, xq, PSU, T_B, 1, 0);
             } else {
-                f32x16 a2[2][NT];
-                const uint4* w2[2] = {wp[0], wp[1]};
-                MI355_UNROLL
-                for (int i = 0; i < 2; ++i)
+                constexpr int ML = TL::MW_LAST;
+                Acc a2[ML][NC];
+                const uint4* w2[ML];
+                MI355_UNROLL
+                for (int i = 0; i < ML; ++i) {
+                    w2[i] = wp[i];
                     MI355_UNROLL
-                    for (int j = 0; j < NT; ++j) a2[i][j] = acc[i][j];
-                if constexpr (H2) h2_chunk<2, NT, NG, NT>(a2, w2, planes + brow * T_B + bcol, PSU, T_B, 1, NG, 0);
-                else b3_chunk<2, NT, NG, NT, W1>(a2, w2, planes + brow * T_B + bcol, PSU, T_B, 1, NG, 0);
-                MI355_UNROLL
-                for (int i = 0; i < 2; ++i)
+                    for (int j = 0; j < NC; ++j) a2[i][j] = acc[i][j];
+                }
+                TL::template conv<ML, NC, W1, H2, RA, true>(a2, w2, xq, PSU, T_B, 1, 0);
+                MI355_UNROLL
+                for (int i = 0; i < ML; ++i)
                     MI355_UNROLL
-                    for (int j = 0; j < NT; ++j) acc[i][j] = a2[i][j];
+                    for (int j = 0; j < NC; ++j) acc[i][j] = a2[i][j];
             }
         }
         if constexpr (H2) {
             MI355_UNROLL
             for (int i = 0; i < MW; ++i)
                 MI355_UNROLL
-                for (int j = 0; j < NT; ++j)
+                for (int j = 0; j < NC; ++j)
                     MI355_UNROLL
-                    for (int r = 0; r < 16; ++r) acc[i][j][r] *= UNACC;
+                    for (int r = 0; r < NR; ++r) acc[i][j][r] *= UNACC;
         }
     }
     WN_TS(5);
     if ((LAB_ABLATE(a) & 4) && acc[0][0][0] != 1.2345f) return;
-    auto store_tile = [&](int i, int j, const float (&old)[16]) {
-        const int t = t0 + j * 32 + bcol;
+    auto store_tile = [&](int i, int j, const float (&old)[NR]) {
+        const int t = t0 + j * TL::CW + bcol;
         if (!valid[i] || t >= a.T) return;
         const bool live = t < len || !to_h[i];
         MI355_UNROLL
-        for (int r = 0; r < 16; ++r) dst[i][(long)((r & 3) + 8 * (r >> 2) + 4 * brow) * ldr[i] + t] = live ? old[r] + acc[i][j][r] : 0.0f;
+        for (int r = 0; r < NR; ++r) dst[i][(long)(TL::reg_row(r) + lrow) * ldr[i] + t] = live ? old[r] + acc[i][j][r] : 0.0f;
     };
     if constexpr (EP == 0) {
-        load_tile(0, 0, old[0]);
-        MI355_UNROLL
-        for (int k = 0; k < MW * NT; ++k) {
-            if (k + 1 < MW * NT) load_tile((k + 1) / NT, (k + 1) % NT, old[(k + 1) & 1]);
+        MI355_UNROLL
+        for (int k = 0; k < EPA && k < MW * NC; ++k) load_tile(k / NC, k % NC, old[k]);
+        MI355_UNROLL
+        for (int k = 0; k < MW * NC; ++k) {
+            if (k + EPA < MW * NC) load_tile((k + EPA) / NC, (k + EPA) % NC, old[(k + EPA) % EPR]);
             SCHED_FENCE();
-            store_tile(k / NT, k % NT, old[k & 1]);
+            store_tile(k / NC, k % NC, old[k % EPR]);
             SCHED_FENCE();
         }
     } else {
-        auto store_tile_b = [&](int i, int j, const float (&o)[16]) MI355_INLINE_LAMBDA {
-            const int t = t0 + j * 32 + bcol;
+        auto store_tile_b = [&](int i, int j, const float (&o)[NR]) MI355_INLINE_LAMBDA {
+            const int t = t0 + j * TL::CW + bcol;
             const bool live = t < len || !to_h[i];
             const BufRsrc rs = buf_rsrc(dst[i]);
             const unsigned row4 = 4u * (unsigned)ldr[i];
-            const unsigned vo = (valid[i] && t < a.T) ? (unsigned)(4 * brow) * row4 + 4u * (unsigned)t : BUF_OOB;
-            MI355_UNROLL
-            for (int r = 0; r < 16; ++r) buf_store_f32(rs, vo, (unsigned)((r & 3) + 8 * (r >> 2)) * row4, live ? o[r] + acc[i][j][r] : 0.0f);
+            const unsigned vo = (valid[i] && t < a.T) ? (unsigned)lrow * row4 + 4u * (unsigned)t : BUF_OOB;
+            MI355_UNROLL
+            for (int r = 0; r < NR; ++r) buf_store_f32(rs, vo, (unsigned)TL::reg_row(r) * row4, live ? o[r] + acc[i][j][r] : 0.0f);
         };
         MI355_UNROLL
-        for (int k = 0; k < EPA && k < MW * NT; ++k) load_tile_b(k / NT, k % NT, old[k]);
-        MI355_UNROLL
-        for (int k = 0; k < MW * NT; ++k) {
-            if (k + EPA < MW * NT) load_tile_b((k + EPA) / NT, (k + EPA) % NT, old[(k + EPA) % EPR]);
+        for (int k = 0; k < EPA && k < MW * NC; ++k) load_tile_b(k / NC, k % NC, old[k]);
+        MI355_UNROLL
+        for (int k = 0; k < MW * NC; ++k) {
+            if (k + EPA < MW * NC) load_tile_b((k + EPA) / NC, (k + EPA) % NC, old[(k + EPA) % EPR]);
             SCHED_FENCE();
-            store_tile_b(k / NT, k % NT, old[k % EPR]);
+            store_tile_b(k / NC, k % NC, old[k % EPR]);
             SCHED_FENCE();
         }
     }
     WN_TS_END();
 }
 
-template <bool W1, int NT, bool H2 = false, int RA = 2, int EP = 0>
+template <int S, bool W1, int NT, bool H2 = false, int RA = 2, int EP = 0>
 __global__ __launch_bounds__(256) void k_wn_layer_b3(WnArgs a) {
-    wn_layer_b3_body<W1, NT, H2, RA, EP>(a);
+    wn_layer_b3_body<S, W1, NT, H2, RA, EP>(a);
+}
+
+int wn_layer_b3_shape() {
+    const char* s = lab_getenv("MI355VITS_WN_SHAPE");
+    return s && atoi(s) == 32 ? 32 : 16;
 }
 
 bool wn_layer_b3_supported(int H, int K, int dil) {
@@ -670,22 +747,38 @@
 #endif
         LAUNCH_KERNEL(kfn, grid, dim3(256), shmem, s, a);
     };
-    if (nt == 4 && a.math != MATH_F16X2) {
-        if (a.math == MATH_BF16W) go(k_wn_layer_b3<true, 4, false, WNB_RING, 1>);
-        else go(k_wn_layer_b3<false, 4, false, WNB_RING, 1>);
+    int epi = WNB_EPI;
+    if (const char* f = lab_getenv("MI355VITS_WN_EPI")) epi = atoi(f);
+    if ((long)a.h_ld * 128 >= 0x7fffffffL || (long)a.s_ld * 128 >= 0x7fffffffL) epi = 0;
+    if (a.math == MATH_F16X2) {
+        if (nt == 1) go(k_wn_layer_b3<32, false, 1, true>);
+        else go(k_wn_layer_b3<32, false, 3, true>);
+        return;
+    }
+    const bool w1 = a.math == MATH_BF16W;
+    if (a.shape != 32) {
+        if (nt == 4) { if (w1) go(k_wn_layer_b3<16, true, 4, false, 2, 1>); else go(k_wn_layer_b3<16, false, 4, false, 2, 1>); }
+        else if (nt == 1) { if (w1) go(k_wn_layer_b3<16, true, 1>); else go(k_wn_layer_b3<16, false, 1>); }
+        else if (w1) go(k_wn_layer_b3<16, true, 3>);
+        else if (epi == 1) go(k_wn_layer_b3<16, false, 3, false, 2, 1>);
+        else go(k_wn_layer_b3<16, false, 3>);
+        return;
+    }
+#if defined(MI355_LAB) || defined(MI355_EMU)
+    if (nt == 4) {
+        if (w1) go(k_wn_layer_b3<32, true, 4, false, WNB_RING, 1>);
+        else go(k_wn_layer_b3<32, false, 4, false, WNB_RING, 1>);
     } else if (nt == 1) {
-        if (a.math == MATH_F16X2) go(k_wn_layer_b3<false, 1, true>);
-        else if (a.math == MATH_BF16W) go(k_wn_layer_b3<true, 1>);
-        else go(k_wn_layer_b3<false, 1>);
+        if (w1) go(k_wn_layer_b3<32, true, 1>);
+        else go(k_wn_layer_b3<32, false, 1>);
     } else {
-        int epi = WNB_EPI;
-        if (const char* f = lab_getenv("MI355VITS_WN_EPI")) epi = atoi(f);
-        if ((long)a.h_ld * 128 >= 0x7fffffffL || (long)a.s_ld * 128 >= 0x7fffffffL) epi = 0;
-        if (a.math == MATH_F16X2) go(k_wn_layer_b3<false, 3, true>);
-        else if (a.math == MATH_BF16W) go(k_wn_layer_b3<true, 3>);
-        else if (epi == 1) go(k_wn_layer_b3<false, 3, false, WNB_RING, 1>);
-        else go(k_wn_layer_b3<false, 3, false, WNB_RING>);
-    }
+        if (w1) go(k_wn_layer_b3<32, true, 3>);
+        else if (epi == 1) go(k_wn_layer_b3<32, false, 3, false, WNB_RING, 1>);
+        else go(k_wn_layer_b3<32, false, 3, false, WNB_RING>);
+    }
+#else
+    throw std::runtime_error("wn_layer_b3: the 32x32x16 form exists in the lab build only");
+#endif
 }
 
 bool wn_layer_fused_supported(int H, int K, int dil) {
diff --git a/mimic3_amd/csrc/lab_api.cpp b/mimic3_amd/csrc/lab_api.cpp
--- a/mimic3_amd/csrc/lab_api.cpp
+++ b/mimic3_amd/csrc/lab_api.cpp
@@ -817,6 +817,12 @@
                 pack_conv_weights_mfma_mode(w_rs.data(), Crs, H, 1, EPI_STD, pr.data());
                 dwi = upload(pi.data(), pi.size() * 4);
                 dwr = upload(pr.data(), pr.size() * 4);
+            } else if (wn_layer_b3_shape() != 32) {
+                std::vector<uint32_t> bi(w16_packed_words(2 * H, H, K)), br(w16_packed_words(Crs, H, 1));
+                pack_conv_weights_w16(w_in.data(), 2 * H, H, K, true, bi.data());
+                pack_conv_weights_w16(w_rs.data(), Crs, H, 1, false, br.data());
+                dwi = upload(bi.data(), bi.size() * 4);
+                dwr = upload(br.data(), br.size() * 4);
             } else {
                 const size_t row = (size_t)H * K;
                 std::vector<float> wg(w_in.size());
@@ -839,7 +845,7 @@
             if (t->cond) { w.cond = dc.as<float>(); w.cond_bs = 2L * H; }
             w.len = dl.as<int>();
             w.B = B; w.H = H; w.T = T; w.K = K; w.dil = dil; w.Crs = Crs; w.skip_init = t->skip_init != 0;
-            if (t->impl == 2) { w.math = MATH_BF16X3; launch_wn_layer_b3(w, nullptr); }
+            if (t->impl == 2) { w.math = MATH_BF16X3; w.shape = wn_layer_b3_shape(); launch_wn_layer_b3(w, nullptr); }
             else launch_wn_layer(w, nullptr);
         }
         HIP_CHECK(hipDeviceSynchronize());
@@ -1314,6 +1320,14 @@
         HIP_CHECK(hipDeviceSynchronize());
         HIP_CHECK(hipGetLastError());
         HIP_CHECK(hipMemcpy(z, dz.p, nz * 4, hipMemcpyDeviceToHost));
+    });
+}
+
+int mi355vits_lab_pack_w16(const float* w, int Cout, int Cin, int K, int gate, uint32_t* out) {
+    return guarded(nullptr, [&] {
+        if (!w || !out) throw EngineError(MI355VITS_ERR_INVALID, "null argument");
+        if (Cout < 1 || Cin < 1 || K < 1 || Cin % 32 != 0 || Cout % (gate ? 64 : 32) != 0) throw EngineError(MI355VITS_ERR_INVALID, "bad shape");
+        pack_conv_weights_w16(w, Cout, Cin, K, gate != 0, out);
     });
 }
 
```

Result: faster. 804.2 million, median of 6 (+1.1%).
